# Oliverbansk/Holistic-Robot-Pose-Estimation

Measured on AMD Instinct MI355X. Metric: images/sec/GPU fwd+bwd HRNet-W32 256x256 bs=64; 1/2/4/8-GPU scaling, higher is better.
Workload: dtype bf16; 1 GPU; full network (HRNet-W32 reg backbone + HRNet-W32 DepthNet + heads + FK loss) fwd+loss+bwd+clip+Adam, BASELINE.json configs[2]; global_batch=64, per_gpu_batch=64, image=3x256x256, hrnet_w32_passes_per_image=2, parallelism=dp1, backend=single-process, rccl_ranks=1, hip_graph=True, plan_mode=hybrid, inputs=resident in HBM, optimizer=hrpe_amd.optim.FusedClipAdam (clip 5 + Adam, lr 1e-4)

## Files before the change

holistic-robot-pose-estimation_amd/_native.py:

```python
import ctypes as C
import os
import subprocess

_HERE = os.path.dirname(os.path.abspath(__file__))
LIB_PATH = os.environ.get("HRP_LIB") or os.path.join(_HERE, "libhrp_hip.so")
CSRC = os.path.join(_HERE, "csrc")

HRP_F32, HRP_BF16, HRP_F32X3 = 0, 1, 2
MAX_TAPS = 16
EW_MAX_IN = 4
EW_IDENTITY, EW_AFFINE, EW_BN_TRAIN = 0, 1, 2
FK_MAX_JOINTS, FK_MAX_KP = 32, 24
PIL_KMAX = 12


class HrpError(RuntimeError):
    pass


class ConvDesc(C.Structure):
    _fields_ = [("x", C.c_void_p), ("w", C.c_void_p), ("y", C.c_void_p), ("res", C.c_void_p),
                ("bias", C.c_void_p), ("scale", C.c_void_p), ("shift", C.c_void_p), ("stats", C.c_void_p),
                ("dtype", C.c_int32),
                ("N", C.c_int32), ("H", C.c_int32), ("W", C.c_int32), ("Cin", C.c_int32), ("x_pitch", C.c_int32),
                ("Ho", C.c_int32), ("Wo", C.c_int32), ("Cout", C.c_int32),
                ("y_H", C.c_int32), ("y_W", C.c_int32), ("y_pitch", C.c_int32), ("res_pitch", C.c_int32),
                ("out_stride", C.c_int32), ("out_off_y", C.c_int32), ("out_off_x", C.c_int32),
                ("in_stride", C.c_int32), ("ntaps", C.c_int32),
                ("dy", C.c_int32 * MAX_TAPS), ("dx", C.c_int32 * MAX_TAPS), ("wtap", C.c_int32 * MAX_TAPS),
                ("w_ntaps", C.c_int32), ("w_cout_pad", C.c_int32), ("relu", C.c_int32),
                ("bnb_x", C.c_void_p), ("bnb_mask", C.c_void_p), ("bnb_consts", C.c_void_p),
                ("bnb_x_pitch", C.c_int32), ("bnb_mask_pitch", C.c_int32),
                ("bnb_stats", C.c_void_p), ("bnb_gamma", C.c_void_p), ("bnb_beta", C.c_void_p),
                ("bnb_count", C.c_float), ("bnb_eps", C.c_float),
                ("pro_mode", C.c_int32), ("pro_reserved", C.c_int32),
                ("pro_x2", C.c_void_p), ("pro_stats", C.c_void_p), ("pro_bsums", C.c_void_p),
                ("pro_gamma", C.c_void_p), ("pro_beta", C.c_void_p),
                ("pro_count", C.c_float), ("pro_eps", C.c_float), ("pro_side", C.c_void_p),
                ("pro_mask", C.c_void_p), ("pro_side2", C.c_void_p), ("pro_side2_acc", C.c_int32), ("pro_reserved2", C.c_int32),
                ("res_mask", C.c_void_p),
                ("tail_mode", C.c_int32), ("tail_side_acc", C.c_int32), ("tail_stats", C.c_void_p), ("tail_bsums", C.c_void_p),
                ("tail_gamma", C.c_void_p), ("tail_beta", C.c_void_p), ("tail_count", C.c_float), ("tail_eps", C.c_float),
                ("tail_mask", C.c_void_p), ("tail_g", C.c_void_p), ("tail_side", C.c_void_p),
                ("tail_x2", C.c_void_p), ("tail_w2", C.c_void_p), ("tail_stats2", C.c_void_p), ("tail_gamma2", C.c_void_p),
                ("tail_beta2", C.c_void_p)]


class WgradDesc(C.Structure):
    _fields_ = [("x", C.c_void_p), ("dy", C.c_void_p), ("dw", C.c_void_p),
                ("dtype", C.c_int32),
                ("N", C.c_int32), ("H", C.c_int32), ("W", C.c_int32), ("Cin", C.c_int32), ("x_pitch", C.c_int32),
                ("Ho", C.c_int32), ("Wo", C.c_int32), ("Cout", C.c_int32), ("dy_pitch", C.c_int32),
                ("in_stride", C.c_int32), ("ntaps", C.c_int32),
                ("dy_t", C.c_int32 * MAX_TAPS), ("dx_t", C.c_int32 * MAX_TAPS),
                ("dw_cin", C.c_int32), ("dw_tap_stride", C.c_int32), ("dw_tap_off", C.c_int32), ("accumulate", C.c_int32),
                ("workspace", C.c_void_p), ("workspace_bytes", C.c_int64),
                ("phase", C.c_int32), ("reserved", C.c_int32)]


class WgradFoldDesc(C.Structure):
    _fields_ = [("workspace", C.c_void_p), ("dw", C.c_void_p),
                ("G", C.c_int32), ("pairs", C.c_int32), ("n_cib", C.c_int32), ("nte", C.c_int32), ("nb", C.c_int32),
                ("Cout", C.c_int32), ("dw_cin", C.c_int32), ("ntaps", C.c_int32), ("dw_tap_stride", C.c_int32),
                ("dw_tap_off", C.c_int32), ("accumulate", C.c_int32), ("reserved", C.c_int32)]


class Sim2RealLossDesc(C.Structure):
    _fields_ = [("rendered", C.c_void_p), ("seg", C.c_void_p), ("kp3d", C.c_void_p), ("kp3d_int", C.c_void_p),
                ("B", C.c_int32), ("HW", C.c_int32), ("K", C.c_int32), ("mask_loss", C.c_int32),
                ("w_mask", C.c_float), ("w_iou", C.c_float), ("w_scale", C.c_float), ("w_align", C.c_float),
                ("terms", C.c_void_p), ("d_rendered", C.c_void_p), ("d_kp3d", C.c_void_p), ("d_kp3d_int", C.c_void_p),
                ("workspace", C.c_void_p)]


class SilhouetteDesc(C.Structure):
    _fields_ = [("uv", C.c_void_p), ("xyz", C.c_void_p), ("faces", C.c_void_p),
                ("B", C.c_int32), ("V", C.c_int32), ("F", C.c_int32), ("H", C.c_int32), ("W", C.c_int32),
                ("sigma", C.c_float), ("blur_radius", C.c_float), ("alpha", C.c_void_p), ("logp", C.c_void_p), ("count", C.c_void_p)]


BLOCK_MAX = 2


class BlockDesc(C.Structure):
    _fields_ = [("conv1", ConvDesc), ("conv2", ConvDesc)]


class BlockInfo(C.Structure):
    _fields_ = [("n", C.c_int32), ("grid", C.c_int32), ("lds_bytes", C.c_int32), ("reserved", C.c_int32),
                ("first_wg", C.c_int32 * BLOCK_MAX), ("bands", C.c_int32 * BLOCK_MAX)]


class PackEntry(C.Structure):
    _fields_ = [("src", C.c_void_p), ("dst", C.c_void_p), ("dst_t", C.c_void_p),
                ("Cout", C.c_int32), ("Cin", C.c_int32), ("ntaps", C.c_int32), ("pad_t", C.c_int32)]


class EwInput(C.Structure):
    _fields_ = [("ptr", C.c_void_p), ("pitch", C.c_int32), ("up", C.c_int32), ("mode", C.c_int32),
                ("a", C.c_void_p), ("b", C.c_void_p), ("stats", C.c_void_p),
                ("count", C.c_float), ("eps", C.c_float)]


class EwDesc(C.Structure):
    _fields_ = [("inp", EwInput * EW_MAX_IN), ("nin", C.c_int32), ("out", C.c_void_p),
                ("out_pitch", C.c_int32), ("dtype", C.c_int32),
                ("N", C.c_int32), ("H", C.c_int32), ("W", C.c_int32), ("C", C.c_int32), ("relu", C.c_int32),
                ("mask", C.c_void_p), ("mask_pitch", C.c_int32), ("consts_out", C.c_void_p)]


class EwBwdDesc(C.Structure):
    _fields_ = [("dout", C.c_void_p), ("out", C.c_void_p), ("dout_pitch", C.c_int32), ("out_pitch", C.c_int32),
                ("inp", EwInput), ("din", C.c_void_p), ("din_pitch", C.c_int32), ("sums", C.c_void_p),
                ("dtype", C.c_int32), ("N", C.c_int32), ("H", C.c_int32), ("W", C.c_int32), ("C", C.c_int32),
                ("relu", C.c_int32), ("accumulate", C.c_int32),
                ("mask", C.c_void_p), ("mask_pitch", C.c_int32),
                ("din2", C.c_void_p), ("din2_pitch", C.c_int32), ("accumulate2", C.c_int32), ("pooled", C.c_void_p)]


class BnEntry(C.Structure):
    _fields_ = [("stats", C.c_void_p), ("a", C.c_void_p), ("b", C.c_void_p), ("c", C.c_void_p), ("d", C.c_void_p),
                ("out_scale", C.c_void_p), ("out_shift", C.c_void_p), ("counter", C.c_void_p),
                ("C", C.c_int32), ("count", C.c_float), ("momentum", C.c_float), ("eps", C.c_float),
                ("accumulate", C.c_int32)]


BATCH_MAX = 32
BATCH_CONV, BATCH_WGRAD, BATCH_EW_FWD, BATCH_EW_BWD_REDUCE, BATCH_EW_BWD_APPLY, BATCH_WGRAD_FOLD = range(6)


class BatchInfo(C.Structure):
    _fields_ = [("family", C.c_int32), ("n", C.c_int32), ("dtype", C.c_int32), ("variant", C.c_int32),
                ("grid", C.c_int32), ("lds_bytes", C.c_int32), ("grid2", C.c_int32),
                ("grid3", C.c_int32), ("lds_bytes3", C.c_int32),
                ("blk0", C.c_int32 * (BATCH_MAX + 1)), ("blk2", C.c_int32 * (BATCH_MAX + 1)),
                ("ws_bytes", C.c_int64 * BATCH_MAX)]


class PoseLossDesc(C.Structure):
    _fields_ = [(n, C.c_void_p) for n in ("pose", "rot", "trans", "root_uv", "depth", "xyz_int", "xyz_fk",
                                          "gt_pose", "gt_root_rot", "gt_root_trans", "gt_root_uv", "gt_kp3d", "gt_kp2d", "mask", "K",
                                          "d_pose", "d_rot", "d_trans", "d_root_uv", "d_depth", "d_xyz_int", "d_xyz_fk", "out")] + \
               [("weights", C.c_float * 10), ("B", C.c_int32), ("P", C.c_int32), ("J", C.c_int32), ("root", C.c_int32),
                ("image_size", C.c_float), ("rot_dim", C.c_int32)]


class EvalDesc(C.Structure):
    INPUTS = ("pred_kp3d_fk", "pred_kp3d_int", "gt_kp3d", "gt_kp2d", "K", "pred_joint", "gt_joint", "pred_rot", "gt_rot")
    PER_IMAGE = ("error3d", "error2d", "mean_jointerror", "error_depth", "batch_error_relative", "error3d_relative",
                 "error3d_int", "error2d_int", "error_depth_int", "batch_error_relative_int", "error3d_relative_int")
    PER_BATCH = ("dis3d", "dis2d", "dis3d_int", "dis2d_int", "l1_jointerror", "rotation_diff")
    _fields_ = [(n, C.c_void_p) for n in INPUTS + PER_IMAGE + PER_BATCH] + \
               [(n, C.c_int32) for n in ("B", "nkp", "dof", "rot_dim", "root", "drop_last_joint", "offset", "capacity",
                                         "batch_index", "batch_capacity")]


DEPTH_LOSS_MAX_KP = 16
DEPTH_LOSS_KINDS = {"l1": 0, "mse": 1}
XY_LOSS_KINDS = {None: 0, "l1": 1, "mse": 2}


class DepthLossDesc(C.Structure):
    POINTERS = ("pred", "gt_root_trans", "gt_kp3d", "mask", "loss", "d_pred", "errors", "losses")
    _fields_ = [(n, C.c_void_p) for n in POINTERS] + \
               [(n, C.c_int32) for n in ("B", "W", "J", "nk")] + [("kp_index", C.c_int32 * DEPTH_LOSS_MAX_KP)] + \
               [(n, C.c_int32) for n in ("depth_loss", "xy_loss", "root_col", "want_grad", "offset", "capacity", "batch_index",
                                         "batch_capacity")]


OPT_CHUNK = 4096


class OptTensor(C.Structure):
    _fields_ = [("param", C.c_void_p), ("grad", C.c_void_p), ("exp_avg", C.c_void_p), ("exp_avg_sq", C.c_void_p),
                ("numel", C.c_int64)]


class OptChunk(C.Structure):
    _fields_ = [("tensor", C.c_int32), ("offset", C.c_int32)]


class OptGroup(C.Structure):
    _fields_ = [("lr", C.c_float), ("beta1", C.c_float), ("beta2", C.c_float), ("eps", C.c_float),
                ("weight_decay", C.c_float), ("reserved", C.c_float * 3)]


class RegStepDesc(C.Structure):
    _fields_ = [("M", C.c_int32), ("P", C.c_int32), ("K", C.c_int32), ("N", C.c_int32),
                ("u_prev", C.c_void_p), ("u_bias", C.c_void_p), ("z", C.c_void_p), ("zw", C.c_void_p),
                ("z_len", C.c_int32), ("z_pitch", C.c_int32), ("zw_sk", C.c_int32), ("zw_sp", C.c_int32),
                ("u_out", C.c_void_p), ("a", C.c_void_p), ("a_mask", C.c_void_p), ("v", C.c_void_p),
                ("a_pitch", C.c_int32), ("v_sk", C.c_int32), ("v_sp", C.c_int32), ("a2_pitch", C.c_int32),
                ("a_out", C.c_void_p), ("w", C.c_void_p), ("bias", C.c_void_p), ("out_mask", C.c_void_p),
                ("a2", C.c_void_p), ("w2", C.c_void_p), ("w_sn", C.c_int64), ("w_sk", C.c_int64),
                ("out_pitch", C.c_int32), ("out_accumulate", C.c_int32), ("out_sum_accumulate", C.c_int32), ("w2_sk", C.c_int32),
                ("out", C.c_void_p), ("out_sum", C.c_void_p)]


class LinWgradDesc(C.Structure):
    _fields_ = [("x", C.c_void_p), ("dy", C.c_void_p), ("dw", C.c_void_p), ("dbias", C.c_void_p),
                ("x_pitch", C.c_int32), ("dy_pitch", C.c_int32), ("dw_ld", C.c_int32), ("M", C.c_int32),
                ("K", C.c_int32), ("N", C.c_int32), ("accumulate", C.c_int32), ("reserved", C.c_int32)]


REG_MAX_P, REG_MAX_PROBLEMS, LIN_WGRAD_MAX = 16, 4, 8
COPY_MAX = 16


class CopyDesc(C.Structure):
    _fields_ = [("src", C.c_void_p), ("dst", C.c_void_p), ("src_pitch", C.c_int), ("dst_pitch", C.c_int), ("rows", C.c_int),
                ("cols", C.c_int), ("accumulate", C.c_int), ("reserved", C.c_int)]


def copy_cols_batch(items, stream):
    for i0 in range(0, len(items), COPY_MAX):
        grp = items[i0:i0 + COPY_MAX]
        arr = (CopyDesc * len(grp))()
        for d, (src, sp, dst, dp, rows, cols, acc) in zip(arr, grp):
            d.src, d.src_pitch, d.dst, d.dst_pitch, d.rows, d.cols, d.accumulate = src, sp, dst, dp, rows, cols, acc
        call("hrp_copy_cols_batch", arr, len(grp), stream)


class FkChain(C.Structure):
    _fields_ = [("njoints", C.c_int32), ("parent", C.c_int32 * FK_MAX_JOINTS), ("type", C.c_int32 * FK_MAX_JOINTS),
                ("cfg", C.c_int32 * FK_MAX_JOINTS), ("mimic_mul", C.c_float * FK_MAX_JOINTS),
                ("mimic_off", C.c_float * FK_MAX_JOINTS), ("origin", (C.c_float * 12) * FK_MAX_JOINTS),
                ("axis", (C.c_float * 3) * FK_MAX_JOINTS), ("nkp", C.c_int32), ("kp_frame", C.c_int32 * FK_MAX_KP),
                ("kp_offset", (C.c_float * 3) * FK_MAX_KP), ("dof", C.c_int32)]


DREAM_BANDS = 32
DREAM_JITTER, DREAM_OCCLUSION, DREAM_SHARPNESS, DREAM_CONTRAST, DREAM_BRIGHTNESS, DREAM_COLOR = 1, 2, 4, 8, 16, 32


class DreamSample(C.Structure):
    _fields_ = [("jitter", C.c_double * 3), ("enh", C.c_double * 4), ("flags", C.c_int32),
                ("occ_x", C.c_int32), ("occ_y", C.c_int32), ("occ_w", C.c_int32), ("occ_h", C.c_int32),
                ("pad_x", C.c_int32), ("pad_y", C.c_int32), ("work_w", C.c_int32), ("work_h", C.c_int32),
                ("crop_x0", C.c_int32), ("crop_y0", C.c_int32), ("crop_x1", C.c_int32), ("crop_y1", C.c_int32),
                ("off_x", C.c_int32), ("off_y", C.c_int32), ("side", C.c_int32), ("reserved", C.c_int32),
                ("noise_off", C.c_int64), ("scratch_off", C.c_int64)]


_P, _I, _F, _L = C.c_void_p, C.c_int, C.c_float, C.c_int64
PROTOTYPES = {
    "hrp_version": [], "hrp_device_ok": [],
    "hrp_nchw_to_nhwc": [_P, _P, _I, _I, _I, _I, _I, _I, _P],
    "hrp_nhwc_to_nchw": [_P, _P, _I, _I, _I, _I, _I, _I, _P],
    "hrp_nchw_grad_from_nhwc": [_P, _P, _I, _I, _I, _I, _I, _I, _P],
    "hrp_pack_weights": [_P, _I, _I, _I, _P],
    "hrp_pack_blocks": [_I, _I, _I, _I, _I, _I],
    "hrp_pack_weights_compact": [_P, _P, _I, _I, _I, _P],
    "hrp_nchw_to_nhwc_s2d": [_P, _P, _I, _I, _I, _I, _I, _I, _P],
    "hrp_u8_nchw_to_nhwc": [_P, _P, _I, _I, _I, _I, _I, _I, _F, _I, _P],
    "hrp_gather_f32": [_P, _P, _P, _I, _I, _P],
    "hrp_pil_resize_table": [_I, _I, _P],
    "hrp_pil_resize_normalize": [_P, _I, _I, _I, _I, _P, _P, _I, _I, _P, _I, _I, _I, _P, _P, _P],
    "hrp_broadcast_hw": [_P, _I, _P, _I, _I, _I, _I, _I, _P],
    "hrp_bilinear_nhwc_to_nchw": [_P, _I, _I, _I, _I, _I, _I, _P, _I, _I, _I, _P],
    "hrp_fill_zero": [_P, _L, _P],
    "hrp_maxpool3x3s2_fwd": [_P, _I, _I, _I, _I, _I, _I, _P, _I, _P, _P],
    "hrp_maxpool3x3s2_bwd": [_P, _I, _P, _P, _I, _I, _I, _I, _I, _I, _I, _P],
    "hrp_conv2d_fwd": [C.POINTER(ConvDesc), _P],
    "hrp_conv_rowstrip_channels": [C.POINTER(ConvDesc)],
    "hrp_conv_pointwise": [C.POINTER(ConvDesc)],
    "hrp_conv2d_bwd_weight": [C.POINTER(WgradDesc), _P],
    "hrp_colsum": [_P, _I, _L, _I, _I, _P, _I, _P, _L, _P],
    "hrp_colsum_workspace_bytes": [_L, _I],
    "hrp_ew_fwd": [C.POINTER(EwDesc), _P],
    "hrp_ew_bwd_reduce": [C.POINTER(EwBwdDesc), _P],
    "hrp_ew_pool2": [_P, _I, _I, _P, _I, _I, _I, _I, _I, _P, _P],
    "hrp_ew_bwd_apply": [C.POINTER(EwBwdDesc), _P],
    "hrp_bn_running_update": [_P, _I, _P], "hrp_bn_fold": [_P, _I, _P], "hrp_bn_param_grad": [_P, _I, _P],
    "hrp_avgpool_fwd": [_P, _I, _I, _I, _I, _I, _P, _I, _P],
    "hrp_avgpool_bwd": [_P, _I, _P, _I, _I, _I, _I, _I, _I, _P],
    "hrp_softargmax3d_fwd": [_P, _I, _I, _I, _I, _I, _I, _I, _I, _I, _P, _P, _P],
    "hrp_softargmax3d_bwd": [_P, _I, _I, _I, _I, _I, _I, _I, _I, _I, _P, _P, _P, _P, _I, _P],
    "hrp_pose_geometry_fwd": [_P, _P, _P, _P, _I, _I, _I, _F, _F, _P, _P, _P, _P, _P],
    "hrp_pose_geometry_bwd": [_P, _P, _P, _P, _I, _I, _I, _F, _F, _P, _P, _P, _P, _P, _P, _P],
    "hrp_fk_project_fwd": [_P, _P, _P, _P, _P, _I, _I, _P, _P, _P, _P],
    "hrp_fk_project_bwd": [_P, _P, _P, _P, _P, _I, _I, _P, _P, _P, _P, _P, _P],
    "hrp_fk_project_rot_fwd": [_P, _P, _P, _I, _P, _P, _I, _I, _P, _P, _P, _P],
    "hrp_fk_project_rot_bwd": [_P, _P, _P, _I, _P, _P, _I, _I, _P, _P, _P, _P, _P, _P],
    "hrp_copy_cols": [_P, _I, _P, _I, _I, _I, _I, _P],
    "hrp_copy_cols_batch": [_P, _I, _P],
    "hrp_scale_rows": [_P, _I, _I, _I, _P, _F, _P],
    "hrp_mul_f32": [_P, _I, _P, _I, _P, _I, _I, _I, _I, _P],
    "hrp_opt_grad_sumsq": [_P, _P, _I, _P, _P, _P],
    "hrp_opt_adam_step": [_P, _P, _I, _P, _F, _P, _F, _F, _F, _F, _P],
    "hrp_opt_adam_step_groups": [_P, _P, _I, _P, _F, _P, _P, _I, _P, _P],
    "hrp_opt_set_group": [_P, _I, _I, _F, _F, _F, _F, _F, _P],
    "hrp_grad_accumulate": [_P, _P, _L, _I, _F, _P],
    "hrp_batch_prepare": [_I, _P, _I, _P, C.POINTER(BatchInfo)],
    "hrp_batch_launch": [_P, C.POINTER(BatchInfo), _P],
    "hrp_softargmax_flat_fwd": [_P, _I, _I, _I, _I, _I, _P, _P, _P],
    "hrp_softargmax_flat_bwd": [_P, _I, _I, _I, _I, _I, _P, _P, _P, _P, _I, _P],
    "hrp_rot6d_compose_fwd": [_P, _P, _P, _I, _P],
    "hrp_rot6d_compose_bwd": [_P, _P, _P, _P, _P, _I, _I, _I, _P],
    "hrp_wgrad_fold_desc_of": [C.POINTER(WgradDesc), C.POINTER(WgradFoldDesc)],
    "hrp_batch_wgrad_fold_descs": [_P, C.POINTER(BatchInfo), C.POINTER(WgradFoldDesc)],
    "hrp_block_channels": [C.POINTER(BlockDesc)],
    "hrp_block_prepare": [_P, _I, _P, C.POINTER(BlockInfo)],
    "hrp_block_launch": [_P, C.POINTER(BlockInfo), _P],
    "hrp_pose_loss": [C.POINTER(PoseLossDesc), _P],
    "hrp_l1_loss": [_P, _P, _F, _I, _P, _P, _P],
    "hrp_sim2real_loss": [C.POINTER(Sim2RealLossDesc), _P],
    "hrp_mesh_pose": [_P, _P, _P, _P, _I, _I, _P, _P, _I, _P, _P, _P, _P],
    "hrp_mesh_pose_bwd": [_P, _P, _P, _P, _I, _I, _P, _P, _I, _P, _P, _P, _P],
    "hrp_silhouette_fwd": [C.POINTER(SilhouetteDesc), _P],
    "hrp_silhouette_bwd": [C.POINTER(SilhouetteDesc), _P, _P, _P],
    "hrp_linear_fwd": [_P, _I, _P, _P, _P, _I, _P, _I, _I, _I, _I, _P, _L, _P],
    "hrp_linear_bwd_data": [_P, _I, _P, _P, _I, _I, _I, _I, _I, _P, _L, _P],
    "hrp_linear_workspace_bytes": [_I, _I, _I],
    "hrp_linear_bwd_weight": [_P, _I, _P, _I, _P, _P, _I, _I, _I, _I, _P],
    "hrp_rng_advance": [_P, _P],
    "hrp_dropout_f32": [_P, _I, _P, _I, _P, _I, _I, _F, _P, C.c_uint32, _P],
    "hrp_dropout_masks": [_P, _L, _F, _P, C.c_uint32, _P],
    "hrp_regressor_step": [_P, _I, _P],
    "hrp_linear_wgrad_batch": [_P, _I, _P],
    "hrp_project_fwd": [_P, _P, _I, _I, _P, _P],
    "hrp_project_bwd": [_P, _P, _P, _I, _I, _P, _P],
    "hrp_pnp_solve": [_P, _P, _I, _P, _I, _P, _I, _I, _P, _P, _P, _P],
    "hrp_pnp_bwd": [_P, _P, _I, _P, _I, _P, _P, _I, _I, _I, _P, _P, _P, _P, _P, _P, _P],
    "hrp_dream_augment": [_P, _I, _I, _I, _P, _P, _L, _I, _I, _P, _L, _P, _P],
    "hrp_dream_crop_resize": [_P, _L, _P, _P, _I, _I, _I, _P, _I, _I, _P, _I, _I, _P],
    "hrp_eval_batch": [C.POINTER(EvalDesc), _P],
    "hrp_depth_loss": [C.POINTER(DepthLossDesc), _P],
}

_lib = None


def source_hash():
    import glob
    import hashlib
    files = [os.path.basename(f) for f in glob.glob(os.path.join(CSRC, "*.hip")) + glob.glob(os.path.join(CSRC, "*.h"))]
    names = sorted(files + ["../../include/hrp.h", "Makefile"])
    h = hashlib.sha256()
    for n in names:
        with open(os.path.join(CSRC, n), "rb") as fh:
            h.update(fh.read())
    return h.hexdigest()[:16]


def build(force=False):
    if force:
        subprocess.run(["make", "-C", CSRC, "clean"], check=True, stdout=subprocess.DEVNULL)
    r = subprocess.run(["make", "-C", CSRC, "-j8"], stdout=subprocess.PIPE, stderr=subprocess.STDOUT, text=True)
    if r.returncode != 0:
        raise HrpError("building libhrp_hip.so failed:\n" + r.stdout[-4000:])
    return LIB_PATH


def lib():
    global _lib
    if _lib is None:
        if not os.path.exists(LIB_PATH):
            raise HrpError(f"{LIB_PATH} not found: run `python -c 'import __graft_entry__ as g; g.build()'` "
                           "(there is no CPU fallback)")
        import torch
        L = C.CDLL(LIB_PATH)
        for name, args in PROTOTYPES.items():
            fn = getattr(L, name)
            fn.argtypes = args
            fn.restype = C.c_int
        L.hrp_last_error.restype = C.c_char_p
        L.hrp_last_error.argtypes = []
        L.hrp_source_hash.restype = C.c_char_p
        L.hrp_source_hash.argtypes = []
        L.hrp_wgrad_workspace_bytes.restype = C.c_int64
        L.hrp_linear_workspace_bytes.restype = C.c_int64
        L.hrp_colsum_workspace_bytes.restype = C.c_int64
        L.hrp_wgrad_workspace_bytes.argtypes = [C.POINTER(WgradDesc)]
        L.hrp_batch_table_bytes.restype = C.c_int64
        L.hrp_batch_table_bytes.argtypes = [C.c_int, C.c_int]
        L.hrp_block_table_bytes.restype = C.c_int64
        L.hrp_block_table_bytes.argtypes = []
        _lib = L
    return _lib


def check(rc, what=""):
    if rc != 0:
        raise HrpError(f"{what} failed ({rc}): {lib().hrp_last_error().decode()}")


_profile_hook = None


def set_profile_hook(fn):
    global _profile_hook
    _profile_hook = fn


def profiling():
    return _profile_hook is not None


_skip = frozenset(filter(None, os.environ.get("HRP_SKIP", "").split(",")))


def call(name, *args):
    if _skip and name in _skip:
        return
    if _profile_hook is not None:
        _profile_hook(name, args, lambda: check(getattr(lib(), name)(*args), name))
        return
    check(getattr(lib(), name)(*args), name)


def call_batch(batch, stream):
    name = "hrp_batch_launch"
    if _skip and (name in _skip or FAMILY_FN[batch.fam] in _skip):
        return
    fn = lambda: check(lib().hrp_batch_launch(batch.table.data_ptr(), C.byref(batch.info), stream), name)
    if _profile_hook is not None:
        _profile_hook(name, (batch,), fn)
        return
    fn()


def call_block(batch, stream):
    name = "hrp_block_launch"
    if _skip and name in _skip:
        return
    fn = lambda: check(lib().hrp_block_launch(batch.table, C.byref(batch.info), stream), name)
    if _profile_hook is not None:
        _profile_hook(name, (batch,), fn)
        return
    fn()


FAMILY_FN = {"block": "hrp_block_launch", "conv": "hrp_conv2d_fwd", "wgrad": "hrp_conv2d_bwd_weight", "wgrad_fold": "hrp_wgrad_fold", "ew_fwd": "hrp_ew_fwd", "ew_red": "hrp_ew_bwd_reduce",
             "ew_app": "hrp_ew_bwd_apply"}
```

holistic-robot-pose-estimation_amd/csrc/core.hip:

```cpp
#include "hrp_common.h"
#include <type_traits>
#include <string.h>

namespace hrp {

static thread_local char g_err[512] = "";

void set_error(const char* fmt, ...) {
  va_list ap;
  va_start(ap, fmt);
  vsnprintf(g_err, sizeof(g_err), fmt, ap);
  va_end(ap);
}

int check_launch(const char* what) {
  hipError_t e = hipGetLastError();
  if (e != hipSuccess) {
    set_error("%s: %s", what, hipGetErrorString(e));
    return HRP_ERR_LAUNCH;
  }
  return HRP_OK;
}

template <typename T, typename S>
__global__ __launch_bounds__(256) void nchw_to_nhwc_kernel(const S* __restrict__ src, void* __restrict__ dst,
                                                           int C, int HW, int pitch, float div) {
  size_t p = (size_t)blockIdx.x * 256 + threadIdx.x;
  int n = blockIdx.y;
  if (p >= (size_t)HW) return;
  const S* s = src + (size_t)n * C * HW + p;
  size_t o = ((size_t)n * HW + p) * pitch;
  if (pitch * Elem<T>::SZ == 16) {
    constexpr int V = 16 / Elem<T>::SZ;
    float v[V];
#pragma unroll
    for (int c = 0; c < V; ++c) {
      v[c] = c < C ? (float)s[(size_t)c * HW] : 0.f;
      if (sizeof(S) == 1) v[c] = v[c] * (1.0f / div);
    }
    *(uint4*)((char*)dst + o * Elem<T>::SZ) = Elem<T>::pack(v);
    return;
  }
  for (int c = 0; c < pitch; ++c) {
    float v = c < C ? (float)s[(size_t)c * HW] : 0.f;
    if (sizeof(S) == 1) v = v * (1.0f / div);
    Elem<T>::st(dst, o + c, v);
  }
}

template <typename T, typename S>
__global__ __launch_bounds__(256) void nchw_to_nhwc_s2d_kernel(const S* __restrict__ src, void* __restrict__ dst,
                                                               int C, int H, int W, int pitch, float div) {
  const int Ho = (H + 1) / 2, Wo = (W + 1) / 2;
  size_t p = (size_t)blockIdx.x * 256 + threadIdx.x;
  const int n = blockIdx.y;
  if (p >= (size_t)Ho * Wo) return;
  const int y = p / Wo, x = p - (size_t)y * Wo;
  const S* sn = src + (size_t)n * C * H * W;
  size_t o = ((size_t)n * Ho * Wo + p) * pitch;
  for (int k = 0; k < pitch; ++k) {
    float v = 0.f;
    if (k < 4 * C) {
      const int q = k / C, c = k - q * C, iy = 2 * y + (q >> 1), ix = 2 * x + (q & 1);
      if (iy < H && ix < W) v = (float)sn[((size_t)c * H + iy) * W + ix];
      if (sizeof(S) == 1) v = v * (1.0f / div);
    }
    Elem<T>::st(dst, o + k, v);
  }
}

__global__ __launch_bounds__(256) void gather_f32_kernel(const float* __restrict__ src, const int* __restrict__ idx,
                                                         float* __restrict__ dst, int n, int accumulate) {
  const int i = blockIdx.x * 256 + threadIdx.x;
  if (i >= n) return;
  const int j = idx[i];
  const float v = j >= 0 ? src[j] : 0.f;
  dst[i] = accumulate ? dst[i] + v : v;
}

template <typename T>
__global__ __launch_bounds__(256) void maxpool_fwd_kernel(const void* __restrict__ x, int H, int W, int C, int pitch,
                                                          void* __restrict__ y, int Ho, int Wo, int y_pitch,
                                                          uint8_t* __restrict__ arg, long total) {
  constexpr int V = Elem<T>::VEC;
  const int nv = C / V;
  for (long i = (long)blockIdx.x * 256 + threadIdx.x; i < total; i += (long)gridDim.x * 256) {
    const int cv = i % nv;
    long r = i / nv;
    const int ox = r % Wo; r /= Wo;
    const int oy = r % Ho;
    const long n = r / Ho;
    float best[V];
    int bi[V];
#pragma unroll
    for (int k = 0; k < V; ++k) { best[k] = -INFINITY; bi[k] = 0; }
    for (int ky = 0; ky < 3; ++ky) {
      const int iy = 2 * oy - 1 + ky;
      if (iy < 0 || iy >= H) continue;
      for (int kx = 0; kx < 3; ++kx) {
        const int ix = 2 * ox - 1 + kx;
        if (ix < 0 || ix >= W) continue;
        float f[V];
        Elem<T>::unpack(*(const uint4*)((const char*)x + ((((size_t)n * H + iy) * W + ix) * pitch + cv * V) * Elem<T>::SZ), f);
#pragma unroll
        for (int k = 0; k < V; ++k)
          if (f[k] > best[k]) { best[k] = f[k]; bi[k] = ky * 3 + kx; }
      }
    }
    const size_t o = (((size_t)n * Ho + oy) * Wo + ox);
    *(uint4*)((char*)y + (o * y_pitch + cv * V) * Elem<T>::SZ) = Elem<T>::pack(best);
    if (arg) {
#pragma unroll
      for (int k = 0; k < V; ++k) arg[o * C + cv * V + k] = (uint8_t)bi[k];
    }
  }
}

template <typename T>
__global__ __launch_bounds__(256) void maxpool_bwd_kernel(const void* __restrict__ dy, int Ho, int Wo, int dy_pitch,
                                                          const uint8_t* __restrict__ arg, void* __restrict__ dx, int H, int W,
                                                          int C, int pitch, int accumulate, long total) {
  constexpr int V = Elem<T>::VEC;
  const int nv = C / V;
  for (long i = (long)blockIdx.x * 256 + threadIdx.x; i < total; i += (long)gridDim.x * 256) {
    const int cv = i % nv;
    long r = i / nv;
    const int ix = r % W; r /= W;
    const int iy = r % H;
    const long n = r / H;
    float g[V];
#pragma unroll
    for (int k = 0; k < V; ++k) g[k] = 0.f;
    for (int oy = iy / 2; oy <= (iy + 1) / 2; ++oy) {
      if (oy < 0 || oy >= Ho) continue;
      const int ky = iy - (2 * oy - 1);
      if (ky < 0 || ky > 2) continue;
      for (int ox = ix / 2; ox <= (ix + 1) / 2; ++ox) {
        if (ox < 0 || ox >= Wo) continue;
        const int kx = ix - (2 * ox - 1);
        if (kx < 0 || kx > 2) continue;
        const size_t o = (((size_t)n * Ho + oy) * Wo + ox);
        float f[V];
        Elem<T>::unpack(*(const uint4*)((const char*)dy + (o * dy_pitch + cv * V) * Elem<T>::SZ), f);
        const uint8_t* a = arg + o * C + cv * V;
#pragma unroll
        for (int k = 0; k < V; ++k)
          if (a[k] == ky * 3 + kx) g[k] += f[k];
      }
    }
    char* dst = (char*)dx + ((((size_t)n * H + iy) * W + ix) * pitch + cv * V) * Elem<T>::SZ;
    if (accumulate) {
      float old[V];
      Elem<T>::unpack(*(const uint4*)dst, old);
#pragma unroll
      for (int k = 0; k < V; ++k) g[k] += old[k];
    }
    *(uint4*)dst = Elem<T>::pack(g);
  }
}

template <typename T, bool GRAD>
__global__ __launch_bounds__(256) void nhwc_to_nchw_kernel(const void* __restrict__ src, float* __restrict__ dst,
                                                           int C, int HW, int pitch) {
  __shared__ float tile[64][65];
  const int n = blockIdx.z, p0 = blockIdx.x * 64, c0 = blockIdx.y * 64;
  const int tx = threadIdx.x & 63, ty = threadIdx.x >> 6;
  for (int r = ty; r < 64; r += 4) {
    int p = p0 + r, c = c0 + tx;
    tile[r][tx] = (p < HW && c < C) ? Elem<T>::ld(src, ((size_t)n * HW + p) * pitch + c) : 0.f;
  }
  __syncthreads();
  for (int r = ty; r < 64; r += 4) {
    int c = c0 + r, p = p0 + tx;
    if (p < HW && c < C) dst[((size_t)n * C + c) * HW + p] = tile[tx][r];
  }
}

template <typename T>
__device__ __forceinline__ void pack_entry(const hrp_pack_entry& e, const unsigned blk, const unsigned nblk) {
  constexpr int CK = 32 / Elem<T>::SZ;
  const unsigned Cout = e.Cout, Cin = e.Cin, nt = e.ntaps;
  const unsigned cout_pad = (Cout + 31) / 32 * 32, cin_pad = (Cin + 31) / 32 * 32;
  auto store_row = [&](void* dst, size_t row, const float (&v)[CK]) {
    if constexpr (std::is_same<T, f32x3_t>::value) {
      uint4* q = (uint4*)((char*)dst + row * 32);
      split_bf16x8(v, q[0], q[1]);
      return;
    }
    float a[CK / 2], b[CK / 2];
#pragma unroll
    for (int k = 0; k < CK / 2; ++k) { a[k] = v[k]; b[k] = v[CK / 2 + k]; }
    uint4* q = (uint4*)((char*)dst + row * 32);
    q[0] = Elem<T>::pack(a);
    q[1] = Elem<T>::pack(b);
  };
  if (e.dst) {
    const unsigned nch = (Cin + CK - 1) / CK, rows = nch * nt * cout_pad;
    for (unsigned i = blk * 256 + threadIdx.x; i < rows; i += nblk * 256) {
      const unsigned tap = i % nt, q = i / nt, co = q % cout_pad, ch = q / cout_pad;
      float v[CK];
#pragma unroll
      for (int k = 0; k < CK; ++k) {
        const unsigned ci = ch * CK + k;
        v[k] = (co < Cout && ci < Cin) ? e.src[((size_t)co * Cin + ci) * nt + tap] : 0.f;
      }
      store_row(e.dst, (size_t)(ch * nt + tap) * cout_pad + co, v);
    }
  }
  if (e.dst_t) {
    const unsigned nch = (Cout + CK - 1) / CK, rows = nch * nt * cin_pad;
    for (unsigned i = blk * 256 + threadIdx.x; i < rows; i += nblk * 256) {
      const unsigned tap = i % nt, q = i / nt, ci = q % cin_pad, ch = q / cin_pad;
      float v[CK];
#pragma unroll
      for (int k = 0; k < CK; ++k) {
        const unsigned co = ch * CK + k;
        v[k] = (co < Cout && ci < Cin) ? e.src[((size_t)co * Cin + ci) * nt + tap] : 0.f;
      }
      store_row(e.dst_t, (size_t)(ch * (nt + e.pad_t) + tap) * cin_pad + ci, v);
    }
  }
}

template <typename T>
__global__ __launch_bounds__(256) void pack_weights_kernel(const hrp_pack_entry* __restrict__ table) {
  const hrp_pack_entry e = table[blockIdx.y];
  pack_entry<T>(e, blockIdx.x, gridDim.x);
}

constexpr int PACK_TILE_TAPS = 9;
template <typename T>
__device__ __forceinline__ void pack_store_row(void* dst, const size_t row, const float (&v)[32 / Elem<T>::SZ]) {
  constexpr int CK = 32 / Elem<T>::SZ;
  uint4* q = (uint4*)((char*)dst + row * 32);
  if constexpr (std::is_same<T, f32x3_t>::value) {
    split_bf16x8(v, q[0], q[1]);
  } else {
    float a[CK / 2], b[CK / 2];
#pragma unroll
    for (int k = 0; k < CK / 2; ++k) { a[k] = v[k]; b[k] = v[CK / 2 + k]; }
    q[0] = Elem<T>::pack(a);
    q[1] = Elem<T>::pack(b);
  }
}

template <typename T>
__device__ __forceinline__ void pack_entry_tile(const hrp_pack_entry& e, const unsigned tile_id, float* __restrict__ lds) {
  constexpr int CK = 32 / Elem<T>::SZ, NC = 32 / CK;
  const unsigned Cout = e.Cout, Cin = e.Cin, nt = e.ntaps;
  const unsigned cout_pad = (Cout + 31) / 32 * 32, cin_pad = (Cin + 31) / 32 * 32;
  const unsigned n_cit = cin_pad / 32;
  if (tile_id >= (cout_pad / 32) * n_cit) return;
  const unsigned co0 = (tile_id / n_cit) * 32, ci0 = (tile_id % n_cit) * 32;
  const unsigned span = 32 * nt, pitch = span + 1;
  {
    const unsigned wave = threadIdx.x >> 6, lane = threadIdx.x & 63;
    const unsigned valid = Cin > ci0 ? (Cin - ci0 < 32 ? (Cin - ci0) * nt : span) : 0;
    for (unsigned r0 = wave; r0 < 32; r0 += 16) {
      for (unsigned j = lane; j < span; j += 64) {
        float v[4];
#pragma unroll
        for (int u = 0; u < 4; ++u) {
          const unsigned co = co0 + r0 + 4 * u;
          v[u] = (co < Cout && j < valid) ? e.src[((size_t)co * Cin + ci0) * nt + j] : 0.f;
        }
#pragma unroll
        for (int u = 0; u < 4; ++u) lds[(r0 + 4 * u) * pitch + j] = v[u];
      }
    }
  }
  __syncthreads();
  if (e.dst) {
    const unsigned nch = (Cin + CK - 1) / CK;
    for (unsigned r = threadIdx.x; r < NC * nt * 32; r += 256) {
      const unsigned co = r & 31, q = r >> 5, tap = q % nt, c = q / nt, ch = ci0 / CK + c;
      if (ch >= nch) continue;
      float v[CK];
#pragma unroll
      for (int k = 0; k < CK; ++k) v[k] = lds[co * pitch + (c * CK + k) * nt + tap];
      pack_store_row<T>(e.dst, (size_t)(ch * nt + tap) * cout_pad + co0 + co, v);
    }
  }
  if (e.dst_t) {
    const unsigned nch = (Cout + CK - 1) / CK;
    for (unsigned r = threadIdx.x; r < NC * nt * 32; r += 256) {
      const unsigned ci = r & 31, q = r >> 5, tap = q % nt, c = q / nt, ch = co0 / CK + c;
      if (ch >= nch) continue;
      float v[CK];
#pragma unroll
      for (int k = 0; k < CK; ++k) v[k] = lds[(c * CK + k) * pitch + ci * nt + tap];
      pack_store_row<T>(e.dst_t, (size_t)(ch * (nt + e.pad_t) + tap) * cin_pad + ci0 + ci, v);
    }
  }
}

constexpr int PACK_ROWS_PER_BLOCK = 256 * 4;
template <typename T>
__global__ __launch_bounds__(256) void pack_weights_compact_kernel(const hrp_pack_entry* __restrict__ table, const int32_t* __restrict__ first,
                                                                   const int count) {
  int lo = 0, hi = count;
  while (hi - lo > 1) {
    const int mid = (lo + hi) >> 1;
    if (first[mid] <= (int)blockIdx.x) lo = mid; else hi = mid;
  }
  const hrp_pack_entry e = table[lo];
  if (e.ntaps <= PACK_TILE_TAPS) {
    __shared__ float lds[32 * (32 * PACK_TILE_TAPS + 1)];
    pack_entry_tile<T>(e, blockIdx.x - first[lo], lds);
    return;
  }
  pack_entry<T>(e, blockIdx.x - first[lo], first[lo + 1] - first[lo]);
}

template <typename T>
__global__ __launch_bounds__(256) void colsum_kernel(const void* __restrict__ x, long rows, int C, int pitch,
                                                     float* __restrict__ out, float* __restrict__ ws) {
  __shared__ float part[4][64];
  const int tx = threadIdx.x & 63, ty = threadIdx.x >> 6;
  const int c = blockIdx.y * 64 + tx;
  float s = 0.f;
  if (c < C)
    for (long r = (long)blockIdx.x * 4 + ty; r < rows; r += (long)gridDim.x * 4) s += Elem<T>::ld(x, (size_t)r * pitch + c);
  part[ty][tx] = s;
  __syncthreads();
  if (ty == 0 && c < C) {
    const float v = part[0][tx] + part[1][tx] + part[2][tx] + part[3][tx];
    if (ws) ws[(size_t)blockIdx.x * C + c] = v;
    else atomicAdd(&out[c], v);
  }
}

__global__ __launch_bounds__(256) void colsum_fold_kernel(const float* __restrict__ ws, int groups, int C, float* __restrict__ out,
                                                          int accumulate) {
  const int c = blockIdx.x * 256 + threadIdx.x;
  if (c >= C) return;
  float v = 0.f;
  for (int g0 = 0; g0 < groups; g0 += 8) {
    float t[8];
#pragma unroll
    for (int u = 0; u < 8; ++u) t[u] = g0 + u < groups ? ws[(size_t)(g0 + u) * C + c] : 0.f;
#pragma unroll
    for (int u = 0; u < 8; ++u) v += t[u];
  }
  out[c] = accumulate ? out[c] + v : v;
}

__global__ void bn_running_update_kernel(const hrp_bn_entry* __restrict__ table) {
  const hrp_bn_entry e = table[blockIdx.x];
  for (int c = threadIdx.x; c < e.C; c += blockDim.x) {
    float mean = slot_sum(e.stats, c, 2 * e.C) / e.count;
    float var = fmaxf(slot_sum(e.stats, e.C + c, 2 * e.C) / e.count - mean * mean, 0.f);
    float unbiased = e.count > 1.f ? var * (e.count / (e.count - 1.f)) : var;
    e.a[c] = (1.f - e.momentum) * e.a[c] + e.momentum * mean;
    e.b[c] = (1.f - e.momentum) * e.b[c] + e.momentum * unbiased;
  }
  if (threadIdx.x == 0 && e.counter) *e.counter += 1;
}

__global__ void bn_fold_kernel(const hrp_bn_entry* __restrict__ table) {
  const hrp_bn_entry e = table[blockIdx.x];
  for (int c = threadIdx.x; c < e.C; c += blockDim.x) {
    float sc = e.a[c] * rsqrtf(e.d[c] + e.eps);
    e.out_scale[c] = sc;
    e.out_shift[c] = e.b[c] - e.c[c] * sc;
  }
}

__global__ void bn_param_grad_kernel(const hrp_bn_entry* __restrict__ table) {
  const hrp_bn_entry e = table[blockIdx.x];
  for (int c = threadIdx.x; c < e.C; c += blockDim.x) {
    float dbeta = slot_sum(e.stats, c, 2 * e.C), dgamma = slot_sum(e.stats, e.C + c, 2 * e.C);
    if (e.accumulate) { e.a[c] += dgamma; e.b[c] += dbeta; }
    else { e.a[c] = dgamma; e.b[c] = dbeta; }
  }
}

template <typename T>
__global__ __launch_bounds__(256) void avgpool_fwd_kernel(const void* __restrict__ x, int HW, int C, int pitch,
                                                          float* __restrict__ out, int out_pitch) {
  const int n = blockIdx.y;
  const int c = blockIdx.x * 256 + threadIdx.x;
  if (c >= C) return;
  float s = 0.f;
  for (int p = 0; p < HW; ++p) s += Elem<T>::ld(x, ((size_t)n * HW + p) * pitch + c);
  out[(size_t)n * out_pitch + c] = s / (float)HW;
}

template <typename T>
__global__ __launch_bounds__(256) void avgpool_bwd_kernel(const float* __restrict__ dout, int dout_pitch, void* __restrict__ dx,
                                                          int HW, int C, int pitch, int accumulate) {
  const int n = blockIdx.y;
  const int c = blockIdx.x * 256 + threadIdx.x;
  if (c >= C) return;
  const float g = dout[(size_t)n * dout_pitch + c] / (float)HW;
  for (int p = 0; p < HW; ++p) {
    size_t o = ((size_t)n * HW + p) * pitch + c;
    Elem<T>::st(dx, o, accumulate ? Elem<T>::ld(dx, o) + g : g);
  }
}

__global__ void copy_cols_kernel(const float* __restrict__ src, int sp, float* __restrict__ dst, int dp, int rows, int cols, int acc) {
  size_t i = (size_t)blockIdx.x * 256 + threadIdx.x;
  if (i >= (size_t)rows * cols) return;
  int r = i / cols, c = i % cols;
  float v = src[(size_t)r * sp + c];
  float* d = dst + (size_t)r * dp + c;
  *d = acc ? *d + v : v;
}

struct CopyBatchArgs { hrp_copy_desc d[HRP_COPY_MAX]; };
__global__ void copy_cols_batch_kernel(const CopyBatchArgs a) {
  const hrp_copy_desc& d = a.d[blockIdx.y];
  const size_t total = (size_t)d.rows * d.cols;
  for (size_t i = (size_t)blockIdx.x * 256 + threadIdx.x; i < total; i += (size_t)gridDim.x * 256) {
    const int r = (int)(i / d.cols), c = (int)(i - (size_t)r * d.cols);
    const float v = d.src ? d.src[(size_t)r * d.src_pitch + c] : 0.f;
    float* q = d.dst + (size_t)r * d.dst_pitch + c;
    *q = d.accumulate ? *q + v : v;
  }
}

__global__ void scale_rows_kernel(float* __restrict__ x, int pitch, int rows, int cols, const float* __restrict__ rs, float s) {
  size_t i = (size_t)blockIdx.x * 256 + threadIdx.x;
  if (i >= (size_t)rows * cols) return;
  int r = i / cols, c = i % cols;
  x[(size_t)r * pitch + c] *= (rs ? rs[r] : 1.f) * s;
}

__global__ void mul_kernel(const float* __restrict__ x, int xp, const float* __restrict__ m, int mp, float* __restrict__ y, int yp,
                           int rows, int cols, int acc) {
  size_t i = (size_t)blockIdx.x * 256 + threadIdx.x;
  if (i >= (size_t)rows * cols) return;
  int r = i / cols, c = i % cols;
  float v = x[(size_t)r * xp + c] * m[(size_t)r * mp + c];
  float* d = y + (size_t)r * yp + c;
  *d = acc ? *d + v : v;
}

__device__ __forceinline__ void philox_round(uint32_t (&c)[4], uint32_t k0, uint32_t k1) {
  const uint32_t hi0 = __umulhi(0xD2511F53u, c[0]), lo0 = 0xD2511F53u * c[0];
  const uint32_t hi1 = __umulhi(0xCD9E8D57u, c[2]), lo1 = 0xCD9E8D57u * c[2];
  const uint32_t n0 = hi1 ^ c[1] ^ k0, n1 = lo1, n2 = hi0 ^ c[3] ^ k1, n3 = lo0;
  c[0] = n0; c[1] = n1; c[2] = n2; c[3] = n3;
}

__global__ void rng_advance_kernel(uint64_t* state) { state[1] += 1; }

__global__ __launch_bounds__(256) void dropout_kernel(const float* __restrict__ x, int xp, float* __restrict__ y, int yp,
                                                      float* __restrict__ mask, int rows, int cols, float keep,
                                                      const uint64_t* __restrict__ state, uint32_t salt) {
  const size_t q = (size_t)blockIdx.x * 256 + threadIdx.x;
  const size_t n = (size_t)rows * cols;
  if (q * 4 >= n) return;
  const uint64_t seed = state[0], step = state[1];
  uint32_t c[4] = {(uint32_t)q, (uint32_t)(q >> 32) ^ salt, (uint32_t)step, (uint32_t)(step >> 32)};
  uint32_t k0 = (uint32_t)seed, k1 = (uint32_t)(seed >> 32);
#pragma unroll
  for (int r = 0; r < 10; ++r) {
    philox_round(c, k0, k1);
    k0 += 0x9E3779B9u; k1 += 0xBB67AE85u;
  }
  const float scale = 1.0f / keep;
#pragma unroll
  for (int j = 0; j < 4; ++j) {
    const size_t i = q * 4 + j;
    if (i >= n) break;
    const float u = (float)(c[j] >> 8) * (1.0f / 16777216.0f);
    const float m = u < keep ? scale : 0.f;
    const int r = (int)(i / cols), cc = (int)(i - (size_t)r * cols);
    mask[i] = m;
    y[(size_t)r * yp + cc] = x[(size_t)r * xp + cc] * m;
  }
}

}

using namespace hrp;

#ifndef HRP_SRC_HASH
#define HRP_SRC_HASH "unknown"
#endif
extern "C" const char* hrp_source_hash(void) { return HRP_SRC_HASH; }

extern "C" int hrp_rng_advance(uint64_t* state_dev, void* stream) {
  HRP_REQUIRE(state_dev, "rng_advance: null state");
  hipLaunchKernelGGL(rng_advance_kernel, dim3(1), dim3(1), 0, (hipStream_t)stream, state_dev);
  return check_launch("rng_advance");
}

extern "C" int hrp_dropout_f32(const float* x, int x_pitch, float* y, int y_pitch, float* mask, int rows, int cols, float keep,
                               const uint64_t* state_dev, uint32_t salt, void* stream) {
  HRP_REQUIRE(x && y && mask && state_dev && rows > 0 && cols > 0, "dropout: bad args");
  HRP_REQUIRE(keep > 0.f && keep <= 1.f, "dropout: keep probability %f", (double)keep);
  const size_t quads = ((size_t)rows * cols + 3) / 4;
  hipLaunchKernelGGL(dropout_kernel, dim3((unsigned)((quads + 255) / 256)), dim3(256), 0, (hipStream_t)stream, x, x_pitch, y, y_pitch,
                     mask, rows, cols, keep, state_dev, salt);
  return check_launch("dropout");
}

extern "C" int hrp_mul_f32(const float* x, int x_pitch, const float* m, int m_pitch, float* y, int y_pitch, int rows, int cols,
                           int accumulate, void* stream) {
  HRP_REQUIRE(x && m && y && rows > 0 && cols > 0, "mul_f32: bad args");
  hipLaunchKernelGGL(mul_kernel, dim3(cdiv(rows * cols, 256)), dim3(256), 0, (hipStream_t)stream, x, x_pitch, m, m_pitch, y, y_pitch,
                     rows, cols, accumulate);
  return check_launch("mul_f32");
}

extern "C" const char* hrp_last_error(void) { return hrp::g_err; }
extern "C" int hrp_version(void) { return 100; }

extern "C" int hrp_device_ok(void) {
  int dev = 0;
  if (hipGetDevice(&dev) != hipSuccess) return 0;
  hipDeviceProp_t p;
  if (hipGetDeviceProperties(&p, dev) != hipSuccess) return 0;
  return strncmp(p.gcnArchName, "gfx950", 6) == 0 ? 1 : 0;
}

extern "C" int hrp_nchw_to_nhwc(const float* src, void* dst, int dtype, int N, int C, int H, int W, int dst_pitch, void* stream) {
  HRP_REQUIRE(src && dst && N > 0 && C > 0 && dst_pitch >= C, "nchw_to_nhwc: bad args");
  dim3 grid(cdiv(H * W, 256), N);
  if (dtype == HRP_F32) hipLaunchKernelGGL((nchw_to_nhwc_kernel<float, float>), grid, dim3(256), 0, (hipStream_t)stream, src, dst, C, H * W, dst_pitch, 1.f);
  else hipLaunchKernelGGL((nchw_to_nhwc_kernel<bf16_t, float>), grid, dim3(256), 0, (hipStream_t)stream, src, dst, C, H * W, dst_pitch, 1.f);
  return check_launch("nchw_to_nhwc");
}

extern "C" int hrp_u8_nchw_to_nhwc(const uint8_t* src, void* dst, int dtype, int N, int C, int H, int W, int dst_pitch,
                                   float divisor, int s2d, void* stream) {
  HRP_REQUIRE(src && dst && N > 0 && C > 0 && divisor > 0.f, "u8_nchw_to_nhwc: bad args");
  HRP_REQUIRE(dst_pitch >= (s2d ? 4 * C : C), "u8_nchw_to_nhwc: dst_pitch too small");
  hipStream_t st = (hipStream_t)stream;
  if (s2d) {
    dim3 grid(cdiv(((H + 1) / 2) * ((W + 1) / 2), 256), N);
    if (dtype == HRP_F32) hipLaunchKernelGGL((nchw_to_nhwc_s2d_kernel<float, uint8_t>), grid, dim3(256), 0, st, src, dst, C, H, W, dst_pitch, divisor);
    else hipLaunchKernelGGL((nchw_to_nhwc_s2d_kernel<bf16_t, uint8_t>), grid, dim3(256), 0, st, src, dst, C, H, W, dst_pitch, divisor);
  } else {
    dim3 grid(cdiv(H * W, 256), N);
    if (dtype == HRP_F32) hipLaunchKernelGGL((nchw_to_nhwc_kernel<float, uint8_t>), grid, dim3(256), 0, st, src, dst, C, H * W, dst_pitch, divisor);
    else hipLaunchKernelGGL((nchw_to_nhwc_kernel<bf16_t, uint8_t>), grid, dim3(256), 0, st, src, dst, C, H * W, dst_pitch, divisor);
  }
  return check_launch("u8_nchw_to_nhwc");
}

extern "C" int hrp_nchw_to_nhwc_s2d(const float* src, void* dst, int dtype, int N, int C, int H, int W, int dst_pitch, void* stream) {
  HRP_REQUIRE(src && dst && N > 0 && C > 0 && dst_pitch >= 4 * C, "nchw_to_nhwc_s2d: bad args");
  dim3 grid(cdiv(((H + 1) / 2) * ((W + 1) / 2), 256), N);
  if (dtype == HRP_F32) hipLaunchKernelGGL((nchw_to_nhwc_s2d_kernel<float, float>), grid, dim3(256), 0, (hipStream_t)stream, src, dst, C, H, W, dst_pitch, 1.f);
  else hipLaunchKernelGGL((nchw_to_nhwc_s2d_kernel<bf16_t, float>), grid, dim3(256), 0, (hipStream_t)stream, src, dst, C, H, W, dst_pitch, 1.f);
  return check_launch("nchw_to_nhwc_s2d");
}

extern "C" int hrp_fill_zero(void* p, int64_t bytes, void* stream) {
  HRP_REQUIRE(p && bytes >= 0, "fill_zero: bad args");
  zero_async(p, (size_t)bytes, (hipStream_t)stream);
  return check_launch("fill_zero");
}

extern "C" int hrp_gather_f32(const float* src, const int32_t* idx, float* dst, int n, int accumulate, void* stream) {
  HRP_REQUIRE(src && idx && dst && n > 0, "gather_f32: bad args");
  hipLaunchKernelGGL(gather_f32_kernel, dim3(cdiv(n, 256)), dim3(256), 0, (hipStream_t)stream, src, idx, dst, n, accumulate);
  return check_launch("gather_f32");
}

extern "C" int hrp_maxpool3x3s2_fwd(const void* x, int dtype, int N, int H, int W, int C, int pitch, void* y, int y_pitch,
                                    uint8_t* argmax, void* stream) {
  const int vec = dtype == HRP_F32 ? 4 : 8, sz = dtype == HRP_F32 ? 4 : 2;
  HRP_REQUIRE(x && y && N > 0 && H > 0 && W > 0 && C > 0, "maxpool_fwd: bad args");
  HRP_REQUIRE(C % vec == 0 && pitch % vec == 0 && y_pitch % vec == 0 && (uintptr_t)x % 16 == 0 && (uintptr_t)y % 16 == 0,
              "maxpool_fwd: channels / pitches must be multiples of %d and the tensors 16-byte aligned", vec);
  (void)sz;
  const int Ho = (H + 2 - 3) / 2 + 1, Wo = (W + 2 - 3) / 2 + 1;
  const long total = (long)N * Ho * Wo * (C / vec);
  long blocks = (total + 255) / 256;
  if (blocks > 4096) blocks = 4096;
  if (dtype == HRP_F32) hipLaunchKernelGGL(maxpool_fwd_kernel<float>, dim3((int)blocks), dim3(256), 0, (hipStream_t)stream, x, H, W, C, pitch, y, Ho, Wo, y_pitch, argmax, total);
  else hipLaunchKernelGGL(maxpool_fwd_kernel<bf16_t>, dim3((int)blocks), dim3(256), 0, (hipStream_t)stream, x, H, W, C, pitch, y, Ho, Wo, y_pitch, argmax, total);
  return check_launch("maxpool_fwd");
}

extern "C" int hrp_maxpool3x3s2_bwd(const void* dy, int dy_pitch, const uint8_t* argmax, void* dx, int dtype, int N, int H, int W,
                                    int C, int pitch, int accumulate, void* stream) {
  const int vec = dtype == HRP_F32 ? 4 : 8;
  HRP_REQUIRE(dy && argmax && dx && N > 0 && H > 0 && W > 0 && C > 0, "maxpool_bwd: bad args");
  HRP_REQUIRE(C % vec == 0 && pitch % vec == 0 && dy_pitch % vec == 0 && (uintptr_t)dx % 16 == 0 && (uintptr_t)dy % 16 == 0,
              "maxpool_bwd: channels / pitches must be multiples of %d and the tensors 16-byte aligned", vec);
  const int Ho = (H + 2 - 3) / 2 + 1, Wo = (W + 2 - 3) / 2 + 1;
  const long total = (long)N * H * W * (C / vec);
  long blocks = (total + 255) / 256;
  if (blocks > 4096) blocks = 4096;
  if (dtype == HRP_F32) hipLaunchKernelGGL(maxpool_bwd_kernel<float>, dim3((int)blocks), dim3(256), 0, (hipStream_t)stream, dy, Ho, Wo, dy_pitch, argmax, dx, H, W, C, pitch, accumulate, total);
  else hipLaunchKernelGGL(maxpool_bwd_kernel<bf16_t>, dim3((int)blocks), dim3(256), 0, (hipStream_t)stream, dy, Ho, Wo, dy_pitch, argmax, dx, H, W, C, pitch, accumulate, total);
  return check_launch("maxpool_bwd");
}

extern "C" int hrp_nhwc_to_nchw(const void* src, float* dst, int dtype, int N, int C, int H, int W, int src_pitch, void* stream) {
  HRP_REQUIRE(src && dst && N > 0 && C > 0 && src_pitch >= C, "nhwc_to_nchw: bad args");
  dim3 grid(cdiv(H * W, 64), cdiv(C, 64), N);
  if (dtype == HRP_F32) hipLaunchKernelGGL((nhwc_to_nchw_kernel<float, false>), grid, dim3(256), 0, (hipStream_t)stream, src, dst, C, H * W, src_pitch);
  else hipLaunchKernelGGL((nhwc_to_nchw_kernel<bf16_t, false>), grid, dim3(256), 0, (hipStream_t)stream, src, dst, C, H * W, src_pitch);
  return check_launch("nhwc_to_nchw");
}

extern "C" int hrp_nchw_grad_from_nhwc(const void* src, float* dst, int dtype, int N, int C, int H, int W, int src_pitch, void* stream) {
  return hrp_nhwc_to_nchw(src, dst, dtype, N, C, H, W, src_pitch, stream);
}

extern "C" int hrp_pack_weights(const hrp_pack_entry* table_dev, int count, int dtype, int max_elems, void* stream) {
  HRP_REQUIRE(table_dev && count > 0, "pack_weights: empty table");
  int bx = cdiv(max_elems, 256 * 16 * 4);
  if (bx < 1) bx = 1;
  if (bx > 256) bx = 256;
  dim3 grid(bx, count);
  if (dtype == HRP_F32) hipLaunchKernelGGL(pack_weights_kernel<float>, grid, dim3(256), 0, (hipStream_t)stream, table_dev);
  else if (dtype == HRP_F32X3) hipLaunchKernelGGL(pack_weights_kernel<f32x3_t>, grid, dim3(256), 0, (hipStream_t)stream, table_dev);
  else hipLaunchKernelGGL(pack_weights_kernel<bf16_t>, grid, dim3(256), 0, (hipStream_t)stream, table_dev);
  return check_launch("pack_weights");
}

extern "C" int hrp_pack_blocks(int Cout, int Cin, int ntaps, int dtype, int has_dst, int has_dst_t) {
  if (Cout <= 0 || Cin <= 0 || ntaps <= 0) return 0;
  const int CK = dtype == HRP_BF16 ? 16 : 8;
  const long cout_pad = (Cout + 31) / 32 * 32, cin_pad = (Cin + 31) / 32 * 32;
  if (ntaps <= PACK_TILE_TAPS) return (int)((cout_pad / 32) * (cin_pad / 32));
  const long rf = has_dst ? (long)cdiv(Cin, CK) * ntaps * cout_pad : 0, rt = has_dst_t ? (long)cdiv(Cout, CK) * ntaps * cin_pad : 0;
  const long rows = rf > rt ? rf : rt;
  const long b = (rows + PACK_ROWS_PER_BLOCK - 1) / PACK_ROWS_PER_BLOCK;
  return (int)(b < 1 ? 1 : b);
}

extern "C" int hrp_pack_weights_compact(const hrp_pack_entry* table_dev, const int32_t* first_block_dev, int count, int total_blocks,
                                        int dtype, void* stream) {
  HRP_REQUIRE(table_dev && first_block_dev && count > 0 && total_blocks >= count, "pack_weights_compact: empty table / fewer workgroups than entries");
  const dim3 grid(total_blocks);
  if (dtype == HRP_F32) hipLaunchKernelGGL(pack_weights_compact_kernel<float>, grid, dim3(256), 0, (hipStream_t)stream, table_dev, first_block_dev, count);
  else if (dtype == HRP_F32X3) hipLaunchKernelGGL(pack_weights_compact_kernel<f32x3_t>, grid, dim3(256), 0, (hipStream_t)stream, table_dev, first_block_dev, count);
  else hipLaunchKernelGGL(pack_weights_compact_kernel<bf16_t>, grid, dim3(256), 0, (hipStream_t)stream, table_dev, first_block_dev, count);
  return check_launch("pack_weights_compact");
}

static inline int colsum_groups(int64_t rows) {
  int gx = (int)((rows + 63) / 64);
  if (gx > 512) gx = 512;
  return gx < 1 ? 1 : gx;
}

extern "C" int64_t hrp_colsum_workspace_bytes(int64_t rows, int C) { return rows > 0 && C > 0 ? (int64_t)colsum_groups(rows) * C * 4 : 0; }

extern "C" int hrp_colsum(const void* x, int dtype, int64_t rows, int C, int pitch, float* out, int accumulate, void* workspace,
                          int64_t workspace_bytes, void* stream) {
  HRP_REQUIRE(x && out && rows > 0 && C > 0, "colsum: bad args");
  const int gx = colsum_groups(rows);
  float* ws = (float*)workspace;
  HRP_REQUIRE(!ws || workspace_bytes >= (int64_t)gx * C * 4, "colsum: workspace too small");
  if (!ws && !accumulate) zero_async(out, sizeof(float) * C, (hipStream_t)stream);
  dim3 grid(gx, cdiv(C, 64));
  if (dtype == HRP_F32) hipLaunchKernelGGL(colsum_kernel<float>, grid, dim3(256), 0, (hipStream_t)stream, x, (long)rows, C, pitch, out, ws);
  else hipLaunchKernelGGL(colsum_kernel<bf16_t>, grid, dim3(256), 0, (hipStream_t)stream, x, (long)rows, C, pitch, out, ws);
  if (ws) hipLaunchKernelGGL(colsum_fold_kernel, dim3(cdiv(C, 256)), dim3(256), 0, (hipStream_t)stream, ws, gx, C, out, accumulate);
  return check_launch("colsum");
}

extern "C" int hrp_bn_running_update(const hrp_bn_entry* table_dev, int count, void* stream) {
  HRP_REQUIRE(table_dev && count > 0, "bn_running_update: empty table");
  hipLaunchKernelGGL(bn_running_update_kernel, dim3(count), dim3(256), 0, (hipStream_t)stream, table_dev);
  return check_launch("bn_running_update");
}
extern "C" int hrp_bn_fold(const hrp_bn_entry* table_dev, int count, void* stream) {
  HRP_REQUIRE(table_dev && count > 0, "bn_fold: empty table");
  hipLaunchKernelGGL(bn_fold_kernel, dim3(count), dim3(256), 0, (hipStream_t)stream, table_dev);
  return check_launch("bn_fold");
}
extern "C" int hrp_bn_param_grad(const hrp_bn_entry* table_dev, int count, void* stream) {
  HRP_REQUIRE(table_dev && count > 0, "bn_param_grad: empty table");
  hipLaunchKernelGGL(bn_param_grad_kernel, dim3(count), dim3(256), 0, (hipStream_t)stream, table_dev);
  return check_launch("bn_param_grad");
}

__global__ __launch_bounds__(256) void opt_grad_sumsq_kernel(const hrp_opt_tensor* __restrict__ tensors,
                                                             const hrp_opt_chunk* __restrict__ chunks,
                                                             float* __restrict__ slots, float* __restrict__ chunk_sums) {
  const hrp_opt_chunk ck = chunks[blockIdx.x];
  const hrp_opt_tensor t = tensors[ck.tensor];
  const int64_t base = (int64_t)ck.offset * HRP_OPT_CHUNK;
  const int64_t left = t.numel - base;
  const int n = left < HRP_OPT_CHUNK ? (int)left : HRP_OPT_CHUNK;
  const float* g = t.grad + base;
  float s = 0.f;
  if ((n & 3) == 0 && ((uintptr_t)g & 15) == 0) {
    for (int i = threadIdx.x * 4; i < n; i += 1024) {
      const float4 v = *(const float4*)(g + i);
      s += v.x * v.x + v.y * v.y + v.z * v.z + v.w * v.w;
    }
  } else {
    for (int i = threadIdx.x; i < n; i += 256) s += g[i] * g[i];
  }
  s = wave_sum(s);
  __shared__ float part[4];
  if ((threadIdx.x & 63) == 0) part[threadIdx.x >> 6] = s;
  __syncthreads();
  if (threadIdx.x == 0) {
    const float tot = part[0] + part[1] + part[2] + part[3];
    if (chunk_sums) chunk_sums[blockIdx.x] = tot;
    else atomicAdd(&slots[blockIdx.x & (HRP_STAT_SLOTS - 1)], tot);
  }
}

__global__ __launch_bounds__(256) void opt_fold_sumsq_kernel(const float* __restrict__ chunk_sums, int n, float* __restrict__ slots) {
  __shared__ float part[256];
  float s = 0.f;
  for (int i = threadIdx.x; i < n; i += 256) s += chunk_sums[i];
  part[threadIdx.x] = s;
  __syncthreads();
  for (int o = 128; o > 0; o >>= 1) {
    if ((int)threadIdx.x < o) part[threadIdx.x] += part[threadIdx.x + o];
    __syncthreads();
  }
  if (threadIdx.x < HRP_STAT_SLOTS) slots[threadIdx.x] = threadIdx.x == 0 ? part[0] : 0.f;
}

template <bool DECAY>
__device__ __forceinline__ void opt_adam_chunk(const hrp_opt_tensor t, const hrp_opt_chunk ck, const float* __restrict__ slots,
                                               float max_norm, const float* __restrict__ step_dev, float lr, float b1, float b2,
                                               float eps, float wd) {
  const int64_t base = (int64_t)ck.offset * HRP_OPT_CHUNK;
  const int64_t left = t.numel - base;
  const int n = left < HRP_OPT_CHUNK ? (int)left : HRP_OPT_CHUNK;
  float clip = 1.f;
  if (max_norm > 0.f) {
    float ss = 0.f;
#pragma unroll
    for (int k = 0; k < HRP_STAT_SLOTS; ++k) ss += slots[k];
    clip = fminf(1.f, max_norm / (sqrtf(ss) + 1e-6f));
  }
  const float step = *step_dev;
  const float bc1 = 1.f - powf(b1, step), bc2 = 1.f - powf(b2, step);
  const float step_size = lr / bc1, inv_sqrt_bc2 = 1.f / sqrtf(bc2);
  float* p = t.param + base;
  float* g = t.grad + base;
  float* m = t.exp_avg + base;
  float* v = t.exp_avg_sq + base;
  auto run = [&](auto with_decay) {
    auto upd = [&](float& pp, float& gg, float& mm, float& vv) {
      gg *= clip;
      if constexpr (decltype(with_decay)::value) {
        const float ge = gg + wd * pp;
        mm = b1 * mm + (1.f - b1) * ge;
        vv = b2 * vv + (1.f - b2) * ge * ge;
      } else {
        mm = b1 * mm + (1.f - b1) * gg;
        vv = b2 * vv + (1.f - b2) * gg * gg;
      }
      pp -= step_size * mm / (sqrtf(vv) * inv_sqrt_bc2 + eps);
    };
    if ((n & 3) == 0 && (((uintptr_t)p | (uintptr_t)g | (uintptr_t)m | (uintptr_t)v) & 15) == 0) {
      for (int i = threadIdx.x * 4; i < n; i += 1024) {
        float4 pp = *(float4*)(p + i), gg = *(float4*)(g + i), mm = *(float4*)(m + i), vv = *(float4*)(v + i);
        upd(pp.x, gg.x, mm.x, vv.x); upd(pp.y, gg.y, mm.y, vv.y); upd(pp.z, gg.z, mm.z, vv.z); upd(pp.w, gg.w, mm.w, vv.w);
        *(float4*)(p + i) = pp; *(float4*)(g + i) = gg; *(float4*)(m + i) = mm; *(float4*)(v + i) = vv;
      }
    } else {
      for (int i = threadIdx.x; i < n; i += 256) upd(p[i], g[i], m[i], v[i]);
    }
  };
  if (DECAY && wd != 0.f) run(std::true_type{});
  else run(std::false_type{});
}

__global__ __launch_bounds__(256) void opt_adam_kernel(const hrp_opt_tensor* __restrict__ tensors,
                                                       const hrp_opt_chunk* __restrict__ chunks,
                                                       const float* __restrict__ slots, float max_norm,
                                                       const float* __restrict__ step_dev, float lr, float b1, float b2,
                                                       float eps) {
  const hrp_opt_chunk ck = chunks[blockIdx.x];
  const hrp_opt_tensor t = tensors[ck.tensor];
  opt_adam_chunk<false>(t, ck, slots, max_norm, step_dev, lr, b1, b2, eps, 0.f);
}

__global__ __launch_bounds__(256) void opt_adam_groups_kernel(const hrp_opt_tensor* __restrict__ tensors,
                                                              const hrp_opt_chunk* __restrict__ chunks,
                                                              const float* __restrict__ slots, float max_norm,
                                                              const float* __restrict__ step_dev,
                                                              const hrp_opt_group* __restrict__ groups, int ngroups,
                                                              const int32_t* __restrict__ tensor_group) {
  const hrp_opt_chunk ck = chunks[blockIdx.x];
  const int gi = tensor_group[ck.tensor];
  const hrp_opt_group h = groups[gi < 0 ? 0 : gi >= ngroups ? ngroups - 1 : gi];
  opt_adam_chunk<true>(tensors[ck.tensor], ck, slots, max_norm, step_dev, h.lr, h.beta1, h.beta2, h.eps, h.weight_decay);
}

__global__ void opt_set_group_kernel(hrp_opt_group* __restrict__ groups, int index, float lr, float b1, float b2, float eps,
                                     float wd) {
  hrp_opt_group h = {};
  h.lr = lr, h.beta1 = b1, h.beta2 = b2, h.eps = eps, h.weight_decay = wd;
  groups[index] = h;
}

extern "C" int hrp_opt_grad_sumsq(const hrp_opt_tensor* tensors_dev, const hrp_opt_chunk* chunks_dev, int nchunks,
                                  float* sumsq_slots, float* chunk_sums, void* stream) {
  HRP_REQUIRE(tensors_dev && chunks_dev && sumsq_slots && nchunks > 0, "opt_grad_sumsq: bad args");
  hipLaunchKernelGGL(opt_grad_sumsq_kernel, dim3(nchunks), dim3(256), 0, (hipStream_t)stream, tensors_dev, chunks_dev, sumsq_slots,
                     chunk_sums);
  if (chunk_sums)
    hipLaunchKernelGGL(opt_fold_sumsq_kernel, dim3(1), dim3(256), 0, (hipStream_t)stream, chunk_sums, nchunks, sumsq_slots);
  return check_launch("opt_grad_sumsq");
}
extern "C" int hrp_opt_adam_step(const hrp_opt_tensor* tensors_dev, const hrp_opt_chunk* chunks_dev, int nchunks,
                                 const float* sumsq_slots, float max_norm, const float* step_dev,
                                 float lr, float beta1, float beta2, float eps, void* stream) {
  HRP_REQUIRE(tensors_dev && chunks_dev && step_dev && nchunks > 0, "opt_adam_step: bad args");
  HRP_REQUIRE(max_norm <= 0.f || sumsq_slots, "opt_adam_step: clipping needs the sum-of-squares slots");
  hipLaunchKernelGGL(opt_adam_kernel, dim3(nchunks), dim3(256), 0, (hipStream_t)stream, tensors_dev, chunks_dev, sumsq_slots,
                     max_norm, step_dev, lr, beta1, beta2, eps);
  return check_launch("opt_adam_step");
}

extern "C" int hrp_opt_adam_step_groups(const hrp_opt_tensor* tensors_dev, const hrp_opt_chunk* chunks_dev, int nchunks,
                                        const float* sumsq_slots, float max_norm, const float* step_dev,
                                        const hrp_opt_group* groups_dev, int ngroups, const int32_t* tensor_group_dev,
                                        void* stream) {
  HRP_REQUIRE(tensors_dev && chunks_dev && step_dev && nchunks > 0, "opt_adam_step_groups: bad args");
  HRP_REQUIRE(groups_dev && tensor_group_dev, "opt_adam_step_groups: null group table");
  HRP_REQUIRE(ngroups >= 1, "opt_adam_step_groups: ngroups %d < 1", ngroups);
  HRP_REQUIRE(max_norm <= 0.f || sumsq_slots, "opt_adam_step_groups: clipping needs the sum-of-squares slots");
  hipLaunchKernelGGL(opt_adam_groups_kernel, dim3(nchunks), dim3(256), 0, (hipStream_t)stream, tensors_dev, chunks_dev,
                     sumsq_slots, max_norm, step_dev, groups_dev, ngroups, tensor_group_dev);
  return check_launch("opt_adam_step_groups");
}
extern "C" int hrp_opt_set_group(hrp_opt_group* groups_dev, int ngroups, int index, float lr, float beta1, float beta2, float eps,
                                 float weight_decay, void* stream) {
  HRP_REQUIRE(groups_dev, "opt_set_group: null group table");
  HRP_REQUIRE(ngroups >= 1, "opt_set_group: ngroups %d < 1", ngroups);
  HRP_REQUIRE(index >= 0 && index < ngroups, "opt_set_group: index %d outside [0, %d)", index, ngroups);
  hipLaunchKernelGGL(opt_set_group_kernel, dim3(1), dim3(1), 0, (hipStream_t)stream, groups_dev, index, lr, beta1, beta2, eps,
                     weight_decay);
  return check_launch("opt_set_group");
}

constexpr int GACC_THREADS = 256, GACC_MAX_BLOCKS = 256 * 8;

typedef float gacc_f4 __attribute__((ext_vector_type(4)));

template <int MODE, bool SCALED, typename V>
__device__ __forceinline__ V gacc_sum(V a, V s, float scale) {
#pragma clang fp contract(off)
  V v = s;
  if (SCALED) v = s * scale;
  if (MODE) v = a + v;
  return v;
}
template <int MODE, typename V>
__device__ __forceinline__ V gacc_load(const V* p) {
  if (MODE) return *p;
  return V(0.f);
}

template <int MODE, bool SCALED>
__global__ __launch_bounds__(GACC_THREADS) void grad_accumulate_kernel(const float* __restrict__ src, float* __restrict__ acc,
                                                                       int64_t n, float scale) {
  const int64_t nvec = n >> 2;
  const int64_t stride = (int64_t)gridDim.x * GACC_THREADS;
  const gacc_f4* __restrict__ s4 = (const gacc_f4*)src;
  gacc_f4* __restrict__ a4 = (gacc_f4*)acc;
  int64_t i = (int64_t)blockIdx.x * GACC_THREADS + threadIdx.x;
  for (; i + stride < nvec; i += 2 * stride) {
    const gacc_f4 s0 = s4[i], s1 = s4[i + stride];
    const gacc_f4 a0 = gacc_load<MODE>(a4 + i), a1 = gacc_load<MODE>(a4 + i + stride);
    a4[i] = gacc_sum<MODE, SCALED>(a0, s0, scale);
    a4[i + stride] = gacc_sum<MODE, SCALED>(a1, s1, scale);
  }
  if (i < nvec) a4[i] = gacc_sum<MODE, SCALED>(gacc_load<MODE>(a4 + i), s4[i], scale);
  const int64_t t = (nvec << 2) + threadIdx.x;
  if (blockIdx.x == 0 && t < n) acc[t] = gacc_sum<MODE, SCALED>(gacc_load<MODE>(acc + t), src[t], scale);
}

extern "C" int hrp_grad_accumulate(const float* src, float* acc, int64_t n, int first, float scale, void* stream) {
  HRP_REQUIRE(src && acc && n > 0, "grad_accumulate: bad args");
  HRP_REQUIRE((uintptr_t)src % 16 == 0 && (uintptr_t)acc % 16 == 0, "grad_accumulate: src and acc must be 16-byte aligned");
  HRP_REQUIRE(src != acc, "grad_accumulate: src and acc are the same buffer");
  const int64_t nvec = n >> 2;
  const int64_t want = (nvec + 2 * GACC_THREADS - 1) / (2 * GACC_THREADS);
  const dim3 grid((unsigned)(want < 1 ? 1 : (want > GACC_MAX_BLOCKS ? GACC_MAX_BLOCKS : want))), block(GACC_THREADS);
  const hipStream_t st = (hipStream_t)stream;
  const bool scaled = scale != 1.f;
  if (first) {
    if (scaled) hipLaunchKernelGGL((grad_accumulate_kernel<0, true>), grid, block, 0, st, src, acc, n, scale);
    else hipLaunchKernelGGL((grad_accumulate_kernel<0, false>), grid, block, 0, st, src, acc, n, scale);
  } else {
    if (scaled) hipLaunchKernelGGL((grad_accumulate_kernel<1, true>), grid, block, 0, st, src, acc, n, scale);
    else hipLaunchKernelGGL((grad_accumulate_kernel<1, false>), grid, block, 0, st, src, acc, n, scale);
  }
  return check_launch("grad_accumulate");
}

extern "C" int hrp_avgpool_fwd(const void* x, int dtype, int N, int HW, int C, int pitch, float* out, int out_pitch, void* stream) {
  HRP_REQUIRE(x && out && N > 0 && HW > 0 && C > 0, "avgpool_fwd: bad args");
  dim3 grid(cdiv(C, 256), N);
  if (dtype == HRP_F32) hipLaunchKernelGGL(avgpool_fwd_kernel<float>, grid, dim3(256), 0, (hipStream_t)stream, x, HW, C, pitch, out, out_pitch);
  else hipLaunchKernelGGL(avgpool_fwd_kernel<bf16_t>, grid, dim3(256), 0, (hipStream_t)stream, x, HW, C, pitch, out, out_pitch);
  return check_launch("avgpool_fwd");
}
extern "C" int hrp_avgpool_bwd(const float* dout, int dout_pitch, void* dx, int dtype, int N, int HW, int C, int pitch, int accumulate, void* stream) {
  HRP_REQUIRE(dout && dx && N > 0 && HW > 0 && C > 0, "avgpool_bwd: bad args");
  dim3 grid(cdiv(C, 256), N);
  if (dtype == HRP_F32) hipLaunchKernelGGL(avgpool_bwd_kernel<float>, grid, dim3(256), 0, (hipStream_t)stream, dout, dout_pitch, dx, HW, C, pitch, accumulate);
  else hipLaunchKernelGGL(avgpool_bwd_kernel<bf16_t>, grid, dim3(256), 0, (hipStream_t)stream, dout, dout_pitch, dx, HW, C, pitch, accumulate);
  return check_launch("avgpool_bwd");
}

extern "C" int hrp_copy_cols(const float* src, int src_pitch, float* dst, int dst_pitch, int rows, int cols, int accumulate, void* stream) {
  HRP_REQUIRE(src && dst && rows > 0 && cols > 0, "copy_cols: bad args");
  hipLaunchKernelGGL(copy_cols_kernel, dim3(cdiv(rows * cols, 256)), dim3(256), 0, (hipStream_t)stream, src, src_pitch, dst, dst_pitch, rows, cols, accumulate);
  return check_launch("copy_cols");
}
extern "C" int hrp_copy_cols_batch(const hrp_copy_desc* descs, int n, void* stream) {
  HRP_REQUIRE(descs && n > 0 && n <= HRP_COPY_MAX, "copy_cols_batch: 1 .. %d problems (n=%d)", HRP_COPY_MAX, n);
  CopyBatchArgs a;
  size_t most = 0;
  for (int i = 0; i < n; ++i) {
    const hrp_copy_desc& d = descs[i];
    HRP_REQUIRE(d.dst && d.rows > 0 && d.cols > 0 && d.dst_pitch >= d.cols && (!d.src || d.src_pitch >= d.cols),
                "copy_cols_batch: problem %d: bad pointers / shape (rows=%d cols=%d pitches %d -> %d)", i, d.rows, d.cols, d.src_pitch, d.dst_pitch);
    HRP_REQUIRE(d.src || !d.accumulate, "copy_cols_batch: problem %d accumulates nothing (src == NULL)", i);
    a.d[i] = d;
    const size_t t = (size_t)d.rows * d.cols;
    most = t > most ? t : most;
  }
  const int gx = (int)(most >= 64 * 256 ? 64 : cdiv((int)most, 256));
  hipLaunchKernelGGL(copy_cols_batch_kernel, dim3(gx, n), dim3(256), 0, (hipStream_t)stream, a);
  return check_launch("copy_cols_batch");
}
extern "C" int hrp_scale_rows(float* x, int pitch, int rows, int cols, const float* row_scale, float s, void* stream) {
  HRP_REQUIRE(x && rows > 0 && cols > 0, "scale_rows: bad args");
  hipLaunchKernelGGL(scale_rows_kernel, dim3(cdiv(rows * cols, 256)), dim3(256), 0, (hipStream_t)stream, x, pitch, rows, cols, row_scale, s);
  return check_launch("scale_rows");
}
```

holistic-robot-pose-estimation_amd/optim.py:

```python
import ctypes as C

import torch

from . import _native as nv


class FusedClipAdam(torch.optim.Optimizer):
    def __init__(self, params, lr=1e-3, betas=(0.9, 0.999), eps=1e-8, max_norm=None, weight_decay=0.0, device_hyper=False):
        params = list(params)
        grouped = any(isinstance(p, dict) for p in params)
        if grouped:
            if not all(isinstance(p, dict) for p in params):
                raise ValueError("FusedClipAdam: either parameters or parameter-group dicts, not both")
            params = [dict(g, params=[p for p in g["params"] if p.requires_grad]) for g in params]
            params = [g for g in params if g["params"]]
        else:
            params = [p for p in params if p.requires_grad]
        if not params:
            raise ValueError("FusedClipAdam: no parameters")
        self._device_hyper = bool(grouped or device_hyper or weight_decay)
        super().__init__(params, dict(lr=float(lr), betas=(float(betas[0]), float(betas[1])), eps=float(eps),
                                      weight_decay=float(weight_decay) if self._device_hyper else 0, amsgrad=False,
                                      maximize=False, foreach=None, capturable=True, differentiable=False, fused=None))
        for g in self.param_groups:
            if g["amsgrad"] or g["maximize"]:
                raise ValueError("FusedClipAdam: amsgrad / maximize are not supported")
        self.params = [p for g in self.param_groups for p in g["params"]] if self._device_hyper else self.param_groups[0]["params"]
        dev = self.params[0].device
        if dev.type != "cuda":
            raise nv.HrpError("FusedClipAdam runs on an MI355X (gfx950) only; there is no CPU path")
        for p in self.params:
            if p.dtype != torch.float32 or not p.is_contiguous() or p.device != dev:
                raise ValueError("FusedClipAdam: parameters must be contiguous fp32 tensors on one device")
        self.device = dev
        self.max_norm = float(max_norm) if max_norm else 0.0
        total = sum((p.numel() + 3) // 4 * 4 for p in self.params)
        self._m = torch.zeros(total, dtype=torch.float32, device=dev)
        self._v = torch.zeros(total, dtype=torch.float32, device=dev)
        self.state_views, off = [], 0
        for p in self.params:
            n = p.numel()
            self.state_views.append((self._m[off:off + n].view_as(p), self._v[off:off + n].view_as(p)))
            off += (n + 3) // 4 * 4
        self.step_count = torch.zeros(1, dtype=torch.float32, device=dev)
        self._publish_state()
        self._slots = torch.zeros(8, dtype=torch.float32, device=dev)
        self._chunk_sums = None
        self._grad_ptrs = None
        self._tensors = self._chunks = None
        self._nchunks = 0
        if self._device_hyper:
            ng = len(self.param_groups)
            self._groups = torch.zeros(ng * C.sizeof(nv.OptGroup) // 4, dtype=torch.float32, device=dev)
            self._tensor_group = torch.tensor([i for i, g in enumerate(self.param_groups) for _ in g["params"]],
                                              dtype=torch.int32, device=dev)
            self._hyper_mirror = [None] * ng
            self.publish_hyper()

    def _hyper(self, g):
        return (float(g["lr"]), float(g["betas"][0]), float(g["betas"][1]), float(g["eps"]), float(g["weight_decay"]))

    def hyper_is_stale(self):
        return self._device_hyper and any(self._hyper(g) != m for g, m in zip(self.param_groups, self._hyper_mirror))

    def publish_hyper(self):
        if not self._device_hyper:
            return
        s = None
        for i, g in enumerate(self.param_groups):
            h = self._hyper(g)
            if h == self._hyper_mirror[i]:
                continue
            if s is None:
                if torch.cuda.is_current_stream_capturing():
                    raise RuntimeError("FusedClipAdam.publish_hyper() during a HIP graph capture: publish before the capture "
                                       "and after every replay")
                s = torch.cuda.current_stream(self.device).cuda_stream
            nv.call("hrp_opt_set_group", self._groups.data_ptr(), len(self.param_groups), i, *h, s)
            self._hyper_mirror[i] = h

    def _publish_state(self):
        for p, (m, v) in zip(self.params, self.state_views):
            self.state[p] = {"step": self.step_count.view(()), "exp_avg": m, "exp_avg_sq": v}

    def state_dict(self):
        sd = super().state_dict()
        sd["state"] = {k: dict(v, step=v["step"].clone()) for k, v in sd["state"].items()}
        return sd

    def load_state_dict(self, state_dict):
        if not self._device_hyper and len(state_dict["param_groups"]) != 1:
            raise ValueError("FusedClipAdam: one parameter group only")
        for g in state_dict["param_groups"]:
            if self._device_hyper:
                if g.get("amsgrad", False) or g.get("maximize", False):
                    raise ValueError("FusedClipAdam: amsgrad / maximize are not supported")
            elif g.get("weight_decay", 0) or g.get("amsgrad", False) or g.get("maximize", False):
                raise ValueError("FusedClipAdam: weight_decay / amsgrad / maximize are not supported")
        super().load_state_dict(state_dict)
        steps = set()
        with torch.no_grad():
            for p, (m, v) in zip(self.params, self.state_views):
                st = self.state.get(p)
                if not st:
                    m.zero_()
                    v.zero_()
                    continue
                m.copy_(st["exp_avg"])
                v.copy_(st["exp_avg_sq"])
                steps.add(float(st["step"]))
            if len(steps) > 1:
                raise ValueError(f"FusedClipAdam: parameters at different step counts {sorted(steps)}")
            self.step_count.fill_(steps.pop() if steps else 0.0)
        for g in self.param_groups:
            g["capturable"] = True
        self._publish_state()

    def _build_tables(self):
        ptrs = tuple(p.grad.data_ptr() for p in self.params)
        if ptrs == self._grad_ptrs:
            return
        tab = (nv.OptTensor * len(self.params))()
        chunks = []
        for i, (p, (m, v)) in enumerate(zip(self.params, self.state_views)):
            g = p.grad
            if g.dtype != torch.float32 or not g.is_contiguous():
                raise ValueError("FusedClipAdam: gradients must be contiguous fp32")
            tab[i].param, tab[i].grad, tab[i].exp_avg, tab[i].exp_avg_sq = p.data_ptr(), g.data_ptr(), m.data_ptr(), v.data_ptr()
            tab[i].numel = p.numel()
            chunks += [(i, k) for k in range((p.numel() + nv.OPT_CHUNK - 1) // nv.OPT_CHUNK)]
        ck = (nv.OptChunk * len(chunks))()
        for j, (i, k) in enumerate(chunks):
            ck[j].tensor, ck[j].offset = i, k
        self._tensors = torch.frombuffer(bytearray(bytes(tab)), dtype=torch.uint8).to(self.device)
        self._chunks = torch.frombuffer(bytearray(bytes(ck)), dtype=torch.uint8).to(self.device)
        self._nchunks = len(chunks)
        self._chunk_sums = torch.zeros(self._nchunks, dtype=torch.float32, device=self.device)
        self._grad_ptrs = ptrs

    def prepare(self):
        if any(p.grad is None for p in self.params):
            raise ValueError("FusedClipAdam: every parameter needs a gradient (run one backward first)")
        self._build_tables()

    @torch.no_grad()
    def step(self, closure=None):
        if closure is not None:
            raise ValueError("FusedClipAdam: closures are not supported")
        if self._device_hyper:
            if not torch.cuda.is_current_stream_capturing():
                self.publish_hyper()
            elif self.hyper_is_stale():
                raise RuntimeError("FusedClipAdam: param_groups changed since the device table was written and a HIP graph is being "
                                   "captured; call publish_hyper() before the capture (and after every replay)")
        self.prepare()
        g = self.param_groups[0]
        s = torch.cuda.current_stream(self.device).cuda_stream
        self.step_count += 1
        if self.max_norm > 0:
            nv.call("hrp_opt_grad_sumsq", self._tensors.data_ptr(), self._chunks.data_ptr(), self._nchunks,
                    self._slots.data_ptr(), self._chunk_sums.data_ptr(), s)
        if self._device_hyper:
            nv.call("hrp_opt_adam_step_groups", self._tensors.data_ptr(), self._chunks.data_ptr(), self._nchunks,
                    self._slots.data_ptr(), self.max_norm, self.step_count.data_ptr(),
                    self._groups.data_ptr(), len(self.param_groups), self._tensor_group.data_ptr(), s)
        else:
            nv.call("hrp_opt_adam_step", self._tensors.data_ptr(), self._chunks.data_ptr(), self._nchunks,
                    self._slots.data_ptr(), self.max_norm, self.step_count.data_ptr(),
                    float(g["lr"]), float(g["betas"][0]), float(g["betas"][1]), float(g["eps"]), s)
        from .plan import bump_param_epoch
        bump_param_epoch()

    def total_norm(self):
        return self._slots.sum().sqrt()

    def zero_grad(self, set_to_none=False):
        for p in self.params:
            if p.grad is not None:
                if set_to_none:
                    p.grad = None
                else:
                    p.grad.zero_()
```

holistic-robot-pose-estimation_amd/parallel.py:

```python
import os

import torch
import torch.distributed as dist


def force_world1():
    return os.environ.get("HRP_DIST_WORLD1", "") not in ("", "0")


def collectives_active():
    return dist.is_available() and dist.is_initialized() and (dist.get_world_size() > 1 or force_world1())


def init_distributed(backend=None):
    world = int(os.environ.get("WORLD_SIZE", "1"))
    rank = int(os.environ.get("RANK", "0"))
    local = int(os.environ.get("LOCAL_RANK", "0"))
    if (world > 1 or force_world1()) and not dist.is_initialized():
        os.environ.setdefault("MASTER_ADDR", "127.0.0.1")
        os.environ.setdefault("MASTER_PORT", "29500")
        if backend is None:
            backend = os.environ.get("HRP_DIST_BACKEND") or ("nccl" if torch.cuda.is_available() else "gloo")
        if backend == "nccl":
            torch.cuda.set_device(local)
        dist.init_process_group(backend=backend, rank=rank, world_size=world)
    return rank, world, local


def broadcast_module(module, src=0):
    if not collectives_active():
        return
    for t in list(module.parameters()) + list(module.buffers()):
        dist.broadcast(t.data, src=src)


class GradAllReducer:

    def __init__(self, bucket_mb=64, payload=None):
        self.bucket_elems = int(bucket_mb * 1024 * 1024 // 4)
        self.payload = payload or os.environ.get("HRP_GRAD_PAYLOAD", "fp32")
        assert self.payload in ("fp32", "bf16")
        self._pending = []

    def buckets(self, flat):
        n = flat.numel()
        return [flat[i:min(i + self.bucket_elems, n)] for i in range(0, n, self.bucket_elems)]

    def start(self, flat, ranges):
        if not collectives_active():
            return []
        works = []
        for off, n in ranges:
            for b in self.buckets(flat[off:off + n]):
                if self.payload == "bf16":
                    c = b.to(torch.bfloat16)
                    self._pending.append((b, c))
                    works.append(dist.all_reduce(c, op=dist.ReduceOp.SUM, async_op=True))
                else:
                    works.append(dist.all_reduce(b, op=dist.ReduceOp.SUM, async_op=True))
        return works

    def finish(self, works, flats):
        for w in works:
            w.wait()
        for b, c in self._pending:
            b.copy_(c)
        self._pending = []
        if collectives_active():
            for flat in flats:
                flat.div_(dist.get_world_size())

    @staticmethod
    def complement(ranges, total):
        out, pos = [], 0
        for off, n in sorted(ranges):
            if off > pos:
                out.append((pos, off - pos))
            pos = max(pos, off + n)
        if pos < total:
            out.append((pos, total - pos))
        return out

    def reduce_module(self, module):
        if not module.accumulation_complete():
            return False
        self(module.flat_grads())
        return True

    def __call__(self, flats):
        if not collectives_active():
            return
        works = []
        for flat in flats:
            works += self.start(flat, [(0, flat.numel())])
        self.finish(works, flats)
```

holistic-robot-pose-estimation_amd/plan.py:

```python
import collections
import contextlib
import ctypes as C
import math
import os

import torch

from . import _native as nv

BN_EPS = 1e-5
STAT_SLOTS = 8


def _rup(a, b):
    return (a + b - 1) // b * b


def _dt(dtype):
    return nv.HRP_F32 if dtype == torch.float32 else nv.HRP_BF16


def _cdt(plan, dtype):
    if dtype == torch.float32:
        return nv.HRP_F32X3 if plan.x3 else nv.HRP_F32
    return nv.HRP_BF16


class TensorH:

    def __init__(self, plan, N, H, W, Cc, dtype, buf=None, offset=0, pitch=None, base=None):
        self.plan, self.N, self.H, self.W, self.C, self.dtype = plan, N, H, W, Cc, dtype
        self.pitch = pitch if pitch is not None else _rup(Cc, 8)
        self.offset = offset
        self.base = base
        if buf is None:
            buf = torch.zeros(N * H * W * self.pitch, dtype=dtype, device=plan.device)
            plan.keep.append(buf)
        self.buf = buf
        self._grad = None
        self.grad_written = False
        self.requires_grad = False
        self.stats = None
        self.producer = None
        self.lane_path = plan.lane_path
        self._grad_paths = []
        self.n_readers = self.n_bn_readers = 0

    @property
    def esz(self):
        return self.buf.element_size()

    def ptr(self):
        return self.buf.data_ptr() + self.offset * self.esz

    def grad_buf(self):
        root = self.base if self.base is not None else self
        if root._grad is None:
            root._grad = torch.zeros_like(root.buf)
            self.plan.keep.append(root._grad)
        return root._grad

    def gptr(self):
        return self.grad_buf().data_ptr() + self.offset * self.esz

    def take_grad_slot(self):
        acc = self.grad_written
        self.grad_written = True
        self.grad_buf()
        root = self.base if self.base is not None else self
        root.grad_written = True
        self.plan.grad_owner[self.gptr()] = root
        here = self.plan.lane_path
        if any(lanes_concurrent(here, q) for q in root._grad_paths):
            raise RuntimeError("plan: a gradient is accumulated from two concurrent lanes")
        root._grad_paths.append(here)
        return 1 if acc else 0

    def check_readable(self):
        if lanes_concurrent(self.plan.lane_path, self.lane_path):
            raise RuntimeError("plan: a tensor is consumed in a lane concurrent with its producer")
        self.materialize()
        self.n_readers += 1

    def materialize(self):
        op = getattr(self, "pending_input", None)
        if op is not None:
            self.pending_input = None
            self.plan.pending_inputs.remove(self)
            self.lane_path = self.plan.lane_path
            self.plan.fwd.append(op)
        pend = getattr(self, "pending_block_end", None)
        if pend is not None:
            self.pending_block_end = None
            self.plan.fwd.append(pend["launch"])
            if self in self.plan.pending_block_ends:
                self.plan.pending_block_ends.remove(self)

    def view4(self):
        return self.buf.view(self.N, self.H, self.W, self.pitch)[..., :self.C]


class Term:

    def __init__(self, t, bn=None, up=1):
        self.t, self.bn, self.up = t, bn, up


class ParamW:

    def __init__(self, param, cout, cin, ntaps):
        self.param, self.cout, self.cin, self.ntaps = param, cout, cin, ntaps
        self.fwd_off = self.bwd_off = None
        self.pad_t = 0
        self.t_ntaps = set()
        self.grad_written = False
        self.first_use = None
        self.src = None


RELU_BITMASK = True

SERIAL_LANES = bool(os.environ.get("HRP_SERIAL_LANES"))


MAX_LANE_DEPTH = 1


PLAN_MODE = os.environ.get("HRP_PLAN_MODE", "hybrid")
FUSE_BN_REDUCE = True
WGRAD_DEFER = True
WGRAD_FOLD_EVERY = 32
WGRAD_SINK = int(os.environ.get("HRP_WGRAD_SINK", "16"))
PARITY_PAD = True
ROWCONV_FUSE = True
BLOCK_END_FUSE = True
BLOCK_END_REDUCE_FUSE = True
BLOCK_FUSE = os.environ.get("HRP_BLOCK_FUSE", "1") not in ("0", "")
MASKED_RES = True
BLOCK_END_FWD_FUSE = os.environ.get("HRP_BLOCK_END_FWD", "1") not in ("0", "")
BNECK_TAIL_FUSE = os.environ.get("HRP_TAIL_FUSE", "1") not in ("0", "")
POOL_FUSE_GRADS = os.environ.get("HRP_POOL_FUSE", "0") not in ("0", "")
LAZY_INPUTS = os.environ.get("HRP_LAZY_INPUTS", "1") not in ("0", "")
ARENA_ZERO_EARLY = True
BATCHING = True
GREEDY_MERGE = True
BATCH_FAMILIES = None
PLAN_STATS = bool(os.environ.get("HRP_PLAN_STATS"))
DBG_SYNC = os.environ.get("HRP_DBG_SYNC")

MAX_TILE_DILATION = 4

PARAM_EPOCH = 0
_PLAN_SERIAL = 0


def bump_param_epoch():
    global PARAM_EPOCH
    PARAM_EPOCH += 1


Entry = collections.namedtuple("Entry", "lane path op")


class _OpList(list):

    def __init__(self, plan):
        super().__init__()
        self.plan = plan

    def append(self, op):
        list.append(self, Entry(self.plan.cur_lane, self.plan.lane_path, op))


FAMILIES = {"conv": (nv.BATCH_CONV, "hrp_conv2d_fwd", nv.ConvDesc),
            "wgrad": (nv.BATCH_WGRAD, "hrp_conv2d_bwd_weight", nv.WgradDesc),
            "ew_fwd": (nv.BATCH_EW_FWD, "hrp_ew_fwd", nv.EwDesc),
            "ew_red": (nv.BATCH_EW_BWD_REDUCE, "hrp_ew_bwd_reduce", nv.EwBwdDesc),
            "ew_app": (nv.BATCH_EW_BWD_APPLY, "hrp_ew_bwd_apply", nv.EwBwdDesc),
            "wgrad_fold": (nv.BATCH_WGRAD_FOLD, None, nv.WgradFoldDesc)}


class Launch:
    __slots__ = ("fam", "desc")

    def __init__(self, fam, desc):
        self.fam, self.desc = fam, desc

    def __call__(self, s):
        nv.call(FAMILIES[self.fam][1], C.byref(self.desc), s)

    def launches(self):
        return [self]

    def fold_desc(self):
        f = nv.WgradFoldDesc()
        nv.check(nv.lib().hrp_wgrad_fold_desc_of(C.byref(self.desc), C.byref(f)), "hrp_wgrad_fold_desc_of")
        return f

    def fold_descs(self):
        return [self.fold_desc()]

    def merge_key(self):
        d = self.desc
        if BATCH_FAMILIES is not None and self.fam not in BATCH_FAMILIES:
            return None
        esz = 2 if d.dtype == nv.HRP_BF16 else 4
        if self.fam == "conv":
            if d.ntaps not in (1, 2, 4, 9) or (d.Cin * esz) % 32 or (d.dtype != nv.HRP_BF16 and d.H == 1 and d.W == 1 and d.Cin >= 512):
                return None
            if d.ntaps == 1 and nv.lib().hrp_conv_pointwise(C.byref(d)):
                return None
            return ("conv", d.dtype, d.ntaps)
        if self.fam == "wgrad":
            return ("wgrad", d.dtype, d.ntaps, d.reserved)
        if d.C % (16 // esz):
            return None
        return (self.fam, d.dtype)

    def written(self):
        d = self.desc
        if self.fam == "conv":
            main = d.y + ((d.out_off_y * d.y_W + d.out_off_x) * d.y_pitch if d.out_stride > 1 else 0)
            return tuple(a for a in (main, d.pro_side, d.pro_side2) if a)
        if self.fam in ("wgrad", "wgrad_fold"):
            return (d.dw + 4 * d.dw_tap_off,)
        if self.fam == "ew_fwd":
            return (d.out,)
        if self.fam == "ew_red":
            return (d.sums,)
        return tuple(x for x in (d.din, d.din2) if x)


class BatchLaunch:

    def __init__(self, plan, items):
        self.plan, self.items = plan, list(items)
        self.fam = items[0].fam
        self.info, self.table, self.singles, self.folds = None, None, False, None

    def launches(self):
        return self.items

    def merge_key(self):
        return self.items[0].merge_key()

    def ws_query(self):
        n = len(self.items)
        arr = (nv.WgradDesc * n)(*[it.desc for it in self.items])
        info = nv.BatchInfo()
        nv.check(nv.lib().hrp_batch_prepare(nv.BATCH_WGRAD, arr, n, None, C.byref(info)), "hrp_batch_prepare")
        return [int(info.ws_bytes[i]) for i in range(n)]

    def prepare(self):
        famid, _, dtype = FAMILIES[self.fam]
        n = len(self.items)
        arr = (dtype * n)(*[it.desc for it in self.items])
        info = nv.BatchInfo()
        nbytes = int(nv.lib().hrp_batch_table_bytes(famid, n))
        host = (C.c_char * nbytes)()
        try:
            nv.check(nv.lib().hrp_batch_prepare(famid, arr, n, host, C.byref(info)), "hrp_batch_prepare")
        except nv.HrpError:
            if self.fam == "wgrad_fold":
                raise
            if PLAN_STATS:
                import sys
                print(f"plan: batch of {n} {self.fam} launches runs one by one ({nv.lib().hrp_last_error().decode()})", file=sys.stderr)
            self.singles = True
            return
        self.info = info
        if self.fam == "wgrad" and self.items[0].desc.phase == 1:
            folds = (nv.WgradFoldDesc * n)()
            nv.check(nv.lib().hrp_batch_wgrad_fold_descs(host, C.byref(info), folds), "hrp_batch_wgrad_fold_descs")
            self.folds = list(folds)
        self.table = torch.frombuffer(bytearray(bytes(host)), dtype=torch.uint8).to(self.plan.device)
        self.plan.keep.append(self.table)

    def fold_descs(self):
        if not self.singles:
            return self.folds
        return [it.fold_desc() for it in self.items]

    def __call__(self, s):
        if self.singles:
            for it in self.items:
                it(s)
        else:
            nv.call_batch(self, s)


class BlockLaunch:
    fam = "block"

    def __init__(self, desc):
        self.desc = desc
        self._single = None

    def launches(self):
        return [self]

    def merge_key(self):
        return ("block",)

    def written(self):
        return (self.desc.conv2.y,)

    def __call__(self, s):
        if self._single is None:
            self._single = BlockBatch(None, [self])
        self._single(s)


class BlockBatch:
    fam = "block"

    def __init__(self, plan, items):
        self.plan, self.items = plan, sorted(items, key=lambda it: it.desc.conv1.Cin)
        self.info, self.table = None, None

    def launches(self):
        return self.items

    def merge_key(self):
        return None

    def prepare(self):
        n = len(self.items)
        arr = (nv.BlockDesc * n)(*[it.desc for it in self.items])
        self.info = nv.BlockInfo()
        self.table = (C.c_char * int(nv.lib().hrp_block_table_bytes()))()
        nv.check(nv.lib().hrp_block_prepare(arr, n, self.table, C.byref(self.info)), "hrp_block_prepare")

    def __call__(self, s):
        if self.table is None:
            self.prepare()
        nv.call_block(self, s)


def _pair_block(plan, ops):
    items = [l for op in ops for l in op.launches()]
    c32 = [it for it in items if it.desc.conv1.Cin == 32]
    c64 = [it for it in items if it.desc.conv1.Cin != 32]
    out = []
    while c32 and c64:
        out.append(BlockBatch(plan, [c32.pop(0), c64.pop(0)]))
    out += [BlockBatch(plan, [it]) for it in c32 + c64]
    return out


def _merge_ops(plan, ops):
    items = [l for op in ops for l in op.launches()]
    out, cur, seen = [], [], set()
    for it in items:
        w = it.written()
        if len(cur) == nv.BATCH_MAX or any(a in seen for a in w):
            out.append(cur)
            cur, seen = [], set()
        cur.append(it)
        seen.update(w)
    out.append(cur)
    return [g[0] if len(g) == 1 else BatchLaunch(plan, g) for g in out]


class _Seq:
    def __init__(self):
        self.items, self.blocks = [], {}


class _Par:
    def __init__(self):
        self.lanes = {}


class _LaneSync:

    def __init__(self, kind, parent, children):
        self.kind, self.parent, self.children = kind, parent, children

    def run(self, streams):
        for c in self.children:
            if self.kind == "fork":
                streams[c].wait_stream(streams[self.parent])
            else:
                streams[self.parent].wait_stream(streams[c])


class _PackJoin:

    def __init__(self, plan):
        self.plan = plan

    def run(self, streams):
        if self.plan._pack_stream is not None:
            streams[0].wait_stream(self.plan._pack_stream)

    def __call__(self, s):
        if self.plan._pack_stream is not None and not SERIAL_LANES:
            torch.cuda.current_stream(self.plan.device).wait_stream(self.plan._pack_stream)


def lanes_concurrent(a, b):
    for (ba, la), (bb, lb) in zip(a, b):
        if ba != bb:
            return False
        if la != lb:
            return True
    return False


class GradAccumulation:

    def __init__(self, steps, average):
        self.steps = steps
        self.scale = 1.0 / steps if average else 1.0
        self.index = 0
        self.buf, self.views, self._key = None, {}, None

    def begin(self):
        self.index = 0

    def complete(self):
        return self.index >= self.steps

    def bind(self, plan):
        key = (str(plan.device), plan.grad_arena.numel(), tuple((id(p), off) for p, (off, _) in zip(plan._grad_params, plan._grad_layout)))
        if key == self._key:
            return
        if self.index:
            raise RuntimeError("gradient accumulation: the set of trainable parameters changed in the middle of a cycle "
                               "(this plan lays its gradient arena out differently); call begin_accumulation() first")
        self.buf = torch.zeros_like(plan.grad_arena)
        self.views = {}
        for p, (off, n) in zip(plan._grad_params, plan._grad_layout):
            v = self.buf[off:off + n].view(p.shape)
            v._hrp_plan_grad = True
            self.views[id(p)] = v
        self._key = key

    def accumulate(self, plan, stream):
        self.bind(plan)
        if self.index >= self.steps:
            raise RuntimeError(f"gradient accumulation: {self.steps} micro-batches are already in the buffer "
                               f"(set_grad_accumulation(steps={self.steps})); call begin_accumulation() to start the next cycle")
        nv.call("hrp_grad_accumulate", plan.grad_arena.data_ptr(), self.buf.data_ptr(), plan.grad_arena.numel(),
                1 if self.index == 0 else 0, self.scale, stream)
        self.index += 1


class Plan:
    def __init__(self, device, dtype, training, need_grad):
        self.device, self.dtype, self.training, self.need_grad = device, dtype, training, need_grad
        self.x3 = False
        self.keep = []
        self.cur_lane, self.lane_path, self.n_lanes = 0, (), 1
        self._lane_ids, self._n_blocks, self._side_streams = {}, 0, []
        self.fwd, self.bwd = _OpList(self), _OpList(self)
        self.weights = {}
        self.weight_list = []
        self.bn_train = []
        self.bn_fold = {}
        self.bn_fold_hat = {}
        self.bn_bwd = []
        self.stats_floats = 0
        self.bsums_floats = 0
        self.param_grads = {}
        self.inputs, self.outputs = {}, {}
        self.dyn = {}
        self.built = False
        self._versions = None
        self._late = []
        self.out_handles = []
        self.grad_arena = None
        self._grad_views = {}
        self._grad_layout = []
        self._grad_params = []
        self.accum = None
        self.bwd_split, self.split_active = None, False
        self.bwd_cuts = None
        self.pre_pack = []
        self.counters = {}
        self.wgrad_ws_bytes = {}
        self.wgrad_ws = {}
        self.merged, self.fwd_run, self.bwd_run = False, [], []
        self._block_lanes = {}
        self._rng, self.n_dropout = None, 0
        self.linear_grad_written = set()
        self.grad_owner = {}
        self.reg_chains = []
        self.pending_inputs = []
        self.pending_block_ends = []
        self.row_last_writer = {}

    def new(self, N, H, W, Cc, dtype=None, pitch=None):
        return TensorH(self, N, H, W, Cc, dtype or self.dtype, pitch=pitch)

    def weight(self, param, cout, cin, ntaps):
        w = self.weights.get(id(param))
        if w is None:
            w = ParamW(param, cout, cin, ntaps)
            self.weights[id(param)] = w
            self.weight_list.append(w)
        if w.first_use is None:
            w.first_use = len(self.fwd)
        return w

    def preallocate_param_grads(self, params):
        params = [p for p in params if p.requires_grad]
        params = [p for p in params if p.dim() > 1] + [p for p in params if p.dim() <= 1]
        total = sum(_rup(p.numel(), 4) for p in params)
        self.grad_arena = torch.zeros(max(total, 4), dtype=torch.float32, device=self.device)
        off = 0
        self._grad_layout = []
        self._grad_params = params
        for p in params:
            self._grad_views[id(p)] = self.grad_arena[off:off + p.numel()].view(p.shape)
            self._grad_views[id(p)]._hrp_plan_grad = True
            self._grad_layout.append((off, p.numel()))
            off += _rup(p.numel(), 4)

    def grad_of_param(self, p):
        e = self.param_grads.get(id(p))
        if e is None:
            g = self._grad_views.get(id(p))
            if g is None:
                g = torch.zeros_like(p, dtype=torch.float32)
            e = (p, g)
            self.param_grads[id(p)] = e
            self.keep.append(e[1])
        return e[1]

    def rng_state(self):
        if self._rng is None:
            global _PLAN_SERIAL
            _PLAN_SERIAL += 1
            rank = torch.distributed.get_rank() if (torch.distributed.is_available() and torch.distributed.is_initialized()) else 0
            seed = (int(torch.initial_seed()) ^ (rank << 48) ^ (_PLAN_SERIAL << 32)) & 0x7FFFFFFFFFFFFFFF
            self._rng = torch.tensor([seed, 0], dtype=torch.int64, device=self.device)
            self.keep.append(self._rng)
        return self._rng

    def alloc_stats(self, Cc):
        off = self.stats_floats
        self.stats_floats += 2 * Cc * STAT_SLOTS
        return off

    def alloc_bsums(self, Cc):
        off = self.bsums_floats
        self.bsums_floats += 2 * Cc * STAT_SLOTS
        return off

    def finalize(self):
        dev = self.device
        self.stats = torch.zeros(max(self.stats_floats, 2), dtype=torch.float64, device=dev)
        self.bsums = torch.zeros(max(self.bsums_floats, 2), dtype=torch.float64, device=dev)
        self._pack_tables, self._pack_tables_late = [], []
        for w in self.weight_list:
            assert all(t == w.ntaps + w.pad_t for t in w.t_ntaps), f"plan: data gradients of one weight disagree on its tap slots ({w.t_ntaps}, pad_t {w.pad_t})"
        cut = self._late_pack_cut()
        for dtype in (torch.float32, torch.bfloat16):
            ws = [w for w in self.weight_list if w.dtype == dtype]
            if not ws:
                continue
            esz = 4 if dtype == torch.float32 else 2
            ck = 32 // esz
            total = 0
            for w in ws:
                nf = math.ceil(w.cin_used / ck) * w.ntaps * _rup(w.cout, 32) * ck
                w.fwd_off = total
                total += _rup(nf, 64)
                w.max_elems = nf
                if w.need_t:
                    nb = math.ceil(w.cout / ck) * (w.ntaps + w.pad_t) * _rup(w.cin_used, 32) * ck
                    w.bwd_off = total
                    total += _rup(nb, 64)
                    w.max_elems = max(nf, nb)
            arena = torch.zeros(total, dtype=dtype, device=dev)
            self.keep.append(arena)
            for w in ws:
                w.arena = arena
            early = [w for w in ws if cut is None or w.first_use is None or w.first_use < cut]
            late = [w for w in ws if not (cut is None or w.first_use is None or w.first_use < cut)]
            for group, dest in ((early, self._pack_tables), (late, self._pack_tables_late)):
                if not group:
                    continue
                tab = (nv.PackEntry * len(group))()
                for i, w in enumerate(group):
                    tab[i].src = (w.src if w.src is not None else w.param).data_ptr()
                    tab[i].dst = arena.data_ptr() + w.fwd_off * esz
                    tab[i].dst_t = (arena.data_ptr() + w.bwd_off * esz) if w.need_t else None
                    tab[i].Cout, tab[i].Cin, tab[i].ntaps, tab[i].pad_t = w.cout, w.cin, w.ntaps, w.pad_t
                tdev = torch.frombuffer(bytearray(bytes(tab)), dtype=torch.uint8).to(dev)
                cdt = _cdt(self, dtype)
                first = [0]
                for w in group:
                    first.append(first[-1] + nv.lib().hrp_pack_blocks(w.cout, w.cin, w.ntaps, cdt, 1, 1 if w.need_t else 0))
                fdev = torch.tensor(first, dtype=torch.int32, device=dev)
                self.keep += [tdev, fdev]
                dest.append((tdev, fdev, len(group), first[-1], cdt))
        self._pack_stream = None
        self._arena_clean = False
        if self._pack_tables_late:
            self._pack_stream = torch.cuda.Stream(device=dev)
            list.insert(self.fwd, cut, Entry(None, (), _PackJoin(self)))
        self.merged = PLAN_MODE in ("merged", "hybrid")
        if not self.merged:
            self.wgrad_ws = {lane: torch.zeros(max(nb // 4, 4), dtype=torch.float32, device=dev)
                             for lane, nb in self.wgrad_ws_bytes.items()}
        for fn in self._late:
            fn()
        self._late = []
        if FUSE_BN_REDUCE and self.need_grad:
            self._fuse_bn_reduce()
        if self.merged:
            self.fwd_run, self.bwd_run = self._flatten(self.fwd), self._flatten(self.bwd)
            if WGRAD_SINK > 1 and WGRAD_DEFER and BATCHING:
                self.bwd_run = self._sink_wgrads(self.bwd_run)
            ops = [e.op for e in self.fwd_run + self.bwd_run if e.lane is not None]
            batches = [op for op in ops if isinstance(op, BatchLaunch)]
            wg_ops = [e for e in self.bwd_run if isinstance(e.op, (Launch, BatchLaunch)) and e.op.fam == "wgrad"]
            defer = WGRAD_DEFER and bool(wg_ops)
            now = {id(e.op) for e in wg_ops if any(it.desc.reserved for it in e.op.launches())}
            if defer:
                total, ws_off = 0, {}
                for e in wg_ops:
                    op = e.op
                    for it in op.launches():
                        it.desc.phase = 0 if id(op) in now else 1
                    if isinstance(op, BatchLaunch):
                        op.ws = op.ws_query()
                    else:
                        op_need = int(nv.lib().hrp_wgrad_workspace_bytes(C.byref(op.desc)))
                        op.desc.workspace_bytes = op_need
                    sizes = op.ws if isinstance(op, BatchLaunch) else [op.desc.workspace_bytes]
                    singles = [int(nv.lib().hrp_wgrad_workspace_bytes(C.byref(it.desc))) for it in op.launches()]
                    ws_off[id(op)] = []
                    for b, b1 in zip(sizes, singles):
                        ws_off[id(op)].append((total, max(b, b1)))
                        total += _rup(max(b, b1), 256)
                self.wgrad_ws = {0: torch.zeros(max(total // 4, 4), dtype=torch.float32, device=dev)}
                base = self.wgrad_ws[0].data_ptr()
                for e in wg_ops:
                    for it, (off, b) in zip(e.op.launches(), ws_off[id(e.op)]):
                        it.desc.workspace, it.desc.workspace_bytes = (base + off, b) if b else (None, 0)
                for op in batches:
                    op.prepare()
                self.bwd_run = self._insert_folds(self.bwd_run)
            else:
                need = {}
                for e in self.fwd_run + self.bwd_run:
                    op = e.op
                    if isinstance(op, BatchLaunch) and op.fam == "wgrad":
                        op.ws = op.ws_query()
                        need[e.lane] = max(need.get(e.lane, 0), sum(_rup(b, 256) for b in op.ws))
                    elif isinstance(op, Launch) and op.fam == "wgrad":
                        need[e.lane] = max(need.get(e.lane, 0), int(nv.lib().hrp_wgrad_workspace_bytes(C.byref(op.desc))))
                self.wgrad_ws = {lane: torch.zeros(max(nb // 4, 4), dtype=torch.float32, device=dev) for lane, nb in need.items()}
                for e in self.fwd_run + self.bwd_run:
                    op = e.op
                    if isinstance(op, BatchLaunch) and op.fam == "wgrad":
                        off = 0
                        for it, b in zip(op.items, op.ws):
                            it.desc.workspace, it.desc.workspace_bytes = self.wgrad_ws[e.lane].data_ptr() + off, b
                            off += _rup(b, 256)
                    elif isinstance(op, Launch) and op.fam == "wgrad":
                        op.desc.workspace, op.desc.workspace_bytes = self.wgrad_ws[e.lane].data_ptr(), self.wgrad_ws[e.lane].numel() * 4
                for op in batches:
                    op.prepare()
                    if op.fam == "wgrad" and op.singles:
                        lane = next(e.lane for e in self.fwd_run + self.bwd_run if e.op is op)
                        for it in op.items:
                            it.desc.workspace, it.desc.workspace_bytes = self.wgrad_ws[lane].data_ptr(), self.wgrad_ws[lane].numel() * 4
            used = {e.lane for e in self.fwd_run + self.bwd_run if e.lane is not None}
            self._side_streams = [torch.cuda.Stream(device=dev) if (i + 1) in used else None for i in range(self.n_lanes - 1)]
        else:
            self._side_streams = [torch.cuda.Stream(device=dev) for _ in range(self.n_lanes - 1)]
        self._bn_tables()
        self.built = True
        if PLAN_STATS:
            import sys
            msg = f"plan: {len(self.fwd)} forward / {len(self.bwd)} backward ops, {self.n_lanes} lanes, {self.counters}"
            if self.merged:
                ops = [e.op for e in self.fwd_run + self.bwd_run if e.lane is not None]
                nb = sum(isinstance(op, BatchLaunch) and not op.singles for op in ops)
                msg += (f"; {PLAN_MODE}: {sum(e.lane is not None for e in self.fwd_run)} / {sum(e.lane is not None for e in self.bwd_run)}"
                        f" launches, {nb} of them batched, streams {sorted({e.lane for e in self.fwd_run if e.lane is not None})}")
            print(msg, file=sys.stderr)


    def _flatten(self, entries):
        from . import plan_passes
        return plan_passes.flatten(self, entries)

    def _fuse_bn_reduce(self):
        from . import plan_passes
        return plan_passes.fuse_bn_reduce(self)

    def _sink_wgrads(self, entries):
        from . import plan_passes
        return plan_passes.sink_wgrads(self, entries)

    def _insert_folds(self, entries):
        from . import plan_passes
        return plan_passes.insert_folds(self, entries)

    def analyze_backward_split(self, min_frac=0.55, fracs=None):
        from . import plan_passes
        return plan_passes.analyze_backward_split(self, min_frac, fracs)

    def _late_pack_cut(self):
        if not self.need_grad or len(self.weight_list) < 64:
            return None
        joins = [i for i, e in enumerate(self.fwd) if e.lane is None and getattr(e.op, "kind", None) == "join"]
        forks = [i for i, e in enumerate(self.fwd) if e.lane is None and getattr(e.op, "kind", None) == "fork"]
        if len(forks) < 2 or not joins or forks[1] < joins[0]:
            return None
        return joins[0] + 1

    def patch_wgrad_ws(self, g, lane):
        if lane in self.wgrad_ws:
            g.workspace, g.workspace_bytes = self.wgrad_ws[lane].data_ptr(), self.wgrad_ws[lane].numel() * 4

    def late(self, fn):
        self._late.append(fn)

    def _table(self, entries):
        tab = (nv.BnEntry * len(entries))()
        for i, e in enumerate(entries):
            for k, v in e.items():
                setattr(tab[i], k, v)
        tdev = torch.frombuffer(bytearray(bytes(tab)), dtype=torch.uint8).to(self.device)
        self.keep.append(tdev)
        return tdev, len(entries)

    def _bn_tables(self):
        self._run_tab = self._fold_tab = self._pgrad_tab = None
        if self.bn_train:
            ents = []
            for bn, off, count in self.bn_train:
                ents.append(dict(stats=self.stats.data_ptr() + 8 * off, a=bn.running_mean.data_ptr(),
                                 b=bn.running_var.data_ptr(), counter=bn.num_batches_tracked.data_ptr(),
                                 C=bn.num_features, count=float(count), momentum=bn.momentum, eps=bn.eps))
            self._run_tab = self._table(ents)
        if self.bn_fold:
            ents = []
            for bn, sc, sh in self.bn_fold.values():
                ents.append(dict(a=bn.weight.data_ptr(), b=bn.bias.data_ptr(), c=bn.running_mean.data_ptr(),
                                 d=bn.running_var.data_ptr(), out_scale=sc.data_ptr(), out_shift=sh.data_ptr(),
                                 C=bn.num_features, eps=bn.eps))
            if self.bn_fold_hat:
                cmax = max(bn.num_features for bn, _, _ in self.bn_fold_hat.values())
                ones, zeros = torch.ones(cmax, device=self.device), torch.zeros(cmax, device=self.device)
                self.keep += [ones, zeros]
                for bn, inv, nmi in self.bn_fold_hat.values():
                    ents.append(dict(a=ones.data_ptr(), b=zeros.data_ptr(), c=bn.running_mean.data_ptr(),
                                     d=bn.running_var.data_ptr(), out_scale=inv.data_ptr(), out_shift=nmi.data_ptr(),
                                     C=bn.num_features, eps=bn.eps))
            self._fold_tab = self._table(ents)
        if self.bn_bwd:
            ents = []
            for bn, off in self.bn_bwd:
                ents.append(dict(stats=self.bsums.data_ptr() + 8 * off, a=self.grad_of_param(bn.weight).data_ptr(),
                                 b=self.grad_of_param(bn.bias).data_ptr(), C=bn.num_features, accumulate=0))
            self._pgrad_tab = self._table(ents)

    def _stream(self):
        return torch.cuda.current_stream(self.device).cuda_stream

    def params_dirty(self):
        v = tuple(w.param._version for w in self.weight_list) + \
            tuple(t._version for bn, _, _ in self.bn_fold.values() for t in (bn.weight, bn.bias, bn.running_mean, bn.running_var)) + \
            (PARAM_EPOCH,)
        if v != self._versions:
            self._versions = v
            return True
        return False

    def run_prep(self, force=False):
        if not (force or self.params_dirty()):
            return
        s = self._stream()
        for op in self.pre_pack:
            op(s)
        late_s = s
        if self._pack_stream is not None and not SERIAL_LANES:
            self._pack_stream.wait_stream(torch.cuda.current_stream(self.device))
            late_s = self._pack_stream.cuda_stream
        for tdev, fdev, n, nblk, dt in self._pack_tables_late:
            nv.call("hrp_pack_weights_compact", tdev.data_ptr(), fdev.data_ptr(), n, nblk, dt, late_s)
        if late_s != s and self.need_grad and self.grad_arena is not None and ARENA_ZERO_EARLY:
            with torch.cuda.stream(self._pack_stream):
                self.grad_arena.zero_()
            self._arena_clean = True
        for tdev, fdev, n, nblk, dt in self._pack_tables:
            nv.call("hrp_pack_weights_compact", tdev.data_ptr(), fdev.data_ptr(), n, nblk, dt, s)
        if self._fold_tab:
            nv.call("hrp_bn_fold", self._fold_tab[0].data_ptr(), self._fold_tab[1], s)

    def lane_id(self, parent, index):
        key = (parent, index)
        if key not in self._lane_ids:
            self._lane_ids[key] = self.n_lanes
            self.n_lanes += 1
        return self._lane_ids[key]

    def _run_list(self, ops):
        if SERIAL_LANES:
            h = self._stream()
            for lane, _, op in ops:
                if lane is not None:
                    op(h)
            return
        streams = [torch.cuda.current_stream(self.device)] + self._side_streams
        handles = [st.cuda_stream if st is not None else None for st in streams]
        dbg = DBG_SYNC
        for lane, _, op in ops:
            if lane is None:
                op.run(streams)
                if dbg:
                    torch.cuda.synchronize(self.device)
            else:
                if dbg == "pre1" and lane == 1:
                    torch.cuda.synchronize(self.device)
                op(handles[lane])
                if dbg == "all" or (dbg == "lane1" and lane == 1) or (dbg == "lane0" and lane == 0):
                    torch.cuda.synchronize(self.device)
                elif dbg == "s1" and lane == 1:
                    streams[1].synchronize()

    def fwd_ops(self):
        return self.fwd_run if self.merged else self.fwd

    def bwd_ops(self):
        return self.bwd_run if self.merged else self.bwd

    def run_forward(self):
        global PARAM_EPOCH
        s = self._stream()
        if self._rng is not None:
            nv.call("hrp_rng_advance", self._rng.data_ptr(), s)
        if self.training and self._run_tab:
            PARAM_EPOCH += 1
        if self.stats_floats:
            self.stats.zero_()
        self._run_list(self.fwd_ops())
        if self._run_tab:
            nv.call("hrp_bn_running_update", self._run_tab[0].data_ptr(), self._run_tab[1], s)

    def run_backward(self, part=None):
        s = self._stream()
        cuts = self.bwd_cuts if self.bwd_cuts else ([self.bwd_split] if self.bwd_split is not None else [])
        if part == "first":
            part = ("seg", 0)
        if part == "rest":
            assert len(cuts) == 1, "run_backward('rest') is the two-segment form"
            part = ("seg", 1)
        j = None if part is None else part[1]
        if j in (None, 0):
            if self.grad_arena is not None and not self._arena_clean:
                self.grad_arena.zero_()
            self._arena_clean = False
            if self.bsums_floats:
                self.bsums.zero_()
        ops = self.bwd_ops()
        if j is None:
            self._run_list(ops)
        else:
            lo = 0 if j == 0 else cuts[j - 1]
            hi = cuts[j] if j < len(cuts) else None
            self._run_list(list.__getitem__(ops, slice(lo, hi)))
        if (j is None or j == len(cuts)) and self._pgrad_tab:
            nv.call("hrp_bn_param_grad", self._pgrad_tab[0].data_ptr(), self._pgrad_tab[1], s)


    def publish_param_grads(self):
        if self.accum is not None:
            views = self.accum.views
            for p, g in self.param_grads.values():
                t = views.get(id(p))
                if t is None:
                    raise RuntimeError("gradient accumulation: a parameter of this plan has no slot in the gradient arena")
                if p.grad is None or p.grad is t or getattr(p.grad, "_hrp_plan_grad", False):
                    p.grad = t
                else:
                    raise RuntimeError("gradient accumulation: a parameter carries a foreign .grad tensor (not a plan's); "
                                       "set it to None first - adding the running sum onto it would count micro-batches twice")
            return
        for p, g in self.param_grads.values():
            if p.grad is None or p.grad is g or getattr(p.grad, "_hrp_plan_grad", False):
                p.grad = g
            else:
                p.grad.add_(g)


_TAPS3 = [(ky - 1, kx - 1) for ky in range(3) for kx in range(3)]


class _BwdStack(list):

    def __init__(self, plan):
        super().__init__()
        self.plan = plan

    def append(self, fn):
        list.append(self, (self.plan.cur_lane, self.plan.lane_path, fn))


class _Parallel:
    def __init__(self, pb, block, lanes):
        self.pb, self.block, self.lanes = pb, block, lanes

    @contextlib.contextmanager
    def lane(self, i):
        p = self.pb.plan
        saved = (p.cur_lane, p.lane_path)
        p.cur_lane, p.lane_path = self.lanes[i], saved[1] + ((self.block, i),)
        try:
            yield
        finally:
            p.cur_lane, p.lane_path = saved


from .plan_blocks import BlockOps
from .plan_heads import HeadOps


class PlanBuilder(BlockOps, HeadOps):
    def __init__(self, plan):
        self.plan = plan
        self.bwd_stack = _BwdStack(plan)
        self.fuse_inference = (not plan.training) and (not plan.need_grad)

    def image_input(self, name, N, Cc, H, W, u8=False, dtype=None, lazy=False):
        p = self.plan
        t = p.new(N, H, W, Cc, dtype)
        dt = _dt(t.dtype)

        def op(s):
            x = p.dyn[name]
            if u8:
                assert x.dtype == torch.uint8
                nv.call("hrp_u8_nchw_to_nhwc", x.data_ptr(), t.ptr(), dt, N, Cc, H, W, t.pitch, 255.0, 0, s)
            else:
                nv.call("hrp_nchw_to_nhwc", x.data_ptr(), t.ptr(), dt, N, Cc, H, W, t.pitch, s)
        if lazy and LAZY_INPUTS:
            t.pending_input = op
            p.pending_inputs.append(t)
        else:
            p.fwd.append(op)
        t.external = name
        return t

    def image_input_s2d(self, name, N, Cc, H, W, u8=False):
        p = self.plan
        t = p.new(N, (H + 1) // 2, (W + 1) // 2, 4 * Cc, pitch=_rup(4 * Cc, 16))
        dt = _dt(t.dtype)

        def op(s):
            x = p.dyn[name]
            if u8:
                assert x.dtype == torch.uint8
                nv.call("hrp_u8_nchw_to_nhwc", x.data_ptr(), t.ptr(), dt, N, Cc, H, W, t.pitch, 255.0, 1, s)
            else:
                nv.call("hrp_nchw_to_nhwc_s2d", x.data_ptr(), t.ptr(), dt, N, Cc, H, W, t.pitch, s)
        p.fwd.append(op)
        t.external = name
        return t

    def stem7x7_s2d(self, xs, weight, want_stats=False):
        p = self.plan
        cout, cin = weight.shape[0], weight.shape[1]
        assert tuple(weight.shape[2:]) == (7, 7) and xs.C == 4 * cin
        dev, dtype = p.device, xs.dtype
        idx_w = torch.full((cout, 4 * cin, 16), -1, dtype=torch.int32)
        idx_g = torch.zeros((cout, cin, 49), dtype=torch.int32)
        for dy in range(2):
            for dx in range(2):
                for ty in range(4):
                    for tx in range(4):
                        ky, kx = 2 * ty + dy - 1, 2 * tx + dx - 1
                        if ky < 0 or kx < 0:
                            continue
                        for c in range(cin):
                            q = (dy * 2 + dx) * cin + c
                            for co in range(cout):
                                idx_w[co, q, ty * 4 + tx] = (co * cin + c) * 49 + ky * 7 + kx
                                idx_g[co, c, ky * 7 + kx] = (co * 4 * cin + q) * 16 + ty * 4 + tx
        idx_w, idx_g = idx_w.to(dev), idx_g.to(dev)
        w12 = torch.zeros(cout, 4 * cin, 4, 4, dtype=torch.float32, device=dev)
        gw12 = torch.zeros(cout, 4 * cin, 16, dtype=torch.float32, device=dev)
        p.keep += [idx_w, idx_g, w12, gw12]
        p.pre_pack.append(lambda s: nv.call("hrp_gather_f32", weight.data_ptr(), idx_w.data_ptr(), w12.data_ptr(),
                                            w12.numel(), 0, s))
        w = ParamW(weight, cout, 4 * cin, 16)
        w.first_use = len(p.fwd)
        w.src, w.dtype, w.cin_used, w.need_t = w12, dtype, 4 * cin, False
        p.weights[("s2d", id(weight))] = w
        p.weight_list.append(w)
        y = p.new(xs.N, xs.H, xs.W, cout, dtype)
        y.requires_grad = p.need_grad
        taps = [(ty - 2, tx - 2) for ty in range(4) for tx in range(4)]
        vec = 8 if dtype == torch.bfloat16 else 4
        d = nv.ConvDesc()
        d.x, d.y, d.dtype = xs.ptr(), y.ptr(), _cdt(p, dtype)
        d.N, d.H, d.W, d.Cin, d.x_pitch = xs.N, xs.H, xs.W, _rup(xs.C, vec), xs.pitch
        d.Ho, d.Wo, d.Cout = y.H, y.W, cout
        d.y_H, d.y_W, d.y_pitch, d.res_pitch = y.H, y.W, y.pitch, y.pitch
        d.out_stride, d.in_stride, d.ntaps, d.w_ntaps, d.w_cout_pad = 1, 1, 16, 16, _rup(cout, 32)
        for i, (a, b) in enumerate(taps):
            d.dy[i], d.dx[i], d.wtap[i] = a, b, i
        if want_stats:
            y.stats = p.alloc_stats(cout)
        esz = 4 if dtype == torch.float32 else 2

        def late():
            d.w = w.arena.data_ptr() + w.fwd_off * esz
            if y.stats is not None:
                d.stats = p.stats.data_ptr() + 8 * y.stats
        p.late(late)
        p.fwd.append(Launch("conv", d))
        y.producer = ("conv", d)
        if p.need_grad and weight.requires_grad:
            def bw():
                if not y.grad_written:
                    return
                lane = p.cur_lane
                for grp in range(4):
                    g = nv.WgradDesc()
                    g.x, g.dy, g.dw, g.dtype = xs.ptr(), y.gptr(), gw12.data_ptr(), _cdt(p, dtype)
                    g.N, g.H, g.W, g.Cin, g.x_pitch = xs.N, xs.H, xs.W, _rup(xs.C, vec), xs.pitch
                    g.Ho, g.Wo, g.Cout, g.dy_pitch = y.H, y.W, cout, y.pitch
                    g.in_stride, g.ntaps = 1, 4
                    for i in range(4):
                        g.dy_t[i], g.dx_t[i] = taps[4 * grp + i]
                    g.dw_cin, g.dw_tap_stride, g.dw_tap_off, g.accumulate = xs.C, 16, 4 * grp, 0
                    g.reserved = 1
                    p.wgrad_ws_bytes[lane] = max(p.wgrad_ws_bytes.get(lane, 0), int(nv.lib().hrp_wgrad_workspace_bytes(C.byref(g))))
                    p.late(lambda g=g, lane=lane: p.patch_wgrad_ws(g, lane))
                    p.bwd.append(Launch("wgrad", g))
                gp = p.grad_of_param(weight)
                acc = 1 if p.grad_arena is not None else 0
                p.bwd.append(lambda s: nv.call("hrp_gather_f32", gw12.data_ptr(), idx_g.data_ptr(), gp.data_ptr(),
                                               gp.numel(), acc, s))
            self.bwd_stack.append(bw)
        return y

    def maxpool3x3s2(self, x):
        p = self.plan
        x.check_readable()
        Ho, Wo = (x.H - 1) // 2 + 1, (x.W - 1) // 2 + 1
        y = p.new(x.N, Ho, Wo, x.C, x.dtype)
        y.requires_grad = p.need_grad and x.requires_grad
        arg = None
        if y.requires_grad:
            arg = torch.zeros(x.N * Ho * Wo * x.C, dtype=torch.uint8, device=p.device)
            p.keep.append(arg)
        p.fwd.append(lambda s: nv.call("hrp_maxpool3x3s2_fwd", x.ptr(), _dt(x.dtype), x.N, x.H, x.W, x.C, x.pitch, y.ptr(),
                                       y.pitch, arg.data_ptr() if arg is not None else None, s))
        if y.requires_grad:
            def bw():
                if not y.grad_written:
                    return
                acc = x.take_grad_slot()
                p.bwd.append(lambda s: nv.call("hrp_maxpool3x3s2_bwd", y.gptr(), y.pitch, arg.data_ptr(), x.gptr(), _dt(x.dtype),
                                               x.N, x.H, x.W, x.C, x.pitch, acc, s))
            self.bwd_stack.append(bw)
        return y

    @staticmethod
    def _class_taps(k, pad, py, px):
        ys = [(ky, (py + pad - ky) // 2) for ky in range(k) if (py + pad - ky) % 2 == 0]
        xs = [(kx, (px + pad - kx) // 2) for kx in range(k) if (px + pad - kx) % 2 == 0]
        return [(oy, ox, ky * k + kx) for (ky, oy) in ys for (kx, ox) in xs]

    def deconv4x4s2(self, x, weight, want_stats=False):
        p = self.plan
        x.check_readable()
        cin_t, cout_t = weight.shape[0], weight.shape[1]
        assert tuple(weight.shape[2:]) == (4, 4) and x.C == cin_t
        dtype = x.dtype
        vec = 8 if dtype == torch.bfloat16 else 4
        esz = 4 if dtype == torch.float32 else 2
        w = p.weight(weight, cin_t, cout_t, 16)
        w.dtype, w.cin_used, w.need_t = dtype, cout_t, True
        y = p.new(x.N, 2 * x.H, 2 * x.W, cout_t, dtype)
        y.requires_grad = p.need_grad
        if want_stats:
            y.stats = p.alloc_stats(cout_t)
        for (py, px) in [(0, 0), (0, 1), (1, 0), (1, 1)]:
            d = nv.ConvDesc()
            d.x, d.y, d.dtype = x.ptr(), y.ptr(), _cdt(p, dtype)
            d.N, d.H, d.W, d.Cin, d.x_pitch = x.N, x.H, x.W, _rup(x.C, vec), x.pitch
            d.Cout = cout_t
            d.y_H, d.y_W, d.y_pitch, d.res_pitch = y.H, y.W, y.pitch, y.pitch
            d.in_stride, d.out_stride, d.out_off_y, d.out_off_x = 1, 2, py, px
            d.Ho, d.Wo = (y.H - py + 1) // 2, (y.W - px + 1) // 2
            tl = self._class_taps(4, 1, py, px)
            d.ntaps = len(tl)
            for i, (a, b, t) in enumerate(tl):
                d.dy[i], d.dx[i], d.wtap[i] = a, b, t
            d.w_ntaps, d.w_cout_pad = 16, _rup(cout_t, 32)

            def late(d=d):
                d.w = w.arena.data_ptr() + w.bwd_off * esz
                if y.stats is not None:
                    d.stats = p.stats.data_ptr() + 8 * y.stats
            p.late(late)
            p.fwd.append(Launch("conv", d))
        if p.need_grad:
            self.bwd_stack.append(lambda: self._deconv_bwd(x, w, y, dtype))
        return y

    def _deconv_bwd(self, x, w, y, dtype):
        p = self.plan
        if not y.grad_written:
            return
        vec = 8 if dtype == torch.bfloat16 else 4
        esz = 4 if dtype == torch.float32 else 2
        taps = [(ky - 1, kx - 1) for ky in range(4) for kx in range(4)]
        if w.param.requires_grad:
            lane = p.cur_lane
            for grp in range(4):
                g = nv.WgradDesc()
                g.x, g.dy, g.dw, g.dtype = y.gptr(), x.ptr(), p.grad_of_param(w.param).data_ptr(), _cdt(p, dtype)
                g.N, g.H, g.W, g.Cin, g.x_pitch = y.N, y.H, y.W, _rup(y.C, vec), y.pitch
                g.Ho, g.Wo, g.Cout, g.dy_pitch = x.H, x.W, x.C, x.pitch
                g.in_stride, g.ntaps = 2, 4
                for i in range(4):
                    g.dy_t[i], g.dx_t[i] = taps[4 * grp + i]
                g.dw_cin, g.dw_tap_stride, g.dw_tap_off = y.C, 16, 4 * grp
                g.accumulate = 1 if (w.grad_written or p.grad_arena is not None) else 0
                p.wgrad_ws_bytes[lane] = max(p.wgrad_ws_bytes.get(lane, 0), int(nv.lib().hrp_wgrad_workspace_bytes(C.byref(g))))
                p.late(lambda g=g, lane=lane: p.patch_wgrad_ws(g, lane))
                p.bwd.append(Launch("wgrad", g))
            w.grad_written = True
        if x.requires_grad:
            acc = x.take_grad_slot()
            d = nv.ConvDesc()
            d.x, d.y, d.dtype = y.gptr(), x.gptr(), _cdt(p, dtype)
            d.N, d.H, d.W, d.Cin, d.x_pitch = y.N, y.H, y.W, _rup(y.C, vec), y.pitch
            d.Ho, d.Wo, d.Cout = x.H, x.W, x.C
            d.y_H, d.y_W, d.y_pitch, d.res_pitch = x.H, x.W, x.pitch, x.pitch
            d.out_stride, d.in_stride, d.ntaps, d.w_ntaps, d.w_cout_pad = 1, 2, 16, 16, _rup(x.C, 32)
# ... 536 lines not shown
```

holistic-robot-pose-estimation_amd/runtime.py:

```python
import os

import torch
import torch.nn as nn

from . import _native as nv
from .plan import GradAccumulation, Plan, PlanBuilder, _dt


def require_gpu(device):
    if device.type != "cuda":
        raise nv.HrpError("hrpe_amd runs on an MI355X (gfx950) only: tensors must live on a HIP device; "
                          "there is no CPU path")
    nv.lib()


GRAPH_CACHE = not os.environ.get("HRP_NO_MODULE_GRAPH")
PLAN_CACHE_MAX = int(os.environ.get("HRP_PLAN_CACHE", "6"))
GRAPH_WARMUP = 2


class Runner:

    def __init__(self, plan, in_names, outs, img_inputs):
        self.plan, self.in_names, self.outs, self.img_inputs = plan, in_names, outs, img_inputs
        self.calls = self.bwd_calls = 0
        self.g_fwd = self.g_bwd = self.static_in = None
        self.graph_failed = False

    def _forward_launches(self, prep=True):
        p = self.plan
        if prep or p.need_grad:
            p.run_prep(force=p.need_grad)
        p.run_forward()

    def _results(self):
        p = self.plan
        res = [None] * len(self.outs)
        dense = [(i, h, shape) for i, (kind, h, shape) in enumerate(self.outs) if kind != "nchw" and h.dtype == torch.float32]
        if len(dense) > 1:
            flat = torch.empty(sum(h.N * h.C for _, h, _ in dense), dtype=torch.float32, device=p.device)
            items, off = [], 0
            for i, h, shape in dense:
                items.append((h.ptr(), h.pitch, flat.data_ptr() + 4 * off, h.C, h.N, h.C, 0))
                res[i] = flat[off:off + h.N * h.C].view(shape)
                off += h.N * h.C
            nv.copy_cols_batch(items, torch.cuda.current_stream(p.device).cuda_stream)
        for i, (kind, h, shape) in enumerate(self.outs):
            if res[i] is not None:
                continue
            if kind == "nchw":
                res[i] = h["out"].clone() if self.g_fwd is not None else h["out"]
            else:
                res[i] = h.buf.view(-1)[h.offset: h.offset + h.N * h.pitch].view(h.N, h.pitch)[:, : h.C].reshape(shape).clone()
        return tuple(res)

    def _graphs_allowed(self):
        p = self.plan
        return (GRAPH_CACHE and not self.graph_failed and not p.split_active and not torch.cuda.is_current_stream_capturing()
                and not nv.profiling())

    def _capture(self, what):
        p = self.plan
        try:
            g = torch.cuda.CUDAGraph()
            pool = self.g_fwd.pool() if self.g_fwd is not None else None
            with torch.cuda.graph(g, pool=pool, capture_error_mode="thread_local"):
                if what == "fwd":
                    self._forward_launches(prep=False)
                else:
                    p._arena_clean = False
                    p.run_backward(None)
            return g
        except Exception as e:
            import sys
            print(f"hrpe_amd: graph capture of the {what} plan failed ({e!r}); running it eagerly", file=sys.stderr)
            self.graph_failed = True
            return None

    def forward(self, tensors):
        p = self.plan
        self.calls += 1
        if self._graphs_allowed() and self.calls > GRAPH_WARMUP:
            if self.g_fwd is None:
                self.static_in = [torch.empty_like(t) for t in tensors]
                for n, st in zip(self.in_names, self.static_in):
                    p.dyn[n] = st
                self.g_fwd = self._capture("fwd")
            if self.g_fwd is not None and p.need_grad and self.g_bwd is None and self.bwd_calls >= GRAPH_WARMUP:
                self.g_bwd = self._capture("bwd")
        if self.g_fwd is not None and self._graphs_allowed():
            for st, t in zip(self.static_in, tensors):
                st.copy_(t)
            if not p.need_grad:
                p.run_prep(force=False)
            self.g_fwd.replay()
            if p.training and p._run_tab:
                from .plan import bump_param_epoch
                bump_param_epoch()
            return self._results()
        for n, t in zip(self.in_names, tensors):
            p.dyn[n] = t
        self._forward_launches()
        return self._results()

    def backward(self, grads):
        p = self.plan
        s = torch.cuda.current_stream(p.device).cuda_stream
        items, keep = [], []
        for (kind, h, shape), g in zip(self.outs, grads):
            t = h["handle"] if kind == "nchw" else h
            if not (t.requires_grad and t.grad_written):
                continue
            gb = t.grad_buf()
            if kind != "nchw" and t.dtype == torch.float32:
                if g is not None:
                    g = g.reshape(t.N, t.C)
                    if g.dtype != torch.float32 or not g.is_contiguous():
                        g = g.contiguous().float()
                    keep.append(g)
                items.append((None if g is None else g.data_ptr(), t.C, t.gptr(), t.pitch, t.N, t.C, 0))
            elif g is None:
                gb.zero_()
            elif kind == "nchw":
                g = g.contiguous().float()
                nv.call("hrp_nchw_to_nhwc", g.data_ptr(), t.gptr(), _dt(t.dtype), t.N, t.C, t.H, t.W, t.pitch, s)
            else:
                gb.view(t.N, t.pitch)[:, : t.C].copy_(g.reshape(t.N, t.C))
        if items:
            nv.copy_cols_batch(items, s)
        self.bwd_calls += 1
        if self.g_bwd is not None and self._graphs_allowed():
            self.g_bwd.replay()
        else:
            p.run_backward("first" if p.split_active else None)
        if p.accum is not None:
            p.accum.accumulate(p, s)
        p.publish_param_grads()
        gin = []
        for n in self.in_names:
            t = self.img_inputs.get(n)
            if t is not None and t.requires_grad and t.grad_written:
                out = torch.empty(t.N, t.C, t.H, t.W, dtype=torch.float32, device=p.device)
                nv.call("hrp_nhwc_to_nchw", t.gptr(), out.data_ptr(), _dt(t.dtype), t.N, t.C, t.H, t.W, t.pitch, s)
                gin.append(out)
            else:
                gin.append(None)
        return gin


class _PlanFn(torch.autograd.Function):
    @staticmethod
    def forward(ctx, runner, anchor, *tensors):
        ctx.runner = runner
        ctx.n = len(tensors)
        outs = runner.forward(tensors)
        return outs

    @staticmethod
    def backward(ctx, *grads):
        gin = ctx.runner.backward(grads)
        return (None, None) + tuple(gin)


MODE_EPOCH = [0]


class PlannedModule(nn.Module):

    def train(self, mode=True):
        MODE_EPOCH[0] += 1
        return super().train(mode)

    def __init__(self):
        super().__init__()
        object.__setattr__(self, "_plans", {})
        object.__setattr__(self, "_bn_sig", (-1, []))
        object.__setattr__(self, "_compute_dtype", torch.float32)
        object.__setattr__(self, "_x3", False)
        object.__setattr__(self, "_accum", None)

    def set_compute_dtype(self, dtype):
        x3 = dtype == "fp32x3"
        if x3:
            dtype = torch.float32
        assert dtype in (torch.float32, torch.bfloat16)
        for m in self.modules():
            if isinstance(m, PlannedModule):
                object.__setattr__(m, "_compute_dtype", dtype)
                object.__setattr__(m, "_x3", x3)
                m._plans.clear()
        return self

    @property
    def compute_dtype(self):
        return self._compute_dtype

    def flat_grads(self):
        if self._accum is not None:
            return [self._accum.buf] if self._accum.buf is not None else []
        return [r.plan.grad_arena for r in self._plans.values() if r.plan.grad_arena is not None]

    def set_grad_accumulation(self, steps, average=False):
        if isinstance(steps, bool) or not isinstance(steps, int) or steps < 1:
            raise ValueError(f"set_grad_accumulation: steps must be an integer >= 1 (got {steps!r})")
        mods = [m for m in self.modules() if isinstance(m, PlannedModule)]
        if steps > 1 and any(r.plan.split_active for m in mods for r in m._plans.values()):
            raise ValueError("set_grad_accumulation(steps > 1) cannot be combined with enable_split_backward(): the overlapped "
                             "all-reduce hands out arena ranges of a single backward; call disable_split_backward() first")
        for m in mods:
            acc = GradAccumulation(steps, bool(average)) if steps > 1 else None
            object.__setattr__(m, "_accum", acc)
            for r in m._plans.values():
                r.plan.accum = acc if r.plan.need_grad else None
        return self

    def begin_accumulation(self):
        for m in self.modules():
            if isinstance(m, PlannedModule) and m._accum is not None:
                m._accum.begin()
        return self

    def accumulation_complete(self):
        return self._accum is None or self._accum.complete()

    def enable_split_backward(self, min_frac=0.55, fracs=None):
        if self._accum is not None:
            raise ValueError("enable_split_backward() cannot be combined with set_grad_accumulation(steps > 1): the ranges it hands "
                             "out are final for ONE backward, not for the accumulated sum; call set_grad_accumulation(1) first")
        runners = [r for r in self._plans.values() if r.plan.grad_arena is not None]
        if len(runners) != 1:
            return None
        plan = runners[0].plan
        if fracs is not None:
            cuts = plan.analyze_backward_split(fracs=fracs)
            if not cuts:
                return None
            plan.bwd_cuts, plan.bwd_split = [c for c, _ in cuts], None
            plan.split_active = True
            return plan, [r for _, r in cuts]
        info = plan.analyze_backward_split(min_frac)
        if info is None:
            return None
        plan.bwd_split, ranges = info
        plan.bwd_cuts = None
        plan.split_active = True
        return plan, ranges

    def check_split_backward(self, ranges):
        runners = [r for r in self._plans.values() if r.plan.grad_arena is not None and r.plan.split_active]
        if len(runners) != 1:
            raise RuntimeError("check_split_backward: no plan with an active split")
        plan = runners[0].plan
        arena = plan.grad_arena
        multi = plan.bwd_cuts is not None
        groups = ranges if multi else [ranges]
        nseg = len(plan.bwd_cuts) + 1 if multi else 2
        snaps = []
        ok = True
        for j in range(1, nseg):
            torch.cuda.synchronize(arena.device)
            grp = groups[j - 1]
            snaps.append((grp, torch.cat([arena[o:o + n] for o, n in grp]).clone() if grp else arena[:0].clone()))
            plan.run_backward(("seg", j))
            torch.cuda.synchronize(arena.device)
            for grp_, before in snaps:
                after = torch.cat([arena[o:o + n] for o, n in grp_]) if grp_ else arena[:0]
                ok = ok and torch.equal(before, after)
        ok = ok and bool(torch.isfinite(arena).all())
        if not ok:
            self.disable_split_backward()
            raise RuntimeError("split backward self-check failed: a later part of the backward touched gradient ranges "
                               "that were final after an earlier one")
        return True

    def disable_split_backward(self):
        for r in self._plans.values():
            r.plan.split_active = False

    def invalidate_plans(self):
        for m in self.modules():
            if isinstance(m, PlannedModule):
                m._plans.clear()
                if m._accum is not None:
                    object.__setattr__(m, "_accum", GradAccumulation(m._accum.steps, m._accum.scale != 1.0))

    def _apply(self, fn, *a, **k):
        r = super()._apply(fn, *a, **k)
        self.invalidate_plans()
        return r

    def load_state_dict(self, *a, **k):
        r = super().load_state_dict(*a, **k)
        for m in self.modules():
            if isinstance(m, PlannedModule):
                for pl in m._plans.values():
                    pl.plan._versions = None
        return r

    def _frozen_bn_signature(self):
        if self._bn_sig[0] != MODE_EPOCH[0]:
            object.__setattr__(self, "_bn_sig", (MODE_EPOCH[0], [m for m in self.modules() if hasattr(m, "running_mean")]))
        sig = 0
        if self.training:
            for i, m in enumerate(self._bn_sig[1]):
                if not m.training:
                    sig |= 1 << i
        return sig

    def _run(self, *tensors):
        dev = tensors[0].device
        require_gpu(dev)
        need_grad = torch.is_grad_enabled() and (any(p.requires_grad for p in self.parameters())
                                                 or any(t.requires_grad for t in tensors))
        bn_eval = self._frozen_bn_signature()
        key = (tuple(tuple(t.shape) for t in tensors), self._compute_dtype, self.training, need_grad,
               tuple(bool(t.requires_grad) for t in tensors) if need_grad else (),
               tuple(t.dtype == torch.uint8 for t in tensors), bn_eval, self._x3)
        runner = self._plans.pop(key, None)
        if runner is not None:
            self._plans[key] = runner
        if runner is None:
            while len(self._plans) >= PLAN_CACHE_MAX:
                self._plans.pop(next(iter(self._plans)))
            plan = Plan(dev, self._compute_dtype, self.training, need_grad)
            plan.x3 = bool(self._x3)
            if need_grad:
                plan.preallocate_param_grads(list(self.parameters()))
                plan.accum = self._accum
            pb = PlanBuilder(plan)
            in_names, outs, img_inputs = self._build(pb, *tensors)
            for kind, h, shape in outs:
                t = h["handle"] if kind == "nchw" else h
                pb.output(t)
            pb.finish()
            runner = Runner(plan, in_names, outs, img_inputs)
            self._plans[key] = runner
        tensors = tuple(t.contiguous() if t.dtype == torch.uint8 else
                        (t.contiguous().float() if t.dtype != torch.float32 or not t.is_contiguous() else t)
                        for t in tensors)
        if need_grad:
            anchor = next((p for p in self.parameters() if p.requires_grad), None)
            if anchor is None:
                anchor = tensors[0]
            return _PlanFn.apply(runner, anchor, *tensors)
        return runner.forward(tensors)


class SingleTensorModule(PlannedModule):

    def forward(self, x):
        return self._run(x)[0]

    def _build(self, pb, x):
        N, Cc, H, W = x.shape
        t = pb.image_input("x", N, Cc, H, W, u8=x.dtype == torch.uint8)
        t.requires_grad = pb.plan.need_grad and x.requires_grad
        y = self.emit(pb, t)
        holder = pb.nchw_output(y)
        holder["handle"] = y
        return ["x"], [("nchw", holder, None)], {"x": t}
```

include/hrp.h:

```cpp
#ifndef HRP_H
#define HRP_H

#include <stdint.h>

#ifdef __cplusplus
extern "C" {
#endif

typedef enum { HRP_F32 = 0, HRP_BF16 = 1, HRP_F32X3 = 2 } hrp_dtype;

typedef enum {
  HRP_OK = 0,
  HRP_ERR_ARG = -1,
  HRP_ERR_LAUNCH = -2,
  HRP_ERR_NODEV = -3
} hrp_status;

#define HRP_MAX_TAPS 16

#define HRP_STAT_SLOTS 8

typedef struct hrp_conv_desc {
  const void* x;
  const void* w;
  void* y;
  const void* res;
  const float* bias;
  const float* scale;
  const float* shift;
  double* stats;
  int32_t dtype;
  int32_t N, H, W, Cin, x_pitch;
  int32_t Ho, Wo, Cout;
  int32_t y_H, y_W, y_pitch, res_pitch;
  int32_t out_stride, out_off_y, out_off_x;
  int32_t in_stride;
  int32_t ntaps;
  int32_t dy[HRP_MAX_TAPS], dx[HRP_MAX_TAPS];
  int32_t wtap[HRP_MAX_TAPS];
  int32_t w_ntaps;
  int32_t w_cout_pad;
  int32_t relu;
  const void* bnb_x;
  const uint8_t* bnb_mask;
  const float* bnb_consts;
  int32_t bnb_x_pitch, bnb_mask_pitch;
  const double* bnb_stats;
  const float* bnb_gamma;
  const float* bnb_beta;
  float bnb_count, bnb_eps;
  int32_t pro_mode, pro_reserved;
  const void* pro_x2;
  const double* pro_stats;
  const double* pro_bsums;
  const float* pro_gamma;
  const float* pro_beta;
  float pro_count, pro_eps;
  void* pro_side;
  const uint8_t* pro_mask;
  void* pro_side2;
  int32_t pro_side2_acc, pro_reserved2;
  const uint8_t* res_mask;
  int32_t tail_mode, tail_side_acc;
  const double* tail_stats;
  const double* tail_bsums;
  const float* tail_gamma;
  const float* tail_beta;
  float tail_count, tail_eps;
  uint8_t* tail_mask;
  const void* tail_g;
  void* tail_side;
  const void* tail_x2;
  const void* tail_w2;
  const double* tail_stats2;
  const float* tail_gamma2;
  const float* tail_beta2;
} hrp_conv_desc;

typedef struct hrp_wgrad_desc {
  const void* x;
  const void* dy;
  float* dw;
  int32_t dtype;
  int32_t N, H, W, Cin, x_pitch;
  int32_t Ho, Wo, Cout, dy_pitch;
  int32_t in_stride, ntaps;
  int32_t dy_t[HRP_MAX_TAPS], dx_t[HRP_MAX_TAPS];
  int32_t dw_cin;
  int32_t dw_tap_stride;
  int32_t dw_tap_off;
  int32_t accumulate;
  void* workspace;
  int64_t workspace_bytes;
  int32_t phase;
  int32_t reserved;
} hrp_wgrad_desc;

typedef struct hrp_wgrad_fold_desc {
  const float* workspace;
  float* dw;
  int32_t G, pairs, n_cib, nte, nb;
  int32_t Cout, dw_cin, ntaps, dw_tap_stride, dw_tap_off, accumulate;
  int32_t reserved;
} hrp_wgrad_fold_desc;

typedef struct hrp_pack_entry {
  const float* src;
  void* dst;
  void* dst_t;
  int32_t Cout, Cin, ntaps;
  int32_t pad_t;
} hrp_pack_entry;

#define HRP_EW_MAX_IN 4
typedef enum { HRP_EW_IDENTITY = 0, HRP_EW_AFFINE = 1, HRP_EW_BN_TRAIN = 2 } hrp_ew_mode;

typedef struct hrp_ew_input {
  const void* ptr;
  int32_t pitch;
  int32_t up;
  int32_t mode;
  const float* a;
  const float* b;
  const double* stats;
  float count;
  float eps;
} hrp_ew_input;

typedef struct hrp_ew_desc {
  hrp_ew_input in[HRP_EW_MAX_IN];
  int32_t nin;
  void* out;
  int32_t out_pitch;
  int32_t dtype;
  int32_t N, H, W, C;
  int32_t relu;
  uint8_t* mask;
  int32_t mask_pitch;
  float* consts_out;
} hrp_ew_desc;

typedef struct hrp_ew_bwd_desc {
  const void* dout;
  const void* out;
  int32_t dout_pitch, out_pitch;
  hrp_ew_input in;
  void* din;
  int32_t din_pitch;
  double* sums;
  int32_t dtype;
  int32_t N, H, W, C;
  int32_t relu;
  int32_t accumulate;
  const uint8_t* mask;
  int32_t mask_pitch;
  void* din2;
  int32_t din2_pitch;
  int32_t accumulate2;
  const float* pooled;
} hrp_ew_bwd_desc;

typedef struct hrp_bn_entry {
  const double* stats;
  float* a;
  float* b;
  const float* c;
  const float* d;
  float* out_scale;
  float* out_shift;
  int64_t* counter;
  int32_t C;
  float count, momentum, eps;
  int32_t accumulate;
} hrp_bn_entry;

#define HRP_FK_MAX_JOINTS 32
#define HRP_FK_MAX_KP 24
typedef struct hrp_fk_chain {
  int32_t njoints;
  int32_t parent[HRP_FK_MAX_JOINTS];
  int32_t type[HRP_FK_MAX_JOINTS];
  int32_t cfg[HRP_FK_MAX_JOINTS];
  float mimic_mul[HRP_FK_MAX_JOINTS], mimic_off[HRP_FK_MAX_JOINTS];
  float origin[HRP_FK_MAX_JOINTS][12];
  float axis[HRP_FK_MAX_JOINTS][3];
  int32_t nkp;
  int32_t kp_frame[HRP_FK_MAX_KP];
  float kp_offset[HRP_FK_MAX_KP][3];
  int32_t dof;
} hrp_fk_chain;

const char* hrp_last_error(void);
int hrp_version(void);
const char* hrp_source_hash(void);
int hrp_device_ok(void);

int hrp_nchw_to_nhwc(const float* src, void* dst, int dtype, int N, int C, int H, int W, int dst_pitch, void* stream);
int hrp_nhwc_to_nchw(const void* src, float* dst, int dtype, int N, int C, int H, int W, int src_pitch, void* stream);
int hrp_nchw_grad_from_nhwc(const void* src, float* dst, int dtype, int N, int C, int H, int W, int src_pitch, void* stream);
int hrp_u8_nchw_to_nhwc(const uint8_t* src, void* dst, int dtype, int N, int C, int H, int W, int dst_pitch,
                        float divisor, int s2d, void* stream);
int hrp_pack_weights(const hrp_pack_entry* table_dev, int count, int dtype, int max_elems, void* stream);
int hrp_pack_blocks(int Cout, int Cin, int ntaps, int dtype, int has_dst, int has_dst_t);
int hrp_pack_weights_compact(const hrp_pack_entry* table_dev, const int32_t* first_block_dev, int count, int total_blocks,
                             int dtype, void* stream);
int hrp_nchw_to_nhwc_s2d(const float* src, void* dst, int dtype, int N, int C, int H, int W, int dst_pitch, void* stream);
int hrp_gather_f32(const float* src, const int32_t* idx, float* dst, int n, int accumulate, void* stream);
int hrp_fill_zero(void* p, int64_t bytes, void* stream);
int hrp_maxpool3x3s2_fwd(const void* x, int dtype, int N, int H, int W, int C, int pitch, void* y, int y_pitch,
                         uint8_t* argmax, void* stream);
int hrp_maxpool3x3s2_bwd(const void* dy, int dy_pitch, const uint8_t* argmax, void* dx, int dtype, int N, int H, int W,
                         int C, int pitch, int accumulate, void* stream);

int hrp_conv2d_fwd(const hrp_conv_desc* d, void* stream);
int hrp_conv_rowstrip_channels(const hrp_conv_desc* d);
int hrp_conv_pointwise(const hrp_conv_desc* d);
int hrp_conv2d_bwd_weight(const hrp_wgrad_desc* d, void* stream);
int64_t hrp_wgrad_workspace_bytes(const hrp_wgrad_desc* d);
int64_t hrp_colsum_workspace_bytes(int64_t rows, int C);
int hrp_colsum(const void* x, int dtype, int64_t rows, int C, int pitch, float* out, int accumulate, void* workspace,
               int64_t workspace_bytes, void* stream);

#define HRP_OPT_CHUNK 4096
typedef struct hrp_opt_tensor {
  float* param;
  float* grad;
  float* exp_avg;
  float* exp_avg_sq;
  int64_t numel;
} hrp_opt_tensor;
typedef struct hrp_opt_chunk {
  int32_t tensor;
  int32_t offset;
} hrp_opt_chunk;
int hrp_opt_grad_sumsq(const hrp_opt_tensor* tensors_dev, const hrp_opt_chunk* chunks_dev, int nchunks,
                       float* sumsq_slots, float* chunk_sums, void* stream);
int hrp_opt_adam_step(const hrp_opt_tensor* tensors_dev, const hrp_opt_chunk* chunks_dev, int nchunks,
                      const float* sumsq_slots, float max_norm, const float* step_dev,
                      float lr, float beta1, float beta2, float eps, void* stream);
typedef struct hrp_opt_group {
  float lr, beta1, beta2, eps;
  float weight_decay;
  float reserved[3];
} hrp_opt_group;
int hrp_opt_adam_step_groups(const hrp_opt_tensor* tensors_dev, const hrp_opt_chunk* chunks_dev, int nchunks,
                             const float* sumsq_slots, float max_norm, const float* step_dev,
                             const hrp_opt_group* groups_dev, int ngroups, const int32_t* tensor_group_dev, void* stream);
int hrp_opt_set_group(hrp_opt_group* groups_dev, int ngroups, int index, float lr, float beta1, float beta2, float eps,
                      float weight_decay, void* stream);
int hrp_grad_accumulate(const float* src, float* acc, int64_t n, int first, float scale, void* stream);

int hrp_ew_fwd(const hrp_ew_desc* d, void* stream);
int hrp_ew_bwd_reduce(const hrp_ew_bwd_desc* d, void* stream);
int hrp_ew_pool2(const void* src, int src_dtype, int src_pitch, const uint8_t* mask, int mask_pitch, int N, int H, int W, int C, float* dst,
                 void* stream);
int hrp_ew_bwd_apply(const hrp_ew_bwd_desc* d, void* stream);

typedef enum {
  HRP_BATCH_CONV = 0, HRP_BATCH_WGRAD = 1, HRP_BATCH_EW_FWD = 2, HRP_BATCH_EW_BWD_REDUCE = 3, HRP_BATCH_EW_BWD_APPLY = 4,
  HRP_BATCH_WGRAD_FOLD = 5
} hrp_batch_family;
#define HRP_BATCH_MAX 32
typedef struct hrp_batch_info {
  int32_t family, n, dtype;
  int32_t variant;
  int32_t grid, lds_bytes;
  int32_t grid2;
  int32_t grid3, lds_bytes3;
  int32_t blk0[HRP_BATCH_MAX + 1];
  int32_t blk2[HRP_BATCH_MAX + 1];
  int64_t ws_bytes[HRP_BATCH_MAX];
} hrp_batch_info;
int64_t hrp_batch_table_bytes(int family, int n);
int hrp_batch_prepare(int family, const void* descs, int n, void* table_host, hrp_batch_info* info);
int hrp_batch_launch(const void* table_dev, const hrp_batch_info* info, void* stream);
int hrp_wgrad_fold_desc_of(const hrp_wgrad_desc* d, hrp_wgrad_fold_desc* out);
int hrp_batch_wgrad_fold_descs(const void* table_host, const hrp_batch_info* info, hrp_wgrad_fold_desc* out);

#define HRP_PIL_KMAX 12
int hrp_pil_resize_table(int in_size, int out_size, int32_t* out);
int hrp_pil_resize_normalize(const void* src, int src_u8, int N, int H, int W, const int32_t* xtab_dev, const int32_t* ytab_dev,
                             int Ho, int Wo, void* dst, int dtype, int dst_pitch, int s2d, const float* mean3, const float* std3,
                             void* stream);
int hrp_broadcast_hw(const float* src, int src_pitch, void* dst, int dtype, int N, int HW, int C, int dst_pitch, void* stream);
int hrp_bilinear_nhwc_to_nchw(const void* src, int dtype, int N, int h, int w, int C, int pitch, float* dst, int H, int W, int act,
                              void* stream);

#define HRP_BLOCK_MAX 2
typedef struct hrp_block_desc {
  hrp_conv_desc conv1, conv2;
} hrp_block_desc;
typedef struct hrp_block_info {
  int32_t n, grid, lds_bytes, reserved;
  int32_t first_wg[HRP_BLOCK_MAX];
  int32_t bands[HRP_BLOCK_MAX];
} hrp_block_info;
int hrp_block_channels(const hrp_block_desc* d);
int64_t hrp_block_table_bytes(void);
int hrp_block_prepare(const hrp_block_desc* descs, int n, void* table, hrp_block_info* info);
int hrp_block_launch(const void* table, const hrp_block_info* info, void* stream);

int hrp_bn_running_update(const hrp_bn_entry* table_dev, int count, void* stream);
int hrp_bn_fold(const hrp_bn_entry* table_dev, int count, void* stream);
int hrp_bn_param_grad(const hrp_bn_entry* table_dev, int count, void* stream);

int hrp_avgpool_fwd(const void* x, int dtype, int N, int HW, int C, int pitch, float* out, int out_pitch, void* stream);
int hrp_avgpool_bwd(const float* dout, int dout_pitch, void* dx, int dtype, int N, int HW, int C, int pitch, int accumulate, void* stream);

int hrp_softargmax3d_fwd(const void* logits, int dtype, int B, int J, int D, int H, int W, int pitch,
                         int root, int fix_root, float* uvd, float* ms, void* stream);
int hrp_softargmax3d_bwd(const void* logits, int dtype, int B, int J, int D, int H, int W, int pitch,
                         int root, int fix_root, const float* uvd, const float* ms, const float* duvd,
                         void* dlogits, int dpitch, void* stream);

int hrp_pose_geometry_fwd(const float* gamma, const float* k_value, const float* uvd, const float* K,
                          int B, int J, int root, float image_size, float depth_factor,
                          float* depth, float* xyz, float* root_uv, float* trans, void* stream);
int hrp_pose_geometry_bwd(const float* gamma, const float* k_value, const float* uvd, const float* K,
                          int B, int J, int root, float image_size, float depth_factor,
                          const float* d_depth, const float* d_xyz, const float* d_root_uv, const float* d_trans,
                          float* d_gamma, float* d_uvd, void* stream);

int hrp_softargmax_flat_fwd(const void* logits, int dtype, int B, int J, int HW, int pitch, float* coord, float* ms, void* stream);
int hrp_softargmax_flat_bwd(const void* logits, int dtype, int B, int J, int HW, int pitch, const float* coord, const float* ms,
                            const float* dcoord, void* dlogits, int dpitch, void* stream);

int hrp_rot6d_compose_fwd(const float* a, const float* b, float* out, int N, void* stream);
int hrp_rot6d_compose_bwd(const float* a, const float* b, const float* dout, float* da, float* db, int N, int acc_a, int acc_b,
                          void* stream);

int hrp_fk_project_fwd(const hrp_fk_chain* chain_dev, const float* q, const float* rot6d, const float* trans,
                       const float* K, int B, int root, float* xyz, float* uv, float* root_rot6d, void* stream);
typedef struct hrp_silhouette_desc {
  const float* uv;
  const float* xyz;
  const int32_t* faces;
  int32_t B, V, F, H, W;
  float sigma, blur_radius;
  float* alpha;
  int64_t* logp;
  int32_t* count;
} hrp_silhouette_desc;
int hrp_silhouette_fwd(const hrp_silhouette_desc* d, void* stream);
int hrp_silhouette_bwd(const hrp_silhouette_desc* d, const float* d_alpha, float* d_uv, void* stream);

int hrp_mesh_pose(const hrp_fk_chain* chain_dev, const float* q, const float* rot6d, const float* trans, int B, int root_kp,
                  const float* verts, const uint8_t* vert_link, int V, const float* K, float* xyz, float* uv, void* stream);
int hrp_mesh_pose_bwd(const hrp_fk_chain* chain_dev, const float* q, const float* rot6d, const float* trans, int B, int root_kp,
                      const float* verts, const uint8_t* vert_link, int V, const float* d_xyz, float* d_rot6d, float* d_trans, void* stream);
int hrp_fk_project_bwd(const hrp_fk_chain* chain_dev, const float* q, const float* rot6d, const float* trans,
                       const float* K, int B, int root, const float* d_xyz, const float* d_uv,
                       float* d_q, float* d_rot6d, float* d_trans, void* stream);
int hrp_fk_project_rot_fwd(const hrp_fk_chain* chain_dev, const float* q, const float* rot, int rot_dim, const float* trans,
                           const float* K, int B, int root, float* xyz, float* uv, float* root_rot, void* stream);
int hrp_fk_project_rot_bwd(const hrp_fk_chain* chain_dev, const float* q, const float* rot, int rot_dim, const float* trans,
                           const float* K, int B, int root, const float* d_xyz, const float* d_uv,
                           float* d_q, float* d_rot, float* d_trans, void* stream);

int hrp_copy_cols(const float* src, int src_pitch, float* dst, int dst_pitch, int rows, int cols, int accumulate, void* stream);
#define HRP_COPY_MAX 16
typedef struct hrp_copy_desc {
  const float* src;
  float* dst;
  int src_pitch, dst_pitch, rows, cols;
  int accumulate, reserved;
} hrp_copy_desc;
int hrp_copy_cols_batch(const hrp_copy_desc* descs, int n, void* stream);
int hrp_scale_rows(float* x, int pitch, int rows, int cols, const float* row_scale, float s, void* stream);
int hrp_mul_f32(const float* x, int x_pitch, const float* m, int m_pitch, float* y, int y_pitch, int rows, int cols,
                int accumulate, void* stream);
int64_t hrp_linear_workspace_bytes(int M, int K, int N);
int hrp_linear_fwd(const float* x, int x_pitch, const float* w, const float* bias, const float* res, int res_pitch,
                   float* y, int y_pitch, int M, int K, int N, void* workspace, int64_t workspace_bytes, void* stream);
int hrp_linear_bwd_data(const float* dy, int dy_pitch, const float* w, float* dx, int dx_pitch, int M, int K, int N,
                        int accumulate, void* workspace, int64_t workspace_bytes, void* stream);
int hrp_linear_bwd_weight(const float* x, int x_pitch, const float* dy, int dy_pitch, float* dw, float* dbias, int M, int K,
                          int N, int accumulate, void* stream);

typedef struct hrp_pose_loss_desc {
  const float *pose, *rot, *trans, *root_uv, *depth, *xyz_int, *xyz_fk;
  const float *gt_pose, *gt_root_rot, *gt_root_trans, *gt_root_uv;
  const float *gt_kp3d, *gt_kp2d, *mask, *K;
  float *d_pose, *d_rot, *d_trans, *d_root_uv, *d_depth, *d_xyz_int, *d_xyz_fk;
  float* out;
  float weights[10];
  int32_t B, P, J, root;
  float image_size;
  int32_t rot_dim;
} hrp_pose_loss_desc;
int hrp_pose_loss(const hrp_pose_loss_desc* d, void* stream);
int hrp_l1_loss(const float* pred, const float* gt, float scale, int n, float* loss, float* d_pred, void* stream);

typedef struct hrp_sim2real_loss_desc {
  const float* rendered;
  const float* seg;
  const float* kp3d;
  const float* kp3d_int;
  int32_t B, HW, K, mask_loss;
  float w_mask, w_iou, w_scale, w_align;
  float* terms;
  float* d_rendered;
  float* d_kp3d;
  float* d_kp3d_int;
  float* workspace;
} hrp_sim2real_loss_desc;
int hrp_sim2real_loss(const hrp_sim2real_loss_desc* d, void* stream);

int hrp_rng_advance(uint64_t* state_dev, void* stream);
int hrp_dropout_f32(const float* x, int x_pitch, float* y, int y_pitch, float* mask, int rows, int cols, float keep,
                    const uint64_t* state_dev, uint32_t salt, void* stream);
int hrp_dropout_masks(float* masks, int64_t n, float keep, const uint64_t* state_dev, uint32_t salt, void* stream);

#define HRP_REG_MAX_P 16
#define HRP_REG_MAX_PROBLEMS 4
typedef struct hrp_regressor_step_desc {
  int32_t M, P, K, N;
  const float* u_prev;
  const float* u_bias;
  const float* z;
  const float* zw;
  int32_t z_len, z_pitch, zw_sk, zw_sp;
  float* u_out;
  const float* a;
  const float* a_mask;
  const float* v;
  int32_t a_pitch, v_sk, v_sp, a2_pitch;
  float* a_out;
  const float* w;
  const float* bias;
  const float* out_mask;
  const float* a2;
  const float* w2;
  int64_t w_sn, w_sk;
  int32_t out_pitch, out_accumulate, out_sum_accumulate;
  int32_t w2_sk;
  float* out;
  float* out_sum;
} hrp_regressor_step_desc;
int hrp_regressor_step(const hrp_regressor_step_desc* descs, int n, void* stream);

#define HRP_LIN_WGRAD_MAX 8
typedef struct hrp_linear_wgrad_desc {
  const float* x;
  const float* dy;
  float* dw;
  float* dbias;
  int32_t x_pitch, dy_pitch, dw_ld, M, K, N, accumulate, reserved;
} hrp_linear_wgrad_desc;
int hrp_linear_wgrad_batch(const hrp_linear_wgrad_desc* descs, int n, void* stream);

int hrp_project_fwd(const float* K, const float* pts, int B, int P, float* uv, void* stream);
int hrp_project_bwd(const float* K, const float* pts, const float* duv, int B, int P, float* dpts, void* stream);

int hrp_pnp_solve(const float* pts2d, const float* pts3d, int pts3d_stride, const float* K, int K_stride, const float* ini_pose,
                  int B, int n, float* P6d, int* status, float* rms, void* stream);
int hrp_pnp_bwd(const float* pts2d, const float* pts3d, int pts3d_stride, const float* K, int K_stride, const float* P6d,
                const float* grad_out, int B, int n, int fast, float* grad_x, float* grad_z, float* grad_K, float* grad_z_sum,
                float* grad_K_sum, int* status, void* stream);

#define HRP_DREAM_BANDS 32
enum {
  HRP_DREAM_JITTER = 1, HRP_DREAM_OCCLUSION = 2, HRP_DREAM_SHARPNESS = 4, HRP_DREAM_CONTRAST = 8, HRP_DREAM_BRIGHTNESS = 16,
  HRP_DREAM_COLOR = 32
};
typedef struct {
  double jitter[3];
  double enh[4];
  int32_t flags;
  int32_t occ_x, occ_y, occ_w, occ_h;
  int32_t pad_x, pad_y, work_w, work_h;
  int32_t crop_x0, crop_y0, crop_x1, crop_y1;
  int32_t off_x, off_y, side;
  int32_t reserved;
  int64_t noise_off;
  int64_t scratch_off;
} hrp_dream_sample;
int hrp_dream_augment(const uint8_t* frames, int B, int H, int W, const hrp_dream_sample* table_dev, const uint8_t* noise,
                      int64_t noise_bytes, int max_h, int max_w, uint8_t* scratch, int64_t scratch_bytes, uint64_t* lsum, void* stream);
int hrp_dream_crop_resize(const uint8_t* scratch, int64_t scratch_bytes, const hrp_dream_sample* table_dev, const uint64_t* lsum, int B,
                          int max_h, int max_w, uint8_t* out0, int h0, int w0, uint8_t* out1, int h1, int w1, void* stream);

typedef struct hrp_eval_desc {
  const float* pred_kp3d_fk;
  const float* pred_kp3d_int;
  const float* gt_kp3d;
  const float* gt_kp2d;
  const float* K;
  const float* pred_joint;
  const float* gt_joint;
  const float* pred_rot;
  const float* gt_rot;
  float *error3d, *error2d, *mean_jointerror, *error_depth, *batch_error_relative, *error3d_relative;
  float *error3d_int, *error2d_int, *error_depth_int, *batch_error_relative_int, *error3d_relative_int;
  float *dis3d, *dis2d, *dis3d_int, *dis2d_int;
  float* l1_jointerror;
  float* rotation_diff;
  int32_t B, nkp, dof;
  int32_t rot_dim;
  int32_t root;
  int32_t drop_last_joint;
  int32_t offset, capacity;
  int32_t batch_index, batch_capacity;
} hrp_eval_desc;
int hrp_eval_batch(const hrp_eval_desc* d, void* stream);

#define HRP_DEPTH_LOSS_MAX_KP 16
enum { HRP_DEPTH_LOSS_L1 = 0, HRP_DEPTH_LOSS_MSE = 1 };
enum { HRP_XY_LOSS_NONE = 0, HRP_XY_LOSS_L1 = 1, HRP_XY_LOSS_MSE = 2 };
typedef struct hrp_depth_loss_desc {
  const float* pred;
  const float* gt_root_trans;
  const float* gt_kp3d;
  const float* mask;
  float* loss;
  float* d_pred;
  float* errors;
  float* losses;
  int32_t B, W, J, nk;
  int32_t kp_index[HRP_DEPTH_LOSS_MAX_KP];
  int32_t depth_loss, xy_loss;
  int32_t root_col;
  int32_t want_grad;
  int32_t offset, capacity;
  int32_t batch_index, batch_capacity;
} hrp_depth_loss_desc;
int hrp_depth_loss(const hrp_depth_loss_desc* d, void* stream);

#ifdef __cplusplus
}
#endif
#endif
```

Measured before the change: 2046 images/sec.

## Fuse Adam update with conv weight packing and skip forward repack when clean

Adds a kernel that applies the clipped Adam update to conv weights tile by tile and writes the packed compute-dtype weights (and transposed copies) directly from the updated values in LDS. This removes the separate pack pass the forward used to run over every weight after each optimizer step. Weight version tracking lets the forward skip repacking when the optimizer already produced packed copies. The cost is extra bookkeeping for staleness (version tuples, plan retirement, load_state_dict hooks), a risk of stale packed weights if parameters change outside the optimizer, and a slightly changed Adam arithmetic order (explicit fma, contraction off).

```diff
diff --git a/holistic-robot-pose-estimation_amd/_native.py b/holistic-robot-pose-estimation_amd/_native.py
--- a/holistic-robot-pose-estimation_amd/_native.py
+++ b/holistic-robot-pose-estimation_amd/_native.py
@@ -169,6 +169,7 @@
 
 
 OPT_CHUNK = 4096
+PACK_TILE_TAPS = 9
 
 
 class OptTensor(C.Structure):
@@ -183,6 +184,13 @@
 class OptGroup(C.Structure):
     _fields_ = [("lr", C.c_float), ("beta1", C.c_float), ("beta2", C.c_float), ("eps", C.c_float),
                 ("weight_decay", C.c_float), ("reserved", C.c_float * 3)]
+
+
+class OptPackEntry(C.Structure):
+    _fields_ = [("param", C.c_void_p), ("dst", C.c_void_p), ("dst_t", C.c_void_p),
+                ("Cout", C.c_int32), ("Cin", C.c_int32), ("ntaps", C.c_int32), ("pad_t", C.c_int32),
+                ("grad", C.c_void_p), ("exp_avg", C.c_void_p), ("exp_avg_sq", C.c_void_p),
+                ("group", C.c_int32), ("reserved", C.c_int32)]
 
 
 class RegStepDesc(C.Structure):
@@ -289,6 +297,7 @@
     "hrp_opt_grad_sumsq": [_P, _P, _I, _P, _P, _P],
     "hrp_opt_adam_step": [_P, _P, _I, _P, _F, _P, _F, _F, _F, _F, _P],
     "hrp_opt_adam_step_groups": [_P, _P, _I, _P, _F, _P, _P, _I, _P, _P],
+    "hrp_opt_adam_pack_step": [_P, _P, _I, _I, _I, _P, _F, _P, _F, _F, _F, _F, _P, _I, _P],
     "hrp_opt_set_group": [_P, _I, _I, _F, _F, _F, _F, _F, _P],
     "hrp_grad_accumulate": [_P, _P, _L, _I, _F, _P],
     "hrp_batch_prepare": [_I, _P, _I, _P, C.POINTER(BatchInfo)],
diff --git a/holistic-robot-pose-estimation_amd/csrc/core.hip b/holistic-robot-pose-estimation_amd/csrc/core.hip
--- a/holistic-robot-pose-estimation_amd/csrc/core.hip
+++ b/holistic-robot-pose-estimation_amd/csrc/core.hip
@@ -244,32 +244,38 @@
   }
 }
 
+__device__ __forceinline__ bool pack_tile_origin(const hrp_pack_entry& e, const unsigned tile_id, unsigned& co0, unsigned& ci0) {
+  const unsigned n_cot = ((unsigned)e.Cout + 31) / 32, n_cit = ((unsigned)e.Cin + 31) / 32;
+  if (tile_id >= n_cot * n_cit) return false;
+  co0 = (tile_id / n_cit) * 32, ci0 = (tile_id % n_cit) * 32;
+  return true;
+}
+
+__device__ __forceinline__ void pack_tile_load(const hrp_pack_entry& e, const unsigned co0, const unsigned ci0, float* __restrict__ lds) {
+  const unsigned Cout = e.Cout, Cin = e.Cin, nt = e.ntaps;
+  const unsigned span = 32 * nt, pitch = span + 1;
+  const unsigned wave = threadIdx.x >> 6, lane = threadIdx.x & 63;
+  const unsigned valid = Cin > ci0 ? (Cin - ci0 < 32 ? (Cin - ci0) * nt : span) : 0;
+  for (unsigned r0 = wave; r0 < 32; r0 += 16) {
+    for (unsigned j = lane; j < span; j += 64) {
+      float v[4];
+#pragma unroll
+      for (int u = 0; u < 4; ++u) {
+        const unsigned co = co0 + r0 + 4 * u;
+        v[u] = (co < Cout && j < valid) ? e.src[((size_t)co * Cin + ci0) * nt + j] : 0.f;
+      }
+#pragma unroll
+      for (int u = 0; u < 4; ++u) lds[(r0 + 4 * u) * pitch + j] = v[u];
+    }
+  }
+}
+
 template <typename T>
-__device__ __forceinline__ void pack_entry_tile(const hrp_pack_entry& e, const unsigned tile_id, float* __restrict__ lds) {
+__device__ __forceinline__ void pack_tile_store(const hrp_pack_entry& e, const unsigned co0, const unsigned ci0, const float* __restrict__ lds) {
   constexpr int CK = 32 / Elem<T>::SZ, NC = 32 / CK;
   const unsigned Cout = e.Cout, Cin = e.Cin, nt = e.ntaps;
   const unsigned cout_pad = (Cout + 31) / 32 * 32, cin_pad = (Cin + 31) / 32 * 32;
-  const unsigned n_cit = cin_pad / 32;
-  if (tile_id >= (cout_pad / 32) * n_cit) return;
-  const unsigned co0 = (tile_id / n_cit) * 32, ci0 = (tile_id % n_cit) * 32;
-  const unsigned span = 32 * nt, pitch = span + 1;
-  {
-    const unsigned wave = threadIdx.x >> 6, lane = threadIdx.x & 63;
-    const unsigned valid = Cin > ci0 ? (Cin - ci0 < 32 ? (Cin - ci0) * nt : span) : 0;
-    for (unsigned r0 = wave; r0 < 32; r0 += 16) {
-      for (unsigned j = lane; j < span; j += 64) {
-        float v[4];
-#pragma unroll
-        for (int u = 0; u < 4; ++u) {
-          const unsigned co = co0 + r0 + 4 * u;
-          v[u] = (co < Cout && j < valid) ? e.src[((size_t)co * Cin + ci0) * nt + j] : 0.f;
-        }
-#pragma unroll
-        for (int u = 0; u < 4; ++u) lds[(r0 + 4 * u) * pitch + j] = v[u];
-      }
-    }
-  }
-  __syncthreads();
+  const unsigned pitch = 32 * nt + 1;
   if (e.dst) {
     const unsigned nch = (Cin + CK - 1) / CK;
     for (unsigned r = threadIdx.x; r < NC * nt * 32; r += 256) {
@@ -292,6 +298,15 @@
       pack_store_row<T>(e.dst_t, (size_t)(ch * (nt + e.pad_t) + tap) * cin_pad + ci0 + ci, v);
     }
   }
+}
+
+template <typename T>
+__device__ __forceinline__ void pack_entry_tile(const hrp_pack_entry& e, const unsigned tile_id, float* __restrict__ lds) {
+  unsigned co0, ci0;
+  if (!pack_tile_origin(e, tile_id, co0, ci0)) return;
+  pack_tile_load(e, co0, ci0, lds);
+  __syncthreads();
+  pack_tile_store<T>(e, co0, ci0, lds);
 }
 
 constexpr int PACK_ROWS_PER_BLOCK = 256 * 4;
@@ -718,6 +733,36 @@
   if (threadIdx.x < HRP_STAT_SLOTS) slots[threadIdx.x] = threadIdx.x == 0 ? part[0] : 0.f;
 }
 
+struct opt_adam_coef { float clip, step_size, inv_sqrt_bc2; };
+__device__ __forceinline__ opt_adam_coef opt_adam_prepare(const float* __restrict__ slots, float max_norm,
+                                                          const float* __restrict__ step_dev, float lr, float b1, float b2) {
+  opt_adam_coef k;
+  k.clip = 1.f;
+  if (max_norm > 0.f) {
+    float ss = 0.f;
+#pragma unroll
+    for (int i = 0; i < HRP_STAT_SLOTS; ++i) ss += slots[i];
+    k.clip = fminf(1.f, max_norm / (sqrtf(ss) + 1e-6f));
+  }
+  const float step = *step_dev;
+  const float bc1 = 1.f - powf(b1, step), bc2 = 1.f - powf(b2, step);
+  k.step_size = lr / bc1, k.inv_sqrt_bc2 = 1.f / sqrtf(bc2);
+  return k;
+}
+template <bool WD>
+__device__ __forceinline__ void opt_adam_update(float& pp, float& gg, float& mm, float& vv, const opt_adam_coef& k, float b1, float b2,
+                                                float eps, float wd) {
+#pragma clang fp contract(off)
+  gg = gg * k.clip;
+  float ge = gg;
+  if constexpr (WD) ge = fmaf(wd, pp, gg);
+  const float m_old = b1 * mm, v_old = b2 * vv, ge2 = (1.f - b2) * ge;
+  mm = fmaf(1.f - b1, ge, m_old);
+  vv = fmaf(ge, ge2, v_old);
+  const float num = k.step_size * mm;
+  pp = pp - num / fmaf(sqrtf(vv), k.inv_sqrt_bc2, eps);
+}
+
 template <bool DECAY>
 __device__ __forceinline__ void opt_adam_chunk(const hrp_opt_tensor t, const hrp_opt_chunk ck, const float* __restrict__ slots,
                                                float max_norm, const float* __restrict__ step_dev, float lr, float b1, float b2,
@@ -725,32 +770,14 @@
   const int64_t base = (int64_t)ck.offset * HRP_OPT_CHUNK;
   const int64_t left = t.numel - base;
   const int n = left < HRP_OPT_CHUNK ? (int)left : HRP_OPT_CHUNK;
-  float clip = 1.f;
-  if (max_norm > 0.f) {
-    float ss = 0.f;
-#pragma unroll
-    for (int k = 0; k < HRP_STAT_SLOTS; ++k) ss += slots[k];
-    clip = fminf(1.f, max_norm / (sqrtf(ss) + 1e-6f));
-  }
-  const float step = *step_dev;
-  const float bc1 = 1.f - powf(b1, step), bc2 = 1.f - powf(b2, step);
-  const float step_size = lr / bc1, inv_sqrt_bc2 = 1.f / sqrtf(bc2);
+  const opt_adam_coef k = opt_adam_prepare(slots, max_norm, step_dev, lr, b1, b2);
   float* p = t.param + base;
   float* g = t.grad + base;
   float* m = t.exp_avg + base;
   float* v = t.exp_avg_sq + base;
   auto run = [&](auto with_decay) {
     auto upd = [&](float& pp, float& gg, float& mm, float& vv) {
-      gg *= clip;
-      if constexpr (decltype(with_decay)::value) {
-        const float ge = gg + wd * pp;
-        mm = b1 * mm + (1.f - b1) * ge;
-        vv = b2 * vv + (1.f - b2) * ge * ge;
-      } else {
-        mm = b1 * mm + (1.f - b1) * gg;
-        vv = b2 * vv + (1.f - b2) * gg * gg;
-      }
-      pp -= step_size * mm / (sqrtf(vv) * inv_sqrt_bc2 + eps);
+      opt_adam_update<decltype(with_decay)::value>(pp, gg, mm, vv, k, b1, b2, eps, wd);
     };
     if ((n & 3) == 0 && (((uintptr_t)p | (uintptr_t)g | (uintptr_t)m | (uintptr_t)v) & 15) == 0) {
       for (int i = threadIdx.x * 4; i < n; i += 1024) {
@@ -793,6 +820,95 @@
   hrp_opt_group h = {};
   h.lr = lr, h.beta1 = b1, h.beta2 = b2, h.eps = eps, h.weight_decay = wd;
   groups[index] = h;
+}
+
+template <int W, bool WD>
+__device__ __forceinline__ void opt_adam_tile(const hrp_opt_pack_entry& e, const unsigned co0, const unsigned ci0, const opt_adam_coef& k,
+                                              float b1, float b2, float eps, float wd, float* __restrict__ lds) {
+  constexpr int U = 3;
+  const unsigned Cout = e.Cout, Cin = e.Cin, nt = e.ntaps;
+  const unsigned span = 32 * nt, pitch = span + 1, per_row = span / W, items = 32 * per_row;
+  const unsigned valid = Cin > ci0 ? (Cin - ci0 < 32 ? (Cin - ci0) * nt : span) : 0;
+  for (unsigned i0 = threadIdx.x; i0 < items; i0 += U * 256) {
+    float pp[U][W], gg[U][W], mm[U][W], vv[U][W];
+    size_t off[U];
+    unsigned at[U];
+    bool live[U], in[U];
+#pragma unroll
+    for (int u = 0; u < U; ++u) {
+      const unsigned i = i0 + u * 256, r = i / per_row, j = (i % per_row) * W;
+      live[u] = i < items;
+      in[u] = live[u] && co0 + r < Cout && j < valid;
+      at[u] = r * pitch + j;
+      off[u] = in[u] ? ((size_t)(co0 + r) * Cin + ci0) * nt + j : 0;
+      {
+        if constexpr (W == 4) {
+          const float4 a = *(const float4*)(e.param + off[u]), b = *(const float4*)(e.grad + off[u]);
+          const float4 c = *(const float4*)(e.exp_avg + off[u]), d = *(const float4*)(e.exp_avg_sq + off[u]);
+          pp[u][0] = a.x, pp[u][1] = a.y, pp[u][2] = a.z, pp[u][3] = a.w;
+          gg[u][0] = b.x, gg[u][1] = b.y, gg[u][2] = b.z, gg[u][3] = b.w;
+          mm[u][0] = c.x, mm[u][1] = c.y, mm[u][2] = c.z, mm[u][3] = c.w;
+          vv[u][0] = d.x, vv[u][1] = d.y, vv[u][2] = d.z, vv[u][3] = d.w;
+        } else {
+          pp[u][0] = e.param[off[u]], gg[u][0] = e.grad[off[u]], mm[u][0] = e.exp_avg[off[u]], vv[u][0] = e.exp_avg_sq[off[u]];
+        }
+      }
+    }
+#pragma unroll
+    for (int u = 0; u < U; ++u) {
+      if (in[u]) {
+#pragma unroll
+        for (int x = 0; x < W; ++x) opt_adam_update<WD>(pp[u][x], gg[u][x], mm[u][x], vv[u][x], k, b1, b2, eps, wd);
+        if constexpr (W == 4) {
+          *(float4*)(e.param + off[u]) = make_float4(pp[u][0], pp[u][1], pp[u][2], pp[u][3]);
+          *(float4*)(e.grad + off[u]) = make_float4(gg[u][0], gg[u][1], gg[u][2], gg[u][3]);
+          *(float4*)(e.exp_avg + off[u]) = make_float4(mm[u][0], mm[u][1], mm[u][2], mm[u][3]);
+          *(float4*)(e.exp_avg_sq + off[u]) = make_float4(vv[u][0], vv[u][1], vv[u][2], vv[u][3]);
+        } else {
+          e.param[off[u]] = pp[u][0], e.grad[off[u]] = gg[u][0], e.exp_avg[off[u]] = mm[u][0], e.exp_avg_sq[off[u]] = vv[u][0];
+        }
+      }
+      if (live[u]) {
+#pragma unroll
+        for (int x = 0; x < W; ++x) lds[at[u] + x] = in[u] ? pp[u][x] : 0.f;
+      }
+    }
+  }
+}
+
+template <typename T, bool GROUPS>
+__global__ __launch_bounds__(256) void opt_adam_pack_kernel(const hrp_opt_pack_entry* __restrict__ table, const int32_t* __restrict__ first,
+                                                            const int count, const float* __restrict__ slots, float max_norm,
+                                                            const float* __restrict__ step_dev, float lr, float b1, float b2, float eps,
+                                                            const hrp_opt_group* __restrict__ groups, int ngroups) {
+  __shared__ float lds[32 * (32 * PACK_TILE_TAPS + 1)];
+  int lo = 0, hi = count;
+  while (hi - lo > 1) {
+    const int mid = (lo + hi) >> 1;
+    if (first[mid] <= (int)blockIdx.x) lo = mid; else hi = mid;
+  }
+  const hrp_opt_pack_entry e = table[lo];
+  hrp_pack_entry pe;
+  pe.src = e.param, pe.dst = e.dst, pe.dst_t = e.dst_t, pe.Cout = e.Cout, pe.Cin = e.Cin, pe.ntaps = e.ntaps, pe.pad_t = e.pad_t;
+  unsigned co0, ci0;
+  if (e.ntaps > PACK_TILE_TAPS || !pack_tile_origin(pe, blockIdx.x - first[lo], co0, ci0)) return;
+  float wd = 0.f;
+  if constexpr (GROUPS) {
+    const hrp_opt_group h = groups[e.group < 0 ? 0 : e.group >= ngroups ? ngroups - 1 : e.group];
+    lr = h.lr, b1 = h.beta1, b2 = h.beta2, eps = h.eps, wd = h.weight_decay;
+  }
+  const opt_adam_coef k = opt_adam_prepare(slots, max_norm, step_dev, lr, b1, b2);
+  const bool vec = (((unsigned)e.Cin * (unsigned)e.ntaps) & 3) == 0 &&
+                   (((uintptr_t)e.param | (uintptr_t)e.grad | (uintptr_t)e.exp_avg | (uintptr_t)e.exp_avg_sq) & 15) == 0;
+  if (GROUPS && wd != 0.f) {
+    if (vec) opt_adam_tile<4, true>(e, co0, ci0, k, b1, b2, eps, wd, lds);
+    else opt_adam_tile<1, true>(e, co0, ci0, k, b1, b2, eps, wd, lds);
+  } else {
+    if (vec) opt_adam_tile<4, false>(e, co0, ci0, k, b1, b2, eps, 0.f, lds);
+    else opt_adam_tile<1, false>(e, co0, ci0, k, b1, b2, eps, 0.f, lds);
+  }
+  __syncthreads();
+  pack_tile_store<T>(pe, co0, ci0, lds);
 }
 
 extern "C" int hrp_opt_grad_sumsq(const hrp_opt_tensor* tensors_dev, const hrp_opt_chunk* chunks_dev, int nchunks,
@@ -825,6 +941,28 @@
   hipLaunchKernelGGL(opt_adam_groups_kernel, dim3(nchunks), dim3(256), 0, (hipStream_t)stream, tensors_dev, chunks_dev,
                      sumsq_slots, max_norm, step_dev, groups_dev, ngroups, tensor_group_dev);
   return check_launch("opt_adam_step_groups");
+}
+extern "C" int hrp_opt_adam_pack_step(const hrp_opt_pack_entry* table_dev, const int32_t* first_block_dev, int count, int total_blocks,
+                                      int dtype, const float* sumsq_slots, float max_norm, const float* step_dev, float lr, float beta1,
+                                      float beta2, float eps, const hrp_opt_group* groups_dev, int ngroups, void* stream) {
+  HRP_REQUIRE(table_dev && first_block_dev && count > 0 && total_blocks >= count, "opt_adam_pack_step: empty table / fewer workgroups than entries");
+  HRP_REQUIRE(dtype == HRP_F32 || dtype == HRP_BF16 || dtype == HRP_F32X3, "opt_adam_pack_step: dtype %d", dtype);
+  HRP_REQUIRE(step_dev, "opt_adam_pack_step: null step counter");
+  HRP_REQUIRE(max_norm <= 0.f || sumsq_slots, "opt_adam_pack_step: clipping needs the sum-of-squares slots");
+  HRP_REQUIRE(!groups_dev || ngroups >= 1, "opt_adam_pack_step: ngroups %d < 1", ngroups);
+  const dim3 grid(total_blocks);
+#define HRP_LAUNCH_ADAM_PACK(T)                                                                                                       \
+  do {                                                                                                                                \
+    if (groups_dev) hipLaunchKernelGGL((opt_adam_pack_kernel<T, true>), grid, dim3(256), 0, (hipStream_t)stream, table_dev,           \
+                                       first_block_dev, count, sumsq_slots, max_norm, step_dev, 0.f, 0.f, 0.f, 0.f, groups_dev, ngroups); \
+    else hipLaunchKernelGGL((opt_adam_pack_kernel<T, false>), grid, dim3(256), 0, (hipStream_t)stream, table_dev, first_block_dev,    \
+                            count, sumsq_slots, max_norm, step_dev, lr, beta1, beta2, eps, (const hrp_opt_group*)nullptr, 0);         \
+  } while (0)
+  if (dtype == HRP_F32) HRP_LAUNCH_ADAM_PACK(float);
+  else if (dtype == HRP_F32X3) HRP_LAUNCH_ADAM_PACK(f32x3_t);
+  else HRP_LAUNCH_ADAM_PACK(bf16_t);
+#undef HRP_LAUNCH_ADAM_PACK
+  return check_launch("opt_adam_pack_step");
 }
 extern "C" int hrp_opt_set_group(hrp_opt_group* groups_dev, int ngroups, int index, float lr, float beta1, float beta2, float eps,
                                  float weight_decay, void* stream) {
diff --git a/holistic-robot-pose-estimation_amd/optim.py b/holistic-robot-pose-estimation_amd/optim.py
--- a/holistic-robot-pose-estimation_amd/optim.py
+++ b/holistic-robot-pose-estimation_amd/optim.py
@@ -1,8 +1,38 @@
 import ctypes as C
+import os
 
 import torch
 
 from . import _native as nv
+
+ADAM_PACK = os.environ.get("HRP_ADAM_PACK", "1") not in ("0", "")
+
+
+def fused_owners(params):
+    from . import plan as PL
+    out = []
+    for p in params:
+        pl = PL.packing_plan(p) if ADAM_PACK else None
+        fw = pl.fused_weight(p) if pl is not None else None
+        out.append(None if fw is None else (pl, fw[0], fw[1]))
+    return out
+
+
+def split_tables(numels, fused):
+    chunks, adam_chunks, tiles = [], [], {}
+    for i, (n, f) in enumerate(zip(numels, fused)):
+        mine = [(i, k) for k in range((n + nv.OPT_CHUNK - 1) // nv.OPT_CHUNK)]
+        chunks += mine
+        if f is None:
+            adam_chunks += mine
+            continue
+        cout, cin, ntaps, cdt, need_t = f
+        if cout * cin * ntaps != n or ntaps > nv.PACK_TILE_TAPS:
+            raise ValueError("FusedClipAdam: a packed weight's shape disagrees with its parameter")
+        rows = tiles.setdefault(cdt, [])
+        first = rows[-1][1] + rows[-1][2] if rows else 0
+        rows.append((i, first, nv.lib().hrp_pack_blocks(cout, cin, ntaps, cdt, 1, 1 if need_t else 0)))
+    return chunks, adam_chunks, tiles
 
 
 class FusedClipAdam(torch.optim.Optimizer):
@@ -46,9 +76,10 @@
         self._publish_state()
         self._slots = torch.zeros(8, dtype=torch.float32, device=dev)
         self._chunk_sums = None
-        self._grad_ptrs = None
-        self._tensors = self._chunks = None
-        self._nchunks = 0
+        self._grad_ptrs = self._owner_key = self._owner_epoch = None
+        self._tensors = self._chunks = self._adam_chunks = None
+        self._nchunks = self._n_adam_chunks = 0
+        self._fused, self._fused_host, self._owner_plans = [], {}, []
         if self._device_hyper:
             ng = len(self.param_groups)
             self._groups = torch.zeros(ng * C.sizeof(nv.OptGroup) // 4, dtype=torch.float32, device=dev)
@@ -116,27 +147,70 @@
             g["capturable"] = True
         self._publish_state()
 
+    def _owners(self):
+        return fused_owners(self.params)
+
     def _build_tables(self):
+        from . import plan as PL
         ptrs = tuple(p.grad.data_ptr() for p in self.params)
-        if ptrs == self._grad_ptrs:
+        if ptrs == self._grad_ptrs and self._owner_epoch == PL.OWNER_EPOCH:
+            return
+        owners = self._owners()
+        okey = tuple(None if o is None else (id(o[0]), o[1].arena.data_ptr(), o[1].fwd_off, o[1].bwd_off, o[2]) for o in owners)
+        self._owner_epoch = PL.OWNER_EPOCH
+        if ptrs == self._grad_ptrs and okey == self._owner_key:
             return
         tab = (nv.OptTensor * len(self.params))()
-        chunks = []
         for i, (p, (m, v)) in enumerate(zip(self.params, self.state_views)):
             g = p.grad
             if g.dtype != torch.float32 or not g.is_contiguous():
                 raise ValueError("FusedClipAdam: gradients must be contiguous fp32")
             tab[i].param, tab[i].grad, tab[i].exp_avg, tab[i].exp_avg_sq = p.data_ptr(), g.data_ptr(), m.data_ptr(), v.data_ptr()
             tab[i].numel = p.numel()
-            chunks += [(i, k) for k in range((p.numel() + nv.OPT_CHUNK - 1) // nv.OPT_CHUNK)]
-        ck = (nv.OptChunk * len(chunks))()
-        for j, (i, k) in enumerate(chunks):
-            ck[j].tensor, ck[j].offset = i, k
+        chunks, adam_chunks, tiles = split_tables(
+            [p.numel() for p in self.params],
+            [None if o is None else (o[1].cout, o[1].cin, o[1].ntaps, o[2], o[1].need_t) for o in owners])
+
+        def chunk_table(items):
+            ck = (nv.OptChunk * max(len(items), 1))()
+            for j, (i, k) in enumerate(items):
+                ck[j].tensor, ck[j].offset = i, k
+            return torch.frombuffer(bytearray(bytes(ck)), dtype=torch.uint8).to(self.device)
+
         self._tensors = torch.frombuffer(bytearray(bytes(tab)), dtype=torch.uint8).to(self.device)
-        self._chunks = torch.frombuffer(bytearray(bytes(ck)), dtype=torch.uint8).to(self.device)
+        self._chunks = chunk_table(chunks)
         self._nchunks = len(chunks)
+        self._adam_chunks = self._chunks if not tiles else chunk_table(adam_chunks)
+        self._n_adam_chunks = len(adam_chunks)
+        self._fused = []
+        self._fused_host = tiles
+        group_of = self._param_groups_index() if self._device_hyper else None
+        for cdt, rows in sorted(tiles.items()):
+            ft = (nv.OptPackEntry * len(rows))()
+            esz = 2 if cdt == nv.HRP_BF16 else 4
+            for j, (i, _, _) in enumerate(rows):
+                w = owners[i][1]
+                ft[j].param, ft[j].grad, ft[j].exp_avg, ft[j].exp_avg_sq = tab[i].param, tab[i].grad, tab[i].exp_avg, tab[i].exp_avg_sq
+                ft[j].dst = w.arena.data_ptr() + w.fwd_off * esz
+                ft[j].dst_t = (w.arena.data_ptr() + w.bwd_off * esz) if w.need_t else None
+                ft[j].Cout, ft[j].Cin, ft[j].ntaps, ft[j].pad_t = w.cout, w.cin, w.ntaps, w.pad_t
+                ft[j].group = group_of[i] if group_of is not None else 0
+            first = [r[1] for r in rows] + [rows[-1][1] + rows[-1][2]]
+            self._fused.append((torch.frombuffer(bytearray(bytes(ft)), dtype=torch.uint8).to(self.device),
+                                torch.tensor(first, dtype=torch.int32, device=self.device), len(rows), first[-1], cdt))
+        plans = {}
+        for o in owners:
+            if o is not None:
+                plans[id(o[0])] = o[0]
+        self._owner_plans = []
+        for pl in plans.values():
+            whole = all(o is not None and o[0] is pl for p, o in zip(self.params, owners) if pl.fused_weight(p) is not None)
+            self._owner_plans.append((pl, whole))
         self._chunk_sums = torch.zeros(self._nchunks, dtype=torch.float32, device=self.device)
-        self._grad_ptrs = ptrs
+        self._grad_ptrs, self._owner_key = ptrs, okey
+
+    def _param_groups_index(self):
+        return [i for i, g in enumerate(self.param_groups) for _ in g["params"]]
 
     def prepare(self):
         if any(p.grad is None for p in self.params):
@@ -160,16 +234,27 @@
         if self.max_norm > 0:
             nv.call("hrp_opt_grad_sumsq", self._tensors.data_ptr(), self._chunks.data_ptr(), self._nchunks,
                     self._slots.data_ptr(), self._chunk_sums.data_ptr(), s)
-        if self._device_hyper:
-            nv.call("hrp_opt_adam_step_groups", self._tensors.data_ptr(), self._chunks.data_ptr(), self._nchunks,
-                    self._slots.data_ptr(), self.max_norm, self.step_count.data_ptr(),
-                    self._groups.data_ptr(), len(self.param_groups), self._tensor_group.data_ptr(), s)
-        else:
-            nv.call("hrp_opt_adam_step", self._tensors.data_ptr(), self._chunks.data_ptr(), self._nchunks,
-                    self._slots.data_ptr(), self.max_norm, self.step_count.data_ptr(),
-                    float(g["lr"]), float(g["betas"][0]), float(g["betas"][1]), float(g["eps"]), s)
+        clean = [pl for pl, whole in self._owner_plans if whole and not pl.weights_dirty()]
+        hyper = (float(g["lr"]), float(g["betas"][0]), float(g["betas"][1]), float(g["eps"]))
+        if self._n_adam_chunks:
+            if self._device_hyper:
+                nv.call("hrp_opt_adam_step_groups", self._tensors.data_ptr(), self._adam_chunks.data_ptr(), self._n_adam_chunks,
+                        self._slots.data_ptr(), self.max_norm, self.step_count.data_ptr(),
+                        self._groups.data_ptr(), len(self.param_groups), self._tensor_group.data_ptr(), s)
+            else:
+                nv.call("hrp_opt_adam_step", self._tensors.data_ptr(), self._adam_chunks.data_ptr(), self._n_adam_chunks,
+                        self._slots.data_ptr(), self.max_norm, self.step_count.data_ptr(), *hyper, s)
+        for tdev, fdev, n, nblk, cdt in self._fused:
+            if self._device_hyper:
+                nv.call("hrp_opt_adam_pack_step", tdev.data_ptr(), fdev.data_ptr(), n, nblk, cdt, self._slots.data_ptr(), self.max_norm,
+                        self.step_count.data_ptr(), 0.0, 0.0, 0.0, 0.0, self._groups.data_ptr(), len(self.param_groups), s)
+            else:
+                nv.call("hrp_opt_adam_pack_step", tdev.data_ptr(), fdev.data_ptr(), n, nblk, cdt, self._slots.data_ptr(), self.max_norm,
+                        self.step_count.data_ptr(), *hyper, None, 0, s)
         from .plan import bump_param_epoch
         bump_param_epoch()
+        for pl in clean:
+            pl.mark_packed()
 
     def total_norm(self):
         return self._slots.sum().sqrt()
diff --git a/holistic-robot-pose-estimation_amd/parallel.py b/holistic-robot-pose-estimation_amd/parallel.py
--- a/holistic-robot-pose-estimation_amd/parallel.py
+++ b/holistic-robot-pose-estimation_amd/parallel.py
@@ -32,6 +32,8 @@
         return
     for t in list(module.parameters()) + list(module.buffers()):
         dist.broadcast(t.data, src=src)
+    from .plan import bump_param_epoch
+    bump_param_epoch()
 
 
 class GradAllReducer:
diff --git a/holistic-robot-pose-estimation_amd/plan.py b/holistic-robot-pose-estimation_amd/plan.py
--- a/holistic-robot-pose-estimation_amd/plan.py
+++ b/holistic-robot-pose-estimation_amd/plan.py
@@ -3,6 +3,7 @@
 import ctypes as C
 import math
 import os
+import weakref
 
 import torch
 
@@ -151,12 +152,62 @@
 MAX_TILE_DILATION = 4
 
 PARAM_EPOCH = 0
+WEIGHT_EPOCH = 0
 _PLAN_SERIAL = 0
 
 
 def bump_param_epoch():
+    global PARAM_EPOCH, WEIGHT_EPOCH
+    PARAM_EPOCH += 1
+    WEIGHT_EPOCH += 1
+
+
+def bump_stats_epoch():
     global PARAM_EPOCH
     PARAM_EPOCH += 1
+
+
+_PACKERS = {}
+OWNER_EPOCH = 0
+_RUN_SERIAL = 0
+_LAST_TRAIN_PLAN = None
+
+
+def note_train_run(plan):
+    global OWNER_EPOCH, _RUN_SERIAL, _LAST_TRAIN_PLAN
+    _RUN_SERIAL += 1
+    plan.run_serial = _RUN_SERIAL
+    if _LAST_TRAIN_PLAN is None or _LAST_TRAIN_PLAN() is not plan:
+        _LAST_TRAIN_PLAN = weakref.ref(plan)
+        OWNER_EPOCH += 1
+
+
+def retire_plan(plan):
+    global OWNER_EPOCH
+    plan.retired = True
+    OWNER_EPOCH += 1
+
+
+def packing_plan(param):
+    refs = _PACKERS.get(id(param))
+    if not refs:
+        return None
+    best, alive = None, []
+    for r in refs:
+        pl = r()
+        if pl is None or pl.retired:
+            continue
+        alive.append(r)
+        w = pl.weights.get(id(param))
+        if w is None or w.param is not param:
+            continue
+        if pl.fused_weight(param) is not None and (best is None or pl.run_serial > best.run_serial):
+            best = pl
+    if alive:
+        _PACKERS[id(param)] = alive
+    else:
+        del _PACKERS[id(param)]
+    return best
 
 
 Entry = collections.namedtuple("Entry", "lane path op")
@@ -468,6 +519,8 @@
         self.dyn = {}
         self.built = False
         self._versions = None
+        self._wversions = None
+        self.run_serial, self.retired = 0, False
         self._late = []
         self.out_handles = []
         self.grad_arena = None
@@ -583,20 +636,14 @@
             for group, dest in ((early, self._pack_tables), (late, self._pack_tables_late)):
                 if not group:
                     continue
-                tab = (nv.PackEntry * len(group))()
-                for i, w in enumerate(group):
-                    tab[i].src = (w.src if w.src is not None else w.param).data_ptr()
-                    tab[i].dst = arena.data_ptr() + w.fwd_off * esz
-                    tab[i].dst_t = (arena.data_ptr() + w.bwd_off * esz) if w.need_t else None
-                    tab[i].Cout, tab[i].Cin, tab[i].ntaps, tab[i].pad_t = w.cout, w.cin, w.ntaps, w.pad_t
-                tdev = torch.frombuffer(bytearray(bytes(tab)), dtype=torch.uint8).to(dev)
-                cdt = _cdt(self, dtype)
-                first = [0]
-                for w in group:
-                    first.append(first[-1] + nv.lib().hrp_pack_blocks(w.cout, w.cin, w.ntaps, cdt, 1, 1 if w.need_t else 0))
-                fdev = torch.tensor(first, dtype=torch.int32, device=dev)
-                self.keep += [tdev, fdev]
-                dest.append((tdev, fdev, len(group), first[-1], cdt))
+                every = [w for w in group if not self._fusable(w)]
+                dest.append((self._pack_table(group, arena, esz, dtype), self._pack_table(every, arena, esz, dtype)))
+        if self.need_grad:
+            for w in self.weight_list:
+                if self._fusable(w) and self.weights.get(id(w.param)) is w:
+                    _PACKERS.setdefault(id(w.param), []).append(weakref.ref(self))
+            global OWNER_EPOCH
+            OWNER_EPOCH += 1
         self._pack_stream = None
         self._arena_clean = False
         if self._pack_tables_late:
@@ -707,6 +754,34 @@
         from . import plan_passes
         return plan_passes.analyze_backward_split(self, min_frac, fracs)
 
+    @staticmethod
+    def _fusable(w):
+        return w.src is None and w.ntaps <= nv.PACK_TILE_TAPS
+
+    def _pack_table(self, group, arena, esz, dtype):
+        if not group:
+            return None
+        tab = (nv.PackEntry * len(group))()
+        for i, w in enumerate(group):
+            tab[i].src = (w.src if w.src is not None else w.param).data_ptr()
+            tab[i].dst = arena.data_ptr() + w.fwd_off * esz
+            tab[i].dst_t = (arena.data_ptr() + w.bwd_off * esz) if w.need_t else None
+            tab[i].Cout, tab[i].Cin, tab[i].ntaps, tab[i].pad_t = w.cout, w.cin, w.ntaps, w.pad_t
+        tdev = torch.frombuffer(bytearray(bytes(tab)), dtype=torch.uint8).to(self.device)
+        cdt = _cdt(self, dtype)
+        first = [0]
+        for w in group:
+            first.append(first[-1] + nv.lib().hrp_pack_blocks(w.cout, w.cin, w.ntaps, cdt, 1, 1 if w.need_t else 0))
+        fdev = torch.tensor(first, dtype=torch.int32, device=self.device)
+        self.keep += [tdev, fdev]
+        return tdev, fdev, len(group), first[-1], cdt
+
+    def fused_weight(self, param):
+        w = self.weights.get(id(param))
+        if w is None or w.param is not param or not self._fusable(w) or w.fwd_off is None:
+            return None
+        return w, _cdt(self, w.dtype)
+
     def _late_pack_cut(self):
         if not self.need_grad or len(self.weight_list) < 64:
             return None
@@ -775,9 +850,41 @@
             return True
         return False
 
+    def _weight_versions(self):
+        return tuple(w.param._version for w in self.weight_list) + (WEIGHT_EPOCH,)
+
+    def weights_dirty(self):
+        return self._wversions is None or self._wversions != self._weight_versions()
+
+    def mark_packed(self):
+        self._wversions = self._weight_versions()
+
+    def _pack(self, tables, which, s):
+        for pair in tables:
+            t = pair[which]
+            if t is not None:
+                tdev, fdev, n, nblk, dt = t
+                nv.call("hrp_pack_weights_compact", tdev.data_ptr(), fdev.data_ptr(), n, nblk, dt, s)
+
+    def repack_weights(self):
+        s = self._stream()
+        for op in self.pre_pack:
+            op(s)
+        self._pack(self._pack_tables_late, 0, s)
+        self._pack(self._pack_tables, 0, s)
+        self.mark_packed()
+
+    def repack_if_dirty(self):
+        if self.weights_dirty():
+            self.repack_weights()
+
     def run_prep(self, force=False):
-        if not (force or self.params_dirty()):
-            return
+        if self.need_grad:
+            which = 0 if self.weights_dirty() else 1
+        else:
+            if not (force or self.params_dirty()):
+                return
+            which = 0
         s = self._stream()
         for op in self.pre_pack:
             op(s)
@@ -785,16 +892,16 @@
         if self._pack_stream is not None and not SERIAL_LANES:
             self._pack_stream.wait_stream(torch.cuda.current_stream(self.device))
             late_s = self._pack_stream.cuda_stream
-        for tdev, fdev, n, nblk, dt in self._pack_tables_late:
-            nv.call("hrp_pack_weights_compact", tdev.data_ptr(), fdev.data_ptr(), n, nblk, dt, late_s)
+        self._pack(self._pack_tables_late, which, late_s)
         if late_s != s and self.need_grad and self.grad_arena is not None and ARENA_ZERO_EARLY:
             with torch.cuda.stream(self._pack_stream):
                 self.grad_arena.zero_()
             self._arena_clean = True
-        for tdev, fdev, n, nblk, dt in self._pack_tables:
-            nv.call("hrp_pack_weights_compact", tdev.data_ptr(), fdev.data_ptr(), n, nblk, dt, s)
+        self._pack(self._pack_tables, which, s)
         if self._fold_tab:
             nv.call("hrp_bn_fold", self._fold_tab[0].data_ptr(), self._fold_tab[1], s)
+        if which == 0:
+            self.mark_packed()
 
     def lane_id(self, parent, index):
         key = (parent, index)
@@ -838,6 +945,8 @@
         s = self._stream()
         if self._rng is not None:
             nv.call("hrp_rng_advance", self._rng.data_ptr(), s)
+        if self.need_grad:
+            note_train_run(self)
         if self.training and self._run_tab:
             PARAM_EPOCH += 1
         if self.stats_floats:
diff --git a/holistic-robot-pose-estimation_amd/runtime.py b/holistic-robot-pose-estimation_amd/runtime.py
--- a/holistic-robot-pose-estimation_amd/runtime.py
+++ b/holistic-robot-pose-estimation_amd/runtime.py
@@ -4,7 +4,7 @@
 import torch.nn as nn
 
 from . import _native as nv
-from .plan import GradAccumulation, Plan, PlanBuilder, _dt
+from .plan import GradAccumulation, Plan, PlanBuilder, _dt, bump_stats_epoch, note_train_run, retire_plan
 
 
 def require_gpu(device):
@@ -26,6 +26,7 @@
         self.calls = self.bwd_calls = 0
         self.g_fwd = self.g_bwd = self.static_in = None
         self.graph_failed = False
+        self.g_fwd_packs = False
 
     def _forward_launches(self, prep=True):
         p = self.plan
@@ -66,6 +67,7 @@
             pool = self.g_fwd.pool() if self.g_fwd is not None else None
             with torch.cuda.graph(g, pool=pool, capture_error_mode="thread_local"):
                 if what == "fwd":
+                    self.g_fwd_packs = p.need_grad and p.weights_dirty()
                     self._forward_launches(prep=False)
                 else:
                     p._arena_clean = False
@@ -93,10 +95,15 @@
                 st.copy_(t)
             if not p.need_grad:
                 p.run_prep(force=False)
+            elif self.g_fwd_packs:
+                p.mark_packed()
+            else:
+                p.repack_if_dirty()
             self.g_fwd.replay()
+            if p.need_grad:
+                note_train_run(p)
             if p.training and p._run_tab:
-                from .plan import bump_param_epoch
-                bump_param_epoch()
+                bump_stats_epoch()
             return self._results()
         for n, t in zip(self.in_names, tensors):
             p.dyn[n] = t
@@ -178,6 +185,7 @@
         object.__setattr__(self, "_compute_dtype", torch.float32)
         object.__setattr__(self, "_x3", False)
         object.__setattr__(self, "_accum", None)
+        self.register_load_state_dict_post_hook(PlannedModule._state_loaded)
 
     def set_compute_dtype(self, dtype):
         x3 = dtype == "fp32x3"
@@ -188,7 +196,7 @@
             if isinstance(m, PlannedModule):
                 object.__setattr__(m, "_compute_dtype", dtype)
                 object.__setattr__(m, "_x3", x3)
-                m._plans.clear()
+                m._drop_plans()
         return self
 
     @property
@@ -280,7 +288,7 @@
     def invalidate_plans(self):
         for m in self.modules():
             if isinstance(m, PlannedModule):
-                m._plans.clear()
+                m._drop_plans()
                 if m._accum is not None:
                     object.__setattr__(m, "_accum", GradAccumulation(m._accum.steps, m._accum.scale != 1.0))
 
@@ -289,13 +297,26 @@
         self.invalidate_plans()
         return r
 
-    def load_state_dict(self, *a, **k):
-        r = super().load_state_dict(*a, **k)
+    def _drop_plans(self):
+        for r in self._plans.values():
+            retire_plan(r.plan)
+        self._plans.clear()
+
+    def repack_weights(self):
         for m in self.modules():
             if isinstance(m, PlannedModule):
-                for pl in m._plans.values():
-                    pl.plan._versions = None
-        return r
+                m._repack_own()
+        return self
+
+    def _repack_own(self):
+        for r in self._plans.values():
+            r.plan._versions = None
+            if r.plan.need_grad:
+                r.plan.repack_weights()
+
+    @staticmethod
+    def _state_loaded(module, incompatible_keys):
+        module._repack_own()
 
     def _frozen_bn_signature(self):
         if self._bn_sig[0] != MODE_EPOCH[0]:
@@ -321,7 +342,7 @@
             self._plans[key] = runner
         if runner is None:
             while len(self._plans) >= PLAN_CACHE_MAX:
-                self._plans.pop(next(iter(self._plans)))
+                retire_plan(self._plans.pop(next(iter(self._plans))).plan)
             plan = Plan(dev, self._compute_dtype, self.training, need_grad)
             plan.x3 = bool(self._x3)
             if need_grad:
diff --git a/include/hrp.h b/include/hrp.h
--- a/include/hrp.h
+++ b/include/hrp.h
@@ -248,6 +248,21 @@
                              const hrp_opt_group* groups_dev, int ngroups, const int32_t* tensor_group_dev, void* stream);
 int hrp_opt_set_group(hrp_opt_group* groups_dev, int ngroups, int index, float lr, float beta1, float beta2, float eps,
                       float weight_decay, void* stream);
+typedef struct hrp_opt_pack_entry {
+  float* param;
+  void* dst;
+  void* dst_t;
+  int32_t Cout, Cin, ntaps;
+  int32_t pad_t;
+  float* grad;
+  float* exp_avg;
+  float* exp_avg_sq;
+  int32_t group;
+  int32_t reserved;
+} hrp_opt_pack_entry;
+int hrp_opt_adam_pack_step(const hrp_opt_pack_entry* table_dev, const int32_t* first_block_dev, int count, int total_blocks,
+                           int dtype, const float* sumsq_slots, float max_norm, const float* step_dev, float lr, float beta1,
+                           float beta2, float eps, const hrp_opt_group* groups_dev, int ngroups, void* stream);
 int hrp_grad_accumulate(const float* src, float* acc, int64_t n, int first, float scale, void* stream);
 
 int hrp_ew_fwd(const hrp_ew_desc* d, void* stream);
```

Result: no change. 2046 images/sec (-0.0%).
